# NBDsoftware/deep_cartograph

Measured on AMD Instinct MI355X. Metric: Deep-TICA training frames/sec on 10Mx512 feature matrix at 1/2/4/8 GPUs, higher is better.
Workload: dtype f32

## Files before the change

### deep_cartograph_amd/_lib.py

```python
from __future__ import annotations

import ctypes as C
import os

_HERE = os.path.dirname(os.path.abspath(__file__))
LIB_PATH = os.path.join(_HERE, "csrc", "libdcv.so")

DCV_MAX_LAYERS = 16
ACT = {None: 0, "linear": 0, "leaky_relu": 1, "relu": 2, "tanh": 3, "elu": 4, "softplus": 5, "shifted_softplus": 6, "custom_sigmoid": 7}
OPTIMIZER = {"Adam": 0, "AdamW": 1, "SGD": 2, "RMSprop": 3, "Adagrad": 4, "Adamax": 5, "NAdam": 6, "RAdam": 7, "Adadelta": 8, "ASGD": 9, "Rprop": 10}
MODEL_DEEPTICA = 1
MODEL_AE = 2
MODEL_VAE = 3
FEAT_DISTANCE, FEAT_TORSION_SINCOS, FEAT_TORSION = 0, 1, 2


class MlpDesc(C.Structure):
    _fields_ = [
        ("model", C.c_int32),
        ("n_layers", C.c_int32),
        ("dims", C.c_int32 * (DCV_MAX_LAYERS + 1)),
        ("act", C.c_int32 * DCV_MAX_LAYERS),
        ("latent_layer", C.c_int32),
        ("lag", C.c_int32),
        ("max_batch", C.c_int32),
        ("tica_reg", C.c_double),
        ("lr", C.c_double),
        ("beta1", C.c_double),
        ("beta2", C.c_double),
        ("eps", C.c_double),
        ("weight_decay", C.c_double),
        ("optimizer", C.c_int32),
        ("amsgrad", C.c_int32),
        ("nesterov", C.c_int32),
        ("centered", C.c_int32),
        ("momentum", C.c_double),
        ("dampening", C.c_double),
        ("alpha", C.c_double),
        ("lr_decay", C.c_double),
        ("initial_accumulator_value", C.c_double),
        ("opt_p", C.c_double * 4),
        ("dropout", C.c_float * DCV_MAX_LAYERS),
        ("seed", C.c_uint64),
        ("batchnorm", C.c_int32 * DCV_MAX_LAYERS),
        ("bn_eps", C.c_double),
        ("bn_momentum", C.c_double),
        ("maximize", C.c_int32),
    ]


class DcvError(RuntimeError):
    pass


_P = C.c_void_p
_I64 = C.c_int64
_I32 = C.c_int32
_SZ = C.c_size_t

SIGNATURES = {
    "dcv_abi_version": (C.c_int, []),
    "dcv_last_error": (C.c_char_p, []),
    "dcv_device_info": (C.c_int, [C.c_int, C.POINTER(C.c_int), C.POINTER(_I64), C.c_char_p, _SZ]),
    "dcv_col_stats_workspace": (_SZ, [_I64, _I32]),
    "dcv_col_stats": (C.c_int, [_P, _I64, _I32, _I64, _P, _P, _SZ, _P]),
    "dcv_col_histogram_workspace": (_SZ, [_I64, _I32, _I32]),
    "dcv_col_histogram": (C.c_int, [_P, _I64, _I32, _I64, _P, _I32, _P, _P, _SZ, _P]),
    "dcv_dip_sorted_workspace": (_SZ, [_I64, _I32]),
    "dcv_dip_sorted": (C.c_int, [_P, _I64, _I32, _I64, _P, _P, _P, _P, _SZ, _P]),
    "dcv_featurize_workspace": (_SZ, [_I64, _I32, _I32]),
    "dcv_featurize": (C.c_int, [_P, _I64, _I64, _I64, _I64, _I32, _P, _I32, C.c_double, _P, _I64, _P, _SZ, _P]),
    "dcv_normalize": (C.c_int, [_P, _P, _I64, _I32, _I64, _I64, _P, _P, _P]),
    "dcv_lagged_cov_workspace": (_SZ, [_I64, _I32, _I32]),
    "dcv_lagged_cov": (C.c_int, [_P, _I64, _I32, _I64, _I32, _P, _P, _P, _SZ, _P]),
    "dcv_project_linear_workspace": (_SZ, [_I64, _I32, _I32]),
    "dcv_project_linear": (C.c_int, [_P, _I64, _I32, _I64, _P, _P, _P, _I32, _P, _P, _P, _P, _P, _P, _SZ, _P]),
    "dcv_mlp_create": (C.c_int, [C.POINTER(MlpDesc), C.POINTER(_P)]),
    "dcv_mlp_destroy": (None, [_P]),
    "dcv_mlp_num_params": (_I64, [_P]),
    "dcv_mlp_param_offset": (_I64, [_P, _I32, _I32]),
    "dcv_mlp_params": (_P, [_P]),
    "dcv_mlp_grads": (_P, [_P]),
    "dcv_mlp_set_params": (C.c_int, [_P, _P, _P]),
    "dcv_mlp_get_params": (C.c_int, [_P, _P, _P]),
    "dcv_mlp_set_lr": (C.c_int, [_P, C.c_double]),
    "dcv_mlp_set_momentum": (C.c_int, [_P, C.c_double]),
    "dcv_mlp_dropout_mask": (C.c_int, [_P, _I32, _I64, _I64, _P, _P]),
    "dcv_mlp_dropout_step": (_I64, [_P]),
    "dcv_mlp_last_path": (_I32, [_P]),
    "dcv_mlp_last_eval_group": (_I32, [_P]),
    "dcv_gemm_tn_split": (C.c_int, [_P, _I64, _P, _I64, _P, _I64, _I64, _I64, _I64, _I64, _P]),
    "dcv_mlp_set_row_sharing": (C.c_int, [_P, _I32]),
    "dcv_mlp_set_feature_range": (C.c_int, [_P, _P, _P]),
    "dcv_mlp_set_kl_beta": (C.c_int, [_P, C.c_double]),
    "dcv_mlp_set_noise": (C.c_int, [_P, _P, _I64]),
    "dcv_mlp_noise_position": (_I64, [_P]),
    "dcv_mlp_latent_sample": (C.c_int, [_P, _I64, _P, _P]),
    "dcv_mlp_forward": (C.c_int, [_P, _P, _I64, _P, _I64, _I32, _I32, _P]),
    "dcv_mlp_stats": (_P, [_P]),
    "dcv_mlp_stats_len": (_I32, [_P]),
    "dcv_mlp_backward": (C.c_int, [_P, _P, _I64, _P, _I64, _I32, _I64, _I32, _P]),
    "dcv_mlp_apply": (C.c_int, [_P, _P]),
    "dcv_mlp_set_upper_grads_callback": (C.c_int, [_P, _P, _P]),
    "dcv_mlp_dp_step": (C.c_int, [_P, _P, _I64, _P, _I64, _I32, _I64, _I32, _I32, _P, _P, _P]),
    "dcv_comm_unique_id": (C.c_int, [_P]),
    "dcv_comm_create": (C.c_int, [_I32, _I32, _P, C.POINTER(_P)]),
    "dcv_comm_destroy": (None, [_P]),
    "dcv_comm_bind_stream": (C.c_int, [_P, _P]),
    "dcv_comm_allreduce": (C.c_int, [_P, _P, _I64, _I32, _I32, _P]),
    "dcv_comm_dp_allreduce_fn": (_P, []),
    "dcv_comm_world": (_I32, [_P]),
    "dcv_comm_rank": (_I32, [_P]),
    "dcv_mlp_set_rank": (C.c_int, [_P, _I32]),
    "dcv_mlp_bn_state": (C.c_int, [_P, _I32, _P, _P, C.POINTER(_I64), _I32, _P]),
    "dcv_mlp_layer_output": (C.c_int, [_P, _I32, _I64, _P, _P]),
    "dcv_mlp_train_step": (C.c_int, [_P, _P, _I64, _P, _I64, _I32, _P]),
    "dcv_mlp_eval_step": (C.c_int, [_P, _P, _I64, _P, _I64, _I32, _P]),
    "dcv_mlp_eval_steps": (C.c_int, [_P, _P, _I64, _P, _I64, _I32, _I32, _P]),
    "dcv_mlp_train_steps": (C.c_int, [_P, _P, _I64, _P, _I64, _I32, _I32, _P]),
    "dcv_mlp_log_width": (_I32, [_P]),
    "dcv_mlp_reset_log": (C.c_int, [_P, _I32, _P]),
    "dcv_mlp_read_log": (C.c_int, [_P, _P, _I32, C.POINTER(_I32), _P]),
    "dcv_mlp_profile_begin": (C.c_int, [_P, _I32, _I32]),
    "dcv_mlp_profile_end": (C.c_int, [_P, _P, _P]),
    "dcv_mlp_profile_pause": (C.c_int, [_P, _I32]),
    "dcv_mlp_graph_launches": (_I64, [_P]),
    "dcv_mlp_set_graph": (C.c_int, [_P, _I32]),
    "dcv_mlp_infer": (C.c_int, [_P, _P, _I64, _I64, _P, _P, _P, _P, _P, _P, _P]),
    "dcv_mlp_input_sensitivity_workspace": (_SZ, [_P, _I64]),
    "dcv_mlp_input_sensitivity": (C.c_int, [_P, _P, _I64, _I64, _P, _P, _P, _P, _SZ, _P]),
    "dcv_kmeans_workspace": (_SZ, [_I64, _I32, _I32]),
    "dcv_kmeans_step": (C.c_int, [_P, _I64, _I32, _P, _P, _I32, _P, _P, _P, _P, _SZ, _P]),
    "dcv_kmeanspp_workspace": (_SZ, [_I64, _I32]),
    "dcv_kmeanspp_potentials": (C.c_int, [_P, _I64, _I32, _P, _P, _I32, _P, _P, _P, _SZ, _P]),
    "dcv_kmeanspp_update": (C.c_int, [_P, _I64, _I32, _P, _P, _I32, _P, _P, _P, _SZ, _P]),
    "dcv_set_gemm_mode": (C.c_int, [C.c_int]),
    "dcv_get_gemm_mode": (C.c_int, []),
    "dcv_label_stats_workspace": (_SZ, [_I64, _I32, _I32]),
    "dcv_label_stats": (C.c_int, [_P, _I64, _I32, _P, _P, _I32, _P, _P, _SZ, _P]),
    "dcv_cluster_dist_sums": (C.c_int, [_P, _I64, _P, _P, _I32, _I32, _P, _P]),
    "dcv_silhouette_sum_workspace": (_SZ, [_I64]),
    "dcv_silhouette_sum": (C.c_int, [_P, _I64, _I32, _P, _P, _P, _P, _SZ, _P]),
    "dcv_linear_binning_workspace": (_SZ, [_I32, _I32]),
    "dcv_linear_binning": (C.c_int, [_P, _I64, _I64, _I32, _P, _P, _P, _I32, _P, _P, _P, _SZ, _P]),
    "dcv_nearest_rows_workspace": (_SZ, [_I64, _I32, _I32]),
    "dcv_nearest_rows": (C.c_int, [_P, _I64, _I32, _P, _I32, _I64, _P, _P, _P, _SZ, _P]),
    "dcv_nearest_point": (C.c_int, [_P, _I64, _P, _I64, _I32, _P, _P]),
    "dcv_linkage_workspace": (_SZ, [_I64, _I32]),
    "dcv_linkage_pdist": (C.c_int, [_P, _I64, _I32, _P, _SZ, _P]),
    "dcv_linkage": (C.c_int, [_P, _I64, _I32, _I32, _P, C.POINTER(_I64), _P, _SZ, _P]),
    "dcv_core_distances_workspace": (_SZ, [_I64, _I32, _I32]),
    "dcv_core_distances": (C.c_int, [_P, _I64, _I32, _I32, _P, _P, _SZ, _P]),
    "dcv_mr_mst_workspace": (_SZ, [_I64, _I32]),
    "dcv_mr_mst": (C.c_int, [_P, _I64, _I32, _P, _P, _P, _P, _P, _SZ, _P]),
    "dcv_gemm_f32": (C.c_int, [_I32, _P, _I64, _P, _I64, _P, _I64, _I64, _I64, _I64, _P]),
}

_lib = None


def load():
    global _lib
    if _lib is not None:
        return _lib
    if not os.path.exists(LIB_PATH):
        raise DcvError(
            f"libdcv.so not found at {LIB_PATH}: build it with `python -c 'import __graft_entry__ as g; g.build()'` "
            "or `make -C deep_cartograph_amd/csrc` -- there is no CPU fallback")
    lib = C.CDLL(LIB_PATH)
    for name, (res, args) in SIGNATURES.items():
        fn = getattr(lib, name)
        fn.restype = res
        fn.argtypes = args
    ver = lib.dcv_abi_version()
    if ver != 5:
        raise DcvError(f"libdcv.so ABI version {ver}, expected 5 (rebuild: make -C deep_cartograph_amd/csrc)")
    _lib = lib
    return lib


def check(rc: int, what: str = ""):
    if rc != 0:
        msg = load().dcv_last_error().decode(errors="replace")
        raise DcvError(f"{what} failed (code {rc}): {msg}")
```

### deep_cartograph_amd/csrc/mlp.hip

```cpp
#include "mlp_state.h"
#include <new>
#include <math.h>
#include <utility>

using namespace dcv;

namespace dcv {

__global__ __launch_bounds__(256) void colsum_kernel(const float* __restrict__ Z, int64_t rows, int n, int64_t ld,
                                                     float* __restrict__ part) {
    __shared__ float red[256];
    const int64_t r0 = (int64_t)blockIdx.x * kColsumRows;
    const int64_t r1 = r0 + kColsumRows < rows ? r0 + kColsumRows : rows;
    const int t = threadIdx.x;
    const int cols = n < 256 ? n : 256;
    const int groups = 256 / cols;
    const int c_in = t % cols, g = t / cols;
    for (int c0 = 0; c0 < n; c0 += cols) {
        const int c = c0 + c_in;
        float s = 0.f;
        if (g < groups && c < n) {
            for (int64_t rb = r0 + g; rb < r1; rb += 8 * (int64_t)groups) {
                float v[8];
#pragma unroll
                for (int u = 0; u < 8; ++u) {
                    const int64_t r = rb + (int64_t)u * groups;
                    v[u] = r < r1 ? Z[r * ld + c] : 0.f;
                }
#pragma unroll
                for (int u = 0; u < 8; ++u) s += v[u];
            }
        }
        red[t] = s;
        __syncthreads();
        if (g == 0 && c < n) {
            float tot = 0.f;
            for (int q = 0; q < groups; ++q) tot += red[q * cols + c_in];
            part[(int64_t)blockIdx.x * n + c] = tot;
        }
        __syncthreads();
    }
}

__global__ __launch_bounds__(kVaeRows) void vae_sample_kernel(const float* __restrict__ H, int64_t ldh, int64_t R, int d,
                                                             const float* __restrict__ eps, float* __restrict__ Z, int64_t ldz,
                                                             double* __restrict__ part) {
    __shared__ double red[kVaeRows];
    const int t = threadIdx.x;
    const int64_t r = (int64_t)blockIdx.x * kVaeRows + t;
    double kl = 0.0;
    if (r < R) {
        for (int j = 0; j < d; ++j) {
            const float mu = H[r * ldh + j], lv = H[r * ldh + d + j];
            Z[r * ldz + j] = __fadd_rn(__fmul_rn(eps[r * d + j], expf(0.5f * lv)), mu);
            kl += (double)lv - exp((double)lv) - (double)mu * (double)mu + 1.0;
        }
        kl *= -0.5;
    }
    red[t] = kl;
    __syncthreads();
    for (int off = kVaeRows / 2; off > 0; off >>= 1) {
        if (t < off) red[t] += red[t + off];
        __syncthreads();
    }
    if (t == 0) part[blockIdx.x] = red[0];
}

__global__ __launch_bounds__(kVaeRows) void vae_sample_backward_kernel(const float* __restrict__ H, int64_t ldh, int64_t R, int d,
                                                                      const float* __restrict__ eps, float* __restrict__ G, int64_t ldg,
                                                                      float beta_over_b) {
    const int64_t r = (int64_t)blockIdx.x * kVaeRows + threadIdx.x;
    if (r >= R) return;
    float dz[8];
    for (int j = 0; j < d; ++j) dz[j] = G[r * ldg + j];
    for (int j = 0; j < d; ++j) {
        const float mu = H[r * ldh + j], lv = H[r * ldh + d + j];
        G[r * ldg + j] = dz[j] + beta_over_b * mu;
        G[r * ldg + d + j] = dz[j] * eps[r * d + j] * 0.5f * expf(0.5f * lv) + beta_over_b * 0.5f * (expf(lv) - 1.f);
    }
}

__global__ __launch_bounds__(256) void dropout_mask_kernel(float* __restrict__ out, int64_t rows, int width, DropCfg drop) {
    const int q4 = (width + 3) / 4;
    for (int64_t i = (int64_t)blockIdx.x * 256 + threadIdx.x; i < rows * q4; i += (int64_t)gridDim.x * 256) {
        const int64_t r = i / q4;
        const int c = (int)(i - r * q4) * 4;
        const float4 k = drop.thr != 0u ? drop.mult(r, c) : make_float4(1.f, 1.f, 1.f, 1.f);
        float* o = out + r * width + c;
        o[0] = k.x;
        if (c + 1 < width) o[1] = k.y;
        if (c + 2 < width) o[2] = k.z;
        if (c + 3 < width) o[3] = k.w;
    }
}

static void wgrad_plan(int out, int in, int64_t rows, int64_t* k_chunk, int64_t* splits) {
    const int64_t tiles = (out <= 32 ? 1 : cdiv(out, 128)) * (in <= 32 ? 1 : cdiv(in, 128));
    int64_t want = cdiv(2 * (int64_t)num_cus(), tiles);
    int64_t max_by_rows = cdiv(rows, 256);
    static const bool q_wide = [] { const char* e = getenv("DCV_WGRAD_Q"); return e && e[0] == '1'; }();
    const int64_t tiles_q = cdiv(out, 64) * cdiv(in, 64);
    const int64_t want_q = cdiv(cdiv(2 * (int64_t)num_cus(), tiles_q), 8) * 8;
    if (out > 32 && in > 32 && want_q <= max_by_rows) {
        int64_t kc = cdiv(cdiv(rows, want_q), 32) * 32;
        if (cdiv(rows, kc) % 8 != 0) kc = cdiv(rows, want_q);
        if (tiles * cdiv(rows, kc) <= (int64_t)num_cus() / 2 &&
            (want > max_by_rows || (q_wide && kc <= 1024))) {
            *k_chunk = kc;
            *splits = cdiv(rows, kc);
            return;
        }
    }
    if (want > max_by_rows) {
        want = max_by_rows >= 8 ? max_by_rows / 8 * 8 : max_by_rows;
    }
    if (want < 1) want = 1;
    int64_t kc = cdiv(cdiv(rows, want), 32) * 32;
    *k_chunk = kc;
    *splits = cdiv(rows, kc);
}

static void mlp_free(dcv_mlp* m) {
    if (!m) return;
    snet_free(m);
    snet_dt_free(m);
    snet_image_free(m);
    auto f = [](void* p) { if (p) (void)hipFree(p); };
    f(m->params); f(m->grads); f(m->adam_m); f(m->adam_v); f(m->opt_aux); f(m->dZ[0]); f(m->dZ[1]); f(m->stats); f(m->gradp);
    f(m->spart); f(m->log); f(m->log_count); f(m->ticket); f(m->feat_range); f(m->ident); f(m->zeros_d); f(m->ones_d); f(m->proj_ws);
    f(m->vae_z); f(m->vae_kpart);
    for (auto& l : m->layers) { f(l.H); f(l.slab); f(l.bpart); f(l.mask); f(l.Y); f(l.rm); f(l.rv); f(l.bn_stat); f(l.bn_part); f(l.bn_gpart); f(l.bn_bpart); }
    g_launch_ev = LaunchEvents{};
    g_launch_taken = nullptr;
    for (hipEvent_t e : m->prof_ev) (void)hipEventDestroy(e);
    f(m->tail.ws); f(m->tail.cnt); f(m->eval_ws.base);
    for (int i = 0; i < 4; ++i) if (m->gexec[i]) (void)hipGraphExecDestroy(m->gexec[i]);
    delete m;
}

static int reset_bn_state(dcv_mlp* m, hipStream_t s) {
    for (auto& p : m->layers) {
        if (!p.bn) continue;
        DCV_CHECK_HIP(hipMemsetAsync(p.rm, 0, (size_t)p.out * sizeof(float), s));
        launch_fill(p.rv, (int64_t)p.out, 1.f, 1, 256, s);
        DCV_CHECK_LAUNCH();
        p.bn_batches = 0;
    }
    return DCV_OK;
}

static int create_validate(const dcv_mlp_desc* desc) {
    const int L = desc->n_layers;
    DCV_REQUIRE(desc->model == DCV_MODEL_DEEPTICA || desc->model == DCV_MODEL_AE || desc->model == DCV_MODEL_VAE, "dcv_mlp_create: unknown model %d",
                desc->model);
    DCV_REQUIRE(L >= 1 && L <= DCV_MAX_LAYERS, "dcv_mlp_create: n_layers=%d out of range", L);
    for (int l = 0; l <= L; ++l) DCV_REQUIRE(desc->dims[l] >= 1, "dcv_mlp_create: dims[%d]=%d", l, desc->dims[l]);
    for (int l = 0; l < L; ++l)
        DCV_REQUIRE(desc->act[l] >= DCV_ACT_NONE && desc->act[l] <= DCV_ACT_CUSTOM_SIGMOID, "dcv_mlp_create: act[%d]=%d unsupported", l, desc->act[l]);
    for (int l = 0; l < L; ++l)
        DCV_REQUIRE(desc->dropout[l] >= 0.f && desc->dropout[l] < 1.f, "dcv_mlp_create: dropout[%d]=%g outside [0, 1)", l, (double)desc->dropout[l]);
    DCV_REQUIRE(desc->optimizer >= DCV_OPT_ADAM && desc->optimizer <= DCV_OPT_RPROP, "dcv_mlp_create: optimizer %d unknown", desc->optimizer);
    DCV_REQUIRE(desc->max_batch >= 1, "dcv_mlp_create: max_batch=%d", desc->max_batch);
    if (desc->model == DCV_MODEL_DEEPTICA) {
        DCV_REQUIRE(desc->dims[L] <= kMaxTicaDim, "dcv_mlp_create: Deep-TICA output dimension %d > %d", desc->dims[L], kMaxTicaDim);
        DCV_REQUIRE(desc->lag >= 0, "dcv_mlp_create: lag=%d", desc->lag);
    } else {
        DCV_REQUIRE(desc->dims[L] == desc->dims[0], "dcv_mlp_create: autoencoder must map F=%d back to F (got %d)", desc->dims[0], desc->dims[L]);
        DCV_REQUIRE(desc->latent_layer >= 1 && desc->latent_layer < L, "dcv_mlp_create: latent_layer=%d", desc->latent_layer);
        DCV_REQUIRE(desc->dims[desc->latent_layer] <= 16, "dcv_mlp_create: latent dimension %d > 16", desc->dims[desc->latent_layer]);
        if (desc->model == DCV_MODEL_VAE) {
            const int h = desc->latent_layer - 1;
            DCV_REQUIRE(desc->dims[desc->latent_layer] % 2 == 0 && desc->dims[desc->latent_layer] <= 16,
                        "dcv_mlp_create: VAE head layer %d must output 2 * d <= 16 columns (got %d)", h, desc->dims[desc->latent_layer]);
            DCV_REQUIRE(desc->act[h] == DCV_ACT_NONE && !(desc->dropout[h] > 0.f) && !desc->batchnorm[h],
                        "dcv_mlp_create: the VAE heads (Linear %d) take no activation, dropout or batch normalisation", h);
        }
    }
    return DCV_OK;
}
static int proj_dim(const dcv_mlp* m) {
    return m->desc.model == DCV_MODEL_AE ? m->desc.dims[m->desc.latent_layer] : m->desc.model == DCV_MODEL_VAE ? m->vae_d : m->d_out;
}
static void plan_layers(dcv_mlp* m) {
    const dcv_mlp_desc* desc = &m->desc;
    const int L = m->L;
    m->layers.resize(L);
    int64_t off = 0;
    int maxdim = 0;
    for (int l = 0; l < L; ++l) {
        LayerPlan& p = m->layers[l];
        p.in = m->vae_d > 0 && l == desc->latent_layer ? m->vae_d : desc->dims[l];
        p.out = desc->dims[l + 1];
        p.act = desc->act[l];
        p.w_off = off;
        off += align_up((size_t)p.in * p.out, 4);
        p.b_off = off;
        off += align_up((size_t)p.out, 4);
        p.bn = desc->batchnorm[l] ? 1 : 0;
        if (p.bn) {
            p.g_off = off;
            off += align_up((size_t)p.out, 4);
            p.be_off = off;
            off += align_up((size_t)p.out, 4);
            m->any_bn = true;
        }
        p.ldh = align_up((size_t)p.out, 4);
        if (p.out > maxdim) maxdim = p.out;
        wgrad_plan(p.out, p.in, m->rows_cap, &p.k_chunk_cap, &p.max_splits);
        p.max_splits = cdiv(m->rows_cap, 256) > p.max_splits ? p.max_splits : cdiv(m->rows_cap, 256);
        if (p.max_splits < 1) p.max_splits = 1;
        if (l == L - 1 && p.out <= 8) {
            int64_t hb = 4 * (int64_t)num_cus();
            if (hb > cdiv(m->rows_cap, 32)) hb = cdiv(m->rows_cap, 32);
            if (hb > p.max_splits) p.max_splits = hb;
        }
    }
    m->n_params = off;
    m->ld_dz = align_up((size_t)maxdim, 4);
    const int d = m->d_out;
    m->stats_len = desc->model == DCV_MODEL_DEEPTICA ? 2 * d + 2 * d * d : desc->model == DCV_MODEL_VAE ? 2 : 1;
    m->log_width = desc->model == DCV_MODEL_DEEPTICA ? 2 + 2 * d * d + d : desc->model == DCV_MODEL_VAE ? 4 : 2;
    m->spart_blocks = desc->model == DCV_MODEL_DEEPTICA ? (int)cdiv(desc->max_batch, kStatBlockRows) : (int)cdiv(m->rows_cap, kSseRows);
}
static int alloc_buffers(dcv_mlp* m) {
    const dcv_mlp_desc* desc = &m->desc;
    int rc = DCV_OK;
    for (int l = 0; l < m->L && rc == DCV_OK; ++l) {
        LayerPlan& p = m->layers[l];
        rc = dmalloc(&p.H, (size_t)m->rows_cap * p.ldh);
        if (rc == DCV_OK) rc = dmalloc(&p.slab, (size_t)p.max_splits * p.in * p.out);
        if (rc == DCV_OK) rc = dmalloc(&p.bpart, (size_t)cdiv(m->rows_cap, 32) * p.out);
        if (rc == DCV_OK && p.bn) {
            const size_t nblk = (size_t)cdiv(m->rows_cap, 256) + 2;
            rc = dmalloc(&p.Y, (size_t)m->rows_cap * p.ldh);
            if (rc == DCV_OK) rc = dmalloc(&p.rm, (size_t)p.out);
            if (rc == DCV_OK) rc = dmalloc(&p.rv, (size_t)p.out);
            if (rc == DCV_OK) rc = dmalloc(&p.bn_stat, (size_t)4 * p.out);
            if (rc == DCV_OK) rc = dmalloc(&p.bn_part, nblk * 2 * p.out);
            if (rc == DCV_OK) rc = dmalloc(&p.bn_gpart, nblk * p.out);
            if (rc == DCV_OK) rc = dmalloc(&p.bn_bpart, nblk * p.out);
        }
        if (rc == DCV_OK && l + 1 < m->L && (p.act == DCV_ACT_RELU || p.act == DCV_ACT_LEAKY_RELU))
            rc = dmalloc(&p.mask, (size_t)((m->rows_cap + 128) * (int64_t)(p.out + 128)) / 64 + 64);
    }
    const int dl = proj_dim(m);
    if (rc == DCV_OK) rc = dmalloc(&m->params, (size_t)m->n_params);
    if (rc == DCV_OK) rc = dmalloc(&m->grads, (size_t)m->n_params);
    if (rc == DCV_OK) rc = dmalloc(&m->adam_m, (size_t)m->n_params);
    if (rc == DCV_OK) rc = dmalloc(&m->adam_v, (size_t)m->n_params);
    if (rc == DCV_OK && (((desc->optimizer == DCV_OPT_ADAM || desc->optimizer == DCV_OPT_ADAMW) && desc->amsgrad) ||
                         (desc->optimizer == DCV_OPT_RMSPROP && desc->centered)))
        rc = dmalloc(&m->opt_aux, (size_t)m->n_params);
    if (rc == DCV_OK) rc = dmalloc(&m->dZ[0], (size_t)m->rows_cap * m->ld_dz);
    if (rc == DCV_OK) rc = dmalloc(&m->dZ[1], (size_t)m->rows_cap * m->ld_dz);
    if (rc == DCV_OK) rc = dmalloc(&m->stats, (size_t)m->stats_len);
    if (rc == DCV_OK) rc = dmalloc(&m->gradp, (size_t)(2 * kMaxTicaDim + 2 * kMaxTicaDim * kMaxTicaDim));
    if (rc == DCV_OK) rc = dmalloc(&m->spart, (size_t)m->spart_blocks * m->stats_len);
    if (rc == DCV_OK) rc = dmalloc(&m->log_count, 1);
    if (rc == DCV_OK) rc = dmalloc(&m->ticket, 4);
    if (rc == DCV_OK) rc = dmalloc(&m->feat_range, (size_t)desc->dims[0]);
    if (rc == DCV_OK && m->vae_d > 0) rc = dmalloc(&m->vae_z, (size_t)m->rows_cap * m->ld_z);
    if (rc == DCV_OK && m->vae_d > 0) rc = dmalloc(&m->vae_kpart, (size_t)cdiv(m->rows_cap, kVaeRows));
    if (rc == DCV_OK) rc = dmalloc(&m->ident, (size_t)dl * dl);
    if (rc == DCV_OK) rc = dmalloc(&m->zeros_d, (size_t)dl);
    if (rc == DCV_OK) rc = dmalloc(&m->ones_d, (size_t)dl);
    m->proj_ws_bytes = dcv_project_linear_workspace(m->rows_cap, dl, dl);
    if (rc == DCV_OK) rc = dmalloc(reinterpret_cast<char**>(&m->proj_ws), m->proj_ws_bytes);
    return rc;
}
static int init_device_state(dcv_mlp* m) {
    const int dl = proj_dim(m);
    hipError_t e = hipMemset(m->params, 0, m->n_params * sizeof(float));
    if (e == hipSuccess) e = hipMemset(m->grads, 0, m->n_params * sizeof(float));
    if (e == hipSuccess && reset_opt_state(m, nullptr) != DCV_OK) e = hipErrorUnknown;
    if (e == hipSuccess) e = hipMemset(m->log_count, 0, sizeof(int));
    if (e == hipSuccess) e = hipMemset(m->ticket, 0, 4 * sizeof(unsigned));
    if (e == hipSuccess) e = hipMemset(m->zeros_d, 0, dl * sizeof(float));
    if (e == hipSuccess) e = hipMemset(m->ident, 0, (size_t)dl * dl * sizeof(float));
    if (e == hipSuccess) {
        launch_fill(m->ones_d, (int64_t)dl, 1.f, 1, 64, nullptr);
        launch_fill(m->feat_range, (int64_t)m->desc.dims[0], 1.f, 4, 256, nullptr);
        std::vector<float> eye((size_t)dl * dl, 0.f);
        for (int i = 0; i < dl; ++i) eye[(size_t)i * dl + i] = 1.f;
        e = hipMemcpy(m->ident, eye.data(), eye.size() * sizeof(float), hipMemcpyHostToDevice);
    }
    if (e == hipSuccess) {
        for (auto& p : m->layers)
            if (p.bn) launch_fill(m->params + p.g_off, (int64_t)p.out, 1.f, 1, 256, nullptr);
        if (reset_bn_state(m, nullptr) != DCV_OK) e = hipErrorUnknown;
    }
    if (e == hipSuccess) (void)alloc_tail_ws(&m->tail, 8);
    if (e == hipSuccess) e = hipDeviceSynchronize();
    if (e == hipSuccess) return DCV_OK;
    set_error("dcv_mlp_create: initialisation failed: %s", hipGetErrorString(e));
    return DCV_EHIP;
}

}

extern "C" int dcv_mlp_create(const dcv_mlp_desc* desc, dcv_mlp** out) {
    DCV_REQUIRE(desc && out, "dcv_mlp_create: null argument");
    *out = nullptr;
    int rc = create_validate(desc);
    if (rc) return rc;
    dcv_mlp* m = new (std::nothrow) dcv_mlp();
    DCV_REQUIRE(m, "dcv_mlp_create: out of host memory");
    m->desc = *desc;
    m->L = desc->n_layers;
    m->d_out = desc->dims[m->L];
    m->rows_cap = desc->model == DCV_MODEL_DEEPTICA ? 2 * (int64_t)desc->max_batch : desc->max_batch;
    m->lr = desc->lr;
    m->momentum_rt = (desc->optimizer == DCV_OPT_ADAM || desc->optimizer == DCV_OPT_ADAMW || desc->optimizer == DCV_OPT_ADAMAX ||
                      desc->optimizer == DCV_OPT_NADAM || desc->optimizer == DCV_OPT_RADAM) ? desc->beta1 : desc->momentum;
    for (int l = 0; l < m->L; ++l) m->any_drop = m->any_drop || desc->dropout[l] > 0.f;
    m->vae_d = desc->model == DCV_MODEL_VAE ? desc->dims[desc->latent_layer] / 2 : 0;
    m->ld_z = align_up((size_t)(m->vae_d > 0 ? m->vae_d : 1), 4);
    static const bool graph_env = [] { const char* e = getenv("DCV_GRAPH"); return e && e[0] == '1'; }();
    m->graph_on = graph_env;
    plan_layers(m);
    rc = alloc_buffers(m);
    if (rc == DCV_OK) rc = init_device_state(m);
    if (rc != DCV_OK) {
        mlp_free(m);
        return rc;
    }
    *out = m;
    return DCV_OK;
}

extern "C" void dcv_mlp_destroy(dcv_mlp* m) { mlp_free(m); }
extern "C" int64_t dcv_mlp_num_params(const dcv_mlp* m) { return m ? m->n_params : 0; }
extern "C" int64_t dcv_mlp_param_offset(const dcv_mlp* m, int32_t layer, int32_t which) {
    if (!m || layer < 0 || layer >= m->L) return -1;
    if (which == 2) return m->layers[layer].g_off;
    if (which == 3) return m->layers[layer].be_off;
    return which == 0 ? m->layers[layer].w_off : m->layers[layer].b_off;
}
extern "C" float* dcv_mlp_params(dcv_mlp* m) { return m ? m->params : nullptr; }
extern "C" float* dcv_mlp_grads(dcv_mlp* m) { return m ? m->grads : nullptr; }
extern "C" double* dcv_mlp_stats(dcv_mlp* m) { return m ? m->stats : nullptr; }
extern "C" int32_t dcv_mlp_stats_len(const dcv_mlp* m) { return m ? m->stats_len : 0; }
extern "C" int32_t dcv_mlp_log_width(const dcv_mlp* m) { return m ? m->log_width : 0; }

extern "C" int dcv_mlp_set_params(dcv_mlp* m, const float* params_h, void* stream) {
    DCV_REQUIRE(m && params_h, "dcv_mlp_set_params: null argument");
    hipStream_t s = as_stream(stream);
    DCV_CHECK_HIP(hipMemcpyAsync(m->params, params_h, m->n_params * sizeof(float), hipMemcpyHostToDevice, s));
    int rc = reset_opt_state(m, s);
    if (rc == DCV_OK) rc = reset_bn_state(m, s);
    if (rc == DCV_OK) rc = snet_image_repack(m, s);
    if (rc) return rc;
    DCV_CHECK_HIP(hipStreamSynchronize(s));
    return DCV_OK;
}

extern "C" int dcv_mlp_get_params(dcv_mlp* m, float* params_h, void* stream) {
    DCV_REQUIRE(m && params_h, "dcv_mlp_get_params: null argument");
    hipStream_t s = as_stream(stream);
    DCV_CHECK_HIP(hipMemcpyAsync(params_h, m->params, m->n_params * sizeof(float), hipMemcpyDeviceToHost, s));
    DCV_CHECK_HIP(hipStreamSynchronize(s));
    return DCV_OK;
}

extern "C" int dcv_mlp_bn_state(dcv_mlp* m, int32_t layer, float* running_mean_h, float* running_var_h, int64_t* num_batches_tracked,
                                int32_t set, void* stream) {
    DCV_REQUIRE(m && layer >= 0 && layer < m->L && running_mean_h && running_var_h && num_batches_tracked, "dcv_mlp_bn_state: bad arguments");
    LayerPlan& p = m->layers[layer];
    DCV_REQUIRE(p.bn, "dcv_mlp_bn_state: layer %d has no batch normalisation", layer);
    hipStream_t s = as_stream(stream);
    const size_t bytes = (size_t)p.out * sizeof(float);
    if (set) {
        DCV_CHECK_HIP(hipMemcpyAsync(p.rm, running_mean_h, bytes, hipMemcpyHostToDevice, s));
        DCV_CHECK_HIP(hipMemcpyAsync(p.rv, running_var_h, bytes, hipMemcpyHostToDevice, s));
        p.bn_batches = *num_batches_tracked;
    } else {
        DCV_CHECK_HIP(hipMemcpyAsync(running_mean_h, p.rm, bytes, hipMemcpyDeviceToHost, s));
        DCV_CHECK_HIP(hipMemcpyAsync(running_var_h, p.rv, bytes, hipMemcpyDeviceToHost, s));
        *num_batches_tracked = p.bn_batches;
    }
    DCV_CHECK_HIP(hipStreamSynchronize(s));
    return DCV_OK;
}

extern "C" int dcv_mlp_set_row_sharing(dcv_mlp* m, int32_t enable) {
    DCV_REQUIRE(m, "dcv_mlp_set_row_sharing: null");
    m->no_row_sharing = enable ? 0 : 1;
    return DCV_OK;
}

extern "C" int dcv_mlp_set_lr(dcv_mlp* m, double lr) {
    DCV_REQUIRE(m, "dcv_mlp_set_lr: null");
    m->lr = lr;
    return DCV_OK;
}

extern "C" int dcv_mlp_set_momentum(dcv_mlp* m, double value) {
    DCV_REQUIRE(m, "dcv_mlp_set_momentum: null");
    m->momentum_rt = value;
    return DCV_OK;
}

extern "C" int dcv_mlp_set_upper_grads_callback(dcv_mlp* m, void (*fn)(void*), void* user) {
    DCV_REQUIRE(m, "dcv_mlp_set_upper_grads_callback: null");
    m->upper_cb = fn;
    m->upper_cb_user = user;
    return DCV_OK;
}

extern "C" int dcv_mlp_set_rank(dcv_mlp* m, int32_t rank) {
    DCV_REQUIRE(m && rank >= 0, "dcv_mlp_set_rank: bad arguments");
    m->drop_rank = (uint32_t)rank;
    return DCV_OK;
}

extern "C" int dcv_mlp_layer_output(dcv_mlp* m, int32_t layer, int64_t rows, float* out_d, void* stream) {
    DCV_REQUIRE(m && out_d && layer >= 0 && layer < m->L && rows >= 1 && rows <= m->rows_cap, "dcv_mlp_layer_output: bad arguments");
    if (m->last_path != 0) {
        set_error("dcv_mlp_layer_output: the last forward ran as a fused small-network launch (activations never left LDS); set DCV_NO_SNET=1");
        return DCV_ESTATE;
    }
    const LayerPlan& p = m->layers[layer];
    DCV_CHECK_HIP(hipMemcpy2DAsync(out_d, (size_t)p.out * sizeof(float), p.H, (size_t)p.ldh * sizeof(float), (size_t)p.out * sizeof(float),
                                   (size_t)rows, hipMemcpyDeviceToDevice, as_stream(stream)));
    return DCV_OK;
}

extern "C" int64_t dcv_mlp_dropout_step(const dcv_mlp* m) { return m ? m->drop_step : 0; }
extern "C" int32_t dcv_mlp_last_path(const dcv_mlp* m) { return m ? m->last_path : -1; }
extern "C" int32_t dcv_mlp_last_eval_group(const dcv_mlp* m) { return m ? m->last_eval_group : -1; }

extern "C" int dcv_mlp_dropout_mask(dcv_mlp* m, int32_t layer, int64_t step, int64_t rows, float* out_d, void* stream) {
    DCV_REQUIRE(m && out_d && layer >= 0 && layer < m->L && rows >= 1 && step >= 0, "dcv_mlp_dropout_mask: bad arguments");
    const bool keep_mode = m->fwd_train;
    const int64_t keep_step = m->cur_step;
    m->fwd_train = true;
    m->cur_step = step;
    const DropCfg dc = drop_cfg(m, layer);
    m->fwd_train = keep_mode;
    m->cur_step = keep_step;
    const int width = m->layers[layer].out;
    int64_t blocks = cdiv(rows * ((width + 3) / 4), 256);
    if (blocks > 4096) blocks = 4096;
    hipLaunchKernelGGL(dropout_mask_kernel, dim3((unsigned)blocks), dim3(256), 0, as_stream(stream), out_d, rows, width, dc);
    DCV_CHECK_LAUNCH();
    return DCV_OK;
}

extern "C" int dcv_mlp_set_feature_range(dcv_mlp* m, const float* range_h, void* stream) {
    DCV_REQUIRE(m && range_h, "dcv_mlp_set_feature_range: null argument");
    hipStream_t s = as_stream(stream);
    DCV_CHECK_HIP(hipMemcpyAsync(m->feat_range, range_h, m->desc.dims[0] * sizeof(float), hipMemcpyHostToDevice, s));
    DCV_CHECK_HIP(hipStreamSynchronize(s));
    return DCV_OK;
}

extern "C" int dcv_mlp_set_kl_beta(dcv_mlp* m, double beta) {
    DCV_REQUIRE(m && m->vae_d > 0, "dcv_mlp_set_kl_beta: not a variational autoencoder");
    m->kl_beta = beta;
    return DCV_OK;
}

extern "C" int dcv_mlp_set_noise(dcv_mlp* m, const float* eps_d, int64_t rows) {
    DCV_REQUIRE(m && m->vae_d > 0, "dcv_mlp_set_noise: not a variational autoencoder");
    DCV_REQUIRE(rows >= 0 && (eps_d != nullptr || rows == 0), "dcv_mlp_set_noise: bad arguments");
    m->noise = eps_d;
    m->noise_rows = rows;
    m->noise_pos = 0;
    return DCV_OK;
}

extern "C" int64_t dcv_mlp_noise_position(const dcv_mlp* m) { return m ? m->noise_pos : -1; }

extern "C" int dcv_mlp_latent_sample(dcv_mlp* m, int64_t rows, float* out_d, void* stream) {
    DCV_REQUIRE(m && out_d && m->vae_d > 0, "dcv_mlp_latent_sample: bad arguments");
    DCV_REQUIRE(rows >= 1 && rows <= m->last_batch, "dcv_mlp_latent_sample: rows=%lld outside [1, %d]", (long long)rows, m->last_batch);
    if (m->last_path != 0) {
        set_error("dcv_mlp_latent_sample: the last forward ran fused: z never left LDS");
        return DCV_ESTATE;
    }
    DCV_CHECK_HIP(hipMemcpy2DAsync(out_d, (size_t)m->vae_d * sizeof(float), m->vae_z, (size_t)m->ld_z * sizeof(float), (size_t)m->vae_d * sizeof(float),
                                   (size_t)rows, hipMemcpyDeviceToDevice, as_stream(stream)));
    return DCV_OK;
}

extern "C" int dcv_mlp_reset_log(dcv_mlp* m, int32_t capacity, void* stream) {
    DCV_REQUIRE(m && capacity >= 1, "dcv_mlp_reset_log: bad arguments");
    hipStream_t s = as_stream(stream);
    if (capacity > m->log_cap) {
        DCV_CHECK_HIP(hipStreamSynchronize(s));
        if (m->log) (void)hipFree(m->log);
        m->log = nullptr;
        m->log_cap = 0;
        int rc = dmalloc(&m->log, (size_t)capacity * m->log_width);
        if (rc) return rc;
        m->log_cap = capacity;
    }
    DCV_CHECK_HIP(hipMemsetAsync(m->log_count, 0, sizeof(int), s));
    return DCV_OK;
}

extern "C" int dcv_mlp_read_log(dcv_mlp* m, double* out_h, int32_t max_records, int32_t* n_records, void* stream) {
    DCV_REQUIRE(m && out_h && n_records, "dcv_mlp_read_log: null argument");
    hipStream_t s = as_stream(stream);
    int cnt = 0;
    DCV_CHECK_HIP(hipMemcpyAsync(&cnt, m->log_count, sizeof(int), hipMemcpyDeviceToHost, s));
    DCV_CHECK_HIP(hipStreamSynchronize(s));
    if (cnt > m->log_cap) cnt = m->log_cap;
    if (cnt > max_records) cnt = max_records;
    if (cnt > 0) {
        DCV_CHECK_HIP(hipMemcpyAsync(out_h, m->log, (size_t)cnt * m->log_width * sizeof(double), hipMemcpyDeviceToHost, s));
        DCV_CHECK_HIP(hipStreamSynchronize(s));
    }
    *n_records = cnt;
    return DCV_OK;
}

namespace dcv {

static bool act_mask_enabled() {
    static const bool off = [] { const char* e = getenv("DCV_NO_ACT_MASK"); return e && e[0] == '1'; }();
    return !off;
}

int run_forward(dcv_mlp* m, const float* Xn, int64_t ld, const RowMap& rows_map, int64_t rows, int n_run, hipStream_t s,
                bool for_backward) {
    for (int l = 0; l < n_run; ++l) {
        LayerPlan& p = m->layers[l];
        p.mask_rows = -1;
        const bool from_z = m->vae_d > 0 && l == m->desc.latent_layer;
        if (from_z) {
            const LayerPlan& hd = m->layers[l - 1];
            m->vae_kblocks = (int)cdiv(rows, kVaeRows);
            hipLaunchKernelGGL(vae_sample_kernel, dim3((unsigned)m->vae_kblocks), dim3(kVaeRows), 0, s, (const float*)hd.H, hd.ldh, rows, m->vae_d,
                               m->eps_cur, m->vae_z, m->ld_z, m->vae_kpart);
            DCV_CHECK_LAUNCH();
        }
        Operand A = l == 0 ? make_operand(Xn, ld, p.in, rows_map)
                           : from_z ? make_operand(m->vae_z, m->ld_z, p.in) : make_operand(layer_out(m, l - 1), m->layers[l - 1].ldh, p.in);
        Operand B = make_operand(m->params + p.w_off, p.in, p.in);
        if (l + 1 < n_run && next_layer_fusable(m, l)) {
            LayerPlan& nx = m->layers[l + 1];
            const bool vec = quad_ok(p.H, p.ldh) && quad_ok(m->params + p.b_off, 4) && quad_ok(m->params + nx.w_off, nx.in);
            prof_mark(m, l, 0, 0, s);
            int rc;
            if (nx.out <= 4) {
                EpiBiasActHead<4> epi{p.H, p.ldh, m->params + p.b_off, p.act, vec, m->params + nx.w_off, nx.in, m->params + nx.b_off, nx.out, nx.act, nx.H, nx.ldh};
                epi.drop = drop_cfg(m, l);
                rc = gemm_nt_head4(A, B, rows, p.out, p.in, epi, s, &m->tail);
            } else {
                EpiBiasActHead<8> epi{p.H, p.ldh, m->params + p.b_off, p.act, vec, m->params + nx.w_off, nx.in, m->params + nx.b_off, nx.out, nx.act, nx.H, nx.ldh};
                epi.drop = drop_cfg(m, l);
                rc = gemm_nt_head8(A, B, rows, p.out, p.in, epi, s, &m->tail);
            }
            if (rc) return rc;
            prof_mark(m, l, 0, 1, s);
            prof_mark(m, l + 1, 0, 0, s);
            prof_mark(m, l + 1, 0, 1, s);
            ++l;
            continue;
        }
        EpiBiasAct epi{p.H, p.ldh, m->params + p.b_off, p.act, quad_ok(p.H, p.ldh) && quad_ok(m->params + p.b_off, 4)};
        epi.drop = drop_cfg(m, l);
        if (for_backward && p.mask && act_mask_enabled()) {
            epi.mask = p.mask;
            p.mask_rows = rows;
        }
        prof_mark(m, l, 0, 0, s);
        if (p.bn) {
            epi.mask = nullptr;
            p.mask_rows = -1;
        }
        int rc = gemm_nt_bias_act(A, B, rows, p.out, p.in, epi, s, &m->tail);
        if (rc) return rc;
        if (p.bn) {
            const bool train = m->fwd_train && for_backward;
            if (train && rows_map.half > 0) {
                rc = bn_forward(m, l, 0, rows_map.half, true, s);
                if (rc == DCV_OK) rc = bn_forward(m, l, rows_map.half, rows - rows_map.half, true, s);
            } else {
                rc = bn_forward(m, l, 0, rows, train, s);
            }
            if (rc) return rc;
        }
        prof_mark(m, l, 0, 1, s);
    }
    return DCV_OK;
}

template <class F>
static int run_graphed(dcv_mlp* m, int slot, hipStream_t s, F&& body) {
    if (!m->graph_on || m->graph_off || s == nullptr || (m->prof_level > 0 && !m->prof_paused) || !m->gwarm[slot]) {
        m->gwarm[slot] = true;
        return body();
    }
    if (hipStreamBeginCapture(s, hipStreamCaptureModeThreadLocal) != hipSuccess) {
        (void)hipGetLastError();
        return body();
    }
    struct HostStep {
        int64_t adam_t, drop_step, cur_step;
        double mu_product, eta;
        int64_t bn_batches[DCV_MAX_LAYERS];
        int64_t noise_pos;
        const float* eps_cur;
    };
    auto snap = [&]() {
        HostStep h{m->adam_t, m->drop_step, m->cur_step, m->nadam_mu_product, m->asgd_eta, {}, m->noise_pos, m->eps_cur};
        for (int l = 0; l < m->L; ++l) h.bn_batches[l] = m->layers[l].bn_batches;
        return h;
    };
    auto restore = [&](const HostStep& h) {
        m->adam_t = h.adam_t; m->drop_step = h.drop_step; m->cur_step = h.cur_step;
        m->nadam_mu_product = h.mu_product; m->asgd_eta = h.eta;
        for (int l = 0; l < m->L; ++l) m->layers[l].bn_batches = h.bn_batches[l];
        m->noise_pos = h.noise_pos; m->eps_cur = h.eps_cur;
    };
    const HostStep h0 = snap();
    const int rc = body();
    hipGraph_t g = nullptr;
    const hipError_t ec = hipStreamEndCapture(s, &g);
    if (rc != DCV_OK || ec != hipSuccess || g == nullptr) {
        if (g) (void)hipGraphDestroy(g);
        (void)hipGetLastError();
        if (rc != DCV_OK) return rc;
        m->gwarm[slot] = false;
        restore(h0);
        return body();
    }
    if (m->gexec[slot]) {
        hipGraphNode_t err_node = nullptr;
        hipGraphExecUpdateResult res = hipGraphExecUpdateSuccess;
        if (hipGraphExecUpdate(m->gexec[slot], g, &err_node, &res) != hipSuccess || res != hipGraphExecUpdateSuccess) {
            (void)hipGetLastError();
            (void)hipGraphExecDestroy(m->gexec[slot]);
            m->gexec[slot] = nullptr;
        }
    }
    if (!m->gexec[slot] && hipGraphInstantiate(&m->gexec[slot], g, nullptr, nullptr, 0) != hipSuccess) {
        (void)hipGetLastError();
        m->gexec[slot] = nullptr;
    }
    (void)hipGraphDestroy(g);
    if (!m->gexec[slot]) {
        m->graph_off = true;
        restore(h0);
        return body();
    }
    DCV_CHECK_HIP(hipGraphLaunch(m->gexec[slot], s));
    m->graph_launches += 1;
    return DCV_OK;
}

bool peek_noise(dcv_mlp* m, int64_t rows) {
    if (m->noise == nullptr || m->noise_pos + rows > m->noise_rows) return false;
    m->eps_cur = m->noise + m->noise_pos * m->vae_d;
    return true;
}
static int take_noise(dcv_mlp* m, int64_t batch) {
    if (!peek_noise(m, batch)) {
        set_error("dcv_mlp step: the VAE noise buffer holds %lld rows, %lld used, a step of %lld rows needs more (dcv_mlp_set_noise)",
                  (long long)m->noise_rows, (long long)m->noise_pos, (long long)batch);
        return DCV_ESTATE;
    }
    m->noise_pos += batch;
    return DCV_OK;
}

int forward_impl(dcv_mlp* m, const float* Xn_d, int64_t ld, const int64_t* idx_d, int64_t row0, int32_t batch, int32_t train, void* stream,
                 int fuse_head) {
    DCV_REQUIRE(m && Xn_d, "dcv_mlp_forward: null argument");
    DCV_REQUIRE(batch >= 1 && batch <= m->desc.max_batch, "dcv_mlp_forward: batch=%d exceeds max_batch=%d", batch, m->desc.max_batch);
    DCV_REQUIRE(ld >= m->desc.dims[0], "dcv_mlp_forward: ld=%lld < F=%d", (long long)ld, m->desc.dims[0]);
    if (fuse_head) DCV_REQUIRE(m->log && m->log_cap > 0, "dcv_mlp step: call dcv_mlp_reset_log first");
    if (m->vae_d > 0) {
        const int rcn = take_noise(m, batch);
        if (rcn) return rcn;
    }
    g_launch_ev = LaunchEvents{};
    step_begin(m, train != 0);
    step_done(m, 0, m->last_batch, false);
    hipStream_t s = as_stream(stream);
    if (m->desc.model == DCV_MODEL_DEEPTICA && !(m->snet_dt_tried && m->snet_dt == nullptr)) {
        prof_mark(m, 0, 0, 0, s);
        const int rcs = snet_dt_forward(m, Xn_d, ld, idx_d, row0, batch, fuse_head == 2 ? 2 : 0, fuse_head != 2, s);
        if (rcs < 0) return rcs;
        if (rcs == DCV_OK) {
            prof_mark(m, 0, 0, 1, s);
            step_done(m, 2, batch, fuse_head == 2);
            return DCV_OK;
        }
        if (prof_on(m, 0)) g_launch_ev = LaunchEvents{};
    }
    const RowMap rm = batch_rows(m, idx_d, row0, batch);
    const int64_t R = rows_of(m, idx_d, batch);
    int rc = run_forward(m, Xn_d, ld, rm, R, m->L, s, fuse_head != 2);
    if (rc) return rc;
    const LayerPlan& last = m->layers[m->L - 1];
    const float* net_out = layer_out(m, m->L - 1);
    bool head_ran = fuse_head != 0;
    if (m->desc.model == DCV_MODEL_DEEPTICA) rc = tica_stats(m, net_out, last.ldh, batch, lag_offset(m, idx_d, batch), fuse_head, &head_ran, s);
    else rc = ae_sse(m, net_out, last.ldh, Xn_d, ld, rm, R, batch, fuse_head != 0, s);
    if (rc) return rc;
    step_done(m, 0, batch, head_ran);
    return DCV_OK;
}

struct Backward {
    dcv_mlp* m;
    const float* Xn;
    int64_t ld;
    const int64_t* idx;
    RowMap rm;
    int64_t R;
    int32_t batch;
    int64_t global_batch;
    hipStream_t s;
    float *dz_cur, *dz_nxt;
    int bblocks;
    ReduceArgs ra;
};

static int backward_blob(dcv_mlp* m, int32_t batch, int64_t global_batch, bool head_in_bwd, bool fuse_opt, hipStream_t s) {
    if (!m->snet_fwd_valid) {
        set_error("dcv_mlp_backward: the fused forward of this batch kept no activations (evaluation step)");
        return DCV_ESTATE;
    }
    ReduceArgsView v;
    prof_mark(m, 0, 1, 0, s);
    const int rc = snet_dt_backward(m, batch, global_batch, head_in_bwd, &v, s);
    if (rc) return rc;
    prof_mark(m, 0, 1, 1, s);
    return finish_grads(m, reduce_args_of(m, v), fuse_opt, false, s);
}
static int seed_gradient(Backward& c, bool fused_head) {
    dcv_mlp* m = c.m;
    const LayerPlan& last = m->layers[m->L - 1];
    const float* net_out = layer_out(m, m->L - 1);
    const int act = last.bn ? DCV_ACT_NONE : last.act;
    const DropCfg drop = last.bn ? kNoDrop : drop_cfg(m, m->L - 1);
    const float hscale = last.bn ? 1.f : drop_hscale(m, m->L - 1);
    int rc = DCV_OK;
    if (!fused_head)
        rc = loss_gradient(m, net_out, last.ldh, c.Xn, c.ld, c.rm, c.R, c.batch, lag_offset(m, c.idx, c.batch), c.global_batch, act, c.dz_cur, drop, hscale, c.s);
    c.bblocks = (int)cdiv(c.R, kColsumRows);
    if (rc == DCV_OK && !fused_head && !last.bn) {
        hipLaunchKernelGGL(colsum_kernel, dim3(c.bblocks), dim3(256), 0, c.s, c.dz_cur, c.R, last.out, m->ld_dz, last.bpart);
        DCV_CHECK_LAUNCH();
    }
    return rc;
}
static int norm_backward(Backward& c, int l) {
    const LayerPlan& p = c.m->layers[l];
    const bool two = c.rm.half > 0;
    int nb = 0;
    const int rc = bn_backward(c.m, l, c.dz_cur, c.m->ld_dz, two ? 2 : 1, two ? (int64_t)c.rm.half : c.R, p.act, drop_hscale(c.m, l), drop_cfg(c.m, l), &nb, c.s);
    if (rc) return rc;
    c.bblocks = nb;
    c.ra.l[c.m->L + l] = ReduceDesc{p.bn_gpart, p.bn_bpart, p.g_off, p.be_off, p.out, p.out, nb, nb, 0, 0};
    return DCV_OK;
}
static int head_backward_layer(Backward& c) {
    dcv_mlp* m = c.m;
    const int l = m->L - 1;
    prof_mark(m, l, 1, 0, c.s);
    const int rc = head_backward(m, c.R, c.batch, lag_offset(m, c.idx, c.batch), c.dz_nxt, &c.bblocks, c.s);
    if (rc) return rc;
    prof_mark(m, l, 1, 1, c.s);
    prof_mark(m, l, 2, 0, c.s);
    prof_mark(m, l, 2, 1, c.s);
    c.ra.l[l] = linear_reduce_desc(m->layers[l], c.bblocks, c.bblocks);
    std::swap(c.dz_cur, c.dz_nxt);
    return DCV_OK;
}
static int64_t plan_wgrad(Backward& c, int l) {
    const LayerPlan& p = c.m->layers[l];
    int64_t kc, splits;
    wgrad_plan(p.out, p.in, c.R, &kc, &splits);
    if (splits > p.max_splits) {
        splits = p.max_splits;
        kc = cdiv(cdiv(c.R, splits), 32) * 32;
        splits = cdiv(c.R, kc);
    }
    c.ra.l[l] = linear_reduce_desc(p, (int)splits, c.bblocks);
    return kc;
}
static EpiSlab slab_epi(const LayerPlan& p) { return EpiSlab{p.slab, p.out, p.in, 1, 0, quad_ok(p.slab, p.in), p.max_splits}; }
static int wgrad_alone(Backward& c, int l, const Operand& B, int64_t kc) {
    const LayerPlan& p = c.m->layers[l];
    prof_mark(c.m, l, 1, 0, c.s);
    const int rc = gemm_tn_slab(make_operand(c.dz_cur, c.m->ld_dz, p.out), B, p.out, p.in, c.R, kc, slab_epi(p), c.s);
    if (rc) return rc;
    prof_mark(c.m, l, 1, 1, c.s);
    return DCV_OK;
}
static int latent_backward_layer(Backward& c, int l) {
    dcv_mlp* m = c.m;
    const LayerPlan& p = m->layers[l];
    const LayerPlan& hd = m->layers[l - 1];
    const int64_t kc = plan_wgrad(c, l);
    int rc = wgrad_alone(c, l, make_operand(m->vae_z, m->ld_z, p.in), kc);
    if (rc) return rc;
    Operand A = make_operand(c.dz_cur, m->ld_dz, p.out);
    Operand Bd = make_operand(m->params + p.w_off, p.in, p.in);
    EpiActGrad eg{c.dz_nxt, m->ld_dz, m->vae_z, m->ld_z, DCV_ACT_NONE, hd.bpart, p.in, quad_ok(c.dz_nxt, m->ld_dz) && quad_ok(m->vae_z, m->ld_z)};
    int dblocks = 0;
    prof_mark(m, l, 2, 0, c.s);
    rc = gemm_nn_act_grad(A, Bd, c.R, p.in, p.out, eg, c.s, &dblocks, &m->tail);
    if (rc) return rc;
    hipLaunchKernelGGL(vae_sample_backward_kernel, dim3((unsigned)cdiv(c.R, kVaeRows)), dim3(kVaeRows), 0, c.s, (const float*)hd.H, hd.ldh, c.R, m->vae_d,
                       m->eps_cur, c.dz_nxt, m->ld_dz, (float)(m->kl_beta / (double)c.global_batch));
    DCV_CHECK_LAUNCH();
    c.bblocks = (int)cdiv(c.R, kColsumRows);
    hipLaunchKernelGGL(colsum_kernel, dim3(c.bblocks), dim3(256), 0, c.s, (const float*)c.dz_nxt, c.R, hd.out, m->ld_dz, hd.bpart);
    DCV_CHECK_LAUNCH();
    prof_mark(m, l, 2, 1, c.s);
    std::swap(c.dz_cur, c.dz_nxt);
    return DCV_OK;
}
static int backward_layer(Backward& c, int l) {
    dcv_mlp* m = c.m;
    hipStream_t s = c.s;
    const LayerPlan& p = m->layers[l];
    const int64_t R = c.R;
    const int64_t kc = plan_wgrad(c, l);
    if (l == 0) return wgrad_alone(c, l, make_operand(c.Xn, c.ld, p.in, c.rm), kc);
    const LayerPlan& q = m->layers[l - 1];
    Operand A = make_operand(c.dz_cur, m->ld_dz, p.out);
    Operand B = make_operand(layer_out(m, l - 1), q.ldh, p.in);
    const EpiSlab epi = slab_epi(p);
    Operand Bd = make_operand(m->params + p.w_off, p.in, p.in);
    EpiActGrad eg{c.dz_nxt, m->ld_dz, q.H, q.ldh, q.act, q.bpart, q.out, quad_ok(c.dz_nxt, m->ld_dz) && quad_ok(q.H, q.ldh)};
    if (q.mask && q.mask_rows == R) {
        eg.mask = q.mask;
        eg.slope = q.act == DCV_ACT_LEAKY_RELU ? 0.01f : 0.f;
    }
    eg.drop = drop_cfg(m, l - 1);
    eg.hscale = drop_hscale(m, l - 1);
    if (q.bn) {
        eg.act = DCV_ACT_NONE;
        eg.mask = nullptr;
        eg.drop = kNoDrop;
        eg.hscale = 1.f;
    }
    prof_mark(m, l, 1, 0, s);
    prof_mark(m, l, 2, 0, s);
    int rc = launch_wgrad_dgrad(A, B, p.out, p.in, R, kc, epi, A, Bd, R, p.in, p.out, eg, &c.bblocks, &m->tail, s);
    if (rc < 0) return rc;
    if (rc == 1) {
        rc = gemm_tn_slab(A, B, p.out, p.in, R, kc, epi, s);
        if (rc) return rc;
        prof_mark(m, l, 1, 1, s);
        prof_mark(m, l, 2, 0, s);
        rc = gemm_nn_act_grad(A, Bd, R, p.in, p.out, eg, s, &c.bblocks, &m->tail);
        if (rc) return rc;
        prof_mark(m, l, 2, 1, s);
    } else {
        prof_mark(m, l, 1, 1, s);
        prof_mark(m, l, 2, 1, s);
    }
    std::swap(c.dz_cur, c.dz_nxt);
    return DCV_OK;
}

int backward_impl(dcv_mlp* m, const float* Xn_d, int64_t ld, const int64_t* idx_d, int64_t row0, int32_t batch, int64_t global_batch, int32_t train,
                  void* stream, bool fuse_opt) {
    DCV_REQUIRE(m && Xn_d, "dcv_mlp_backward: null argument");
    g_launch_ev = LaunchEvents{};
    if (m->last_batch != batch) {
        set_error("dcv_mlp_backward: batch=%d does not match the preceding forward (%d)", batch, m->last_batch);
        return DCV_ESTATE;
    }
    DCV_REQUIRE(global_batch >= batch, "dcv_mlp_backward: global_batch=%lld < batch=%d", (long long)global_batch, batch);
    if (m->any_drop && train && !m->fwd_train) {
        set_error("dcv_mlp_backward: train=1 after an evaluation-mode forward (dropout masks would not match)");
        return DCV_ESTATE;
    }
    DCV_REQUIRE(m->log && m->log_cap > 0, "dcv_mlp_backward: call dcv_mlp_reset_log first");
    hipStream_t s = as_stream(stream);
    const bool tica = m->desc.model == DCV_MODEL_DEEPTICA;
    const bool head_in_bwd = tica && m->last_path == 2 && train && !m->head_done && m->snet_fwd_valid;
    int rc = loss_record(m, global_batch, train != 0, head_in_bwd, s);
    if (rc || !train) return rc;
    if (tica && m->last_path == 2) return backward_blob(m, batch, global_batch, head_in_bwd, fuse_opt, s);
    const int L = m->L;
    Backward c{m, Xn_d, ld, idx_d, batch_rows(m, idx_d, row0, batch), rows_of(m, idx_d, batch), batch, global_batch, s, m->dZ[0], m->dZ[1], 0, ReduceArgs{}};
    c.ra.L = L;
    const bool fused_head = tica && head_fusable(m);
    rc = seed_gradient(c, fused_head);
    bool upper_done = false;
    for (int l = L - 1; l >= 0 && rc == DCV_OK; --l) {
        if (l == 0) rc = reduce_upper(m, c.ra, fuse_opt, &upper_done, s);
        if (rc == DCV_OK && m->layers[l].bn) rc = norm_backward(c, l);
        if (rc) break;
        if (fused_head && l == L - 1) rc = head_backward_layer(c);
        else if (m->vae_d > 0 && l == m->desc.latent_layer) rc = latent_backward_layer(c, l);
        else rc = backward_layer(c, l);
    }
    if (rc) return rc;
    return finish_grads(m, c.ra, fuse_opt, upper_done, s);
}

static int snet_step(dcv_mlp* m, const float* Xn_d, int64_t ld, const int64_t* idx_d, int64_t row0, int32_t batch, int32_t train, void* stream) {
    if ((m->desc.model != DCV_MODEL_AE && m->desc.model != DCV_MODEL_VAE) || m->any_drop || m->any_bn || (m->snet_tried && m->snet == nullptr)) return 1;
    if (!(Xn_d && batch >= 1 && batch <= m->desc.max_batch && ld >= m->desc.dims[0] && m->log && m->log_cap > 0)) return 1;
    if (m->vae_d > 0 && !peek_noise(m, batch)) return 1;
    hipStream_t s = as_stream(stream);
    ReduceArgsView v;
    prof_mark(m, 0, 0, 0, s);
    prof_mark(m, 0, 1, 0, s);
    int rc = snet_ae_step(m, Xn_d, ld, RowMap{idx_d, row0, 0, 0}, batch, batch, train, &v, s);
    if (rc) return rc;
    if (m->vae_d > 0) m->noise_pos += batch;
    prof_mark(m, 0, 0, 1, s);
    prof_mark(m, 0, 1, 1, s);
    step_begin(m, train != 0);
    step_done(m, 1, batch, false);
    if (!train) return DCV_OK;
    return finish_grads(m, reduce_args_of(m, v), true, false, s);
}

}

extern "C" int dcv_mlp_profile_begin(dcv_mlp* m, int32_t max_steps, int32_t level) {
    DCV_REQUIRE(m && max_steps >= 1 && (level == 1 || level == 2), "dcv_mlp_profile_begin: bad arguments");
    const size_t need = (size_t)3 * m->L * max_steps * 2;
    while (m->prof_ev.size() < need) {
        hipEvent_t e;
        DCV_CHECK_HIP(hipEventCreate(&e));
        m->prof_ev.push_back(e);
    }
    m->prof_cap = max_steps;
    m->prof_cnt.assign((size_t)3 * m->L, 0);
    m->prof_kind_off = 0;
    m->prof_paused = false;
    m->prof_level = level;
    return DCV_OK;
}

extern "C" int dcv_mlp_profile_pause(dcv_mlp* m, int32_t paused) {
    DCV_REQUIRE(m, "dcv_mlp_profile_pause: null");
    m->prof_paused = (paused & 1) != 0;
    m->prof_kind_off = (paused >> 1) & 7;
    return DCV_OK;
}

extern "C" int dcv_mlp_profile_end(dcv_mlp* m, double* ms_h, int32_t* counts_h) {
    DCV_REQUIRE(m && ms_h && counts_h, "dcv_mlp_profile_end: null argument");
    const int level = m->prof_level;
    m->prof_level = 0;
    for (int c = 0; c < 3 * m->L; ++c) {
        ms_h[c] = 0.0;
        counts_h[c] = 0;
        const int layer = c / 3, kind = c % 3;
        if (level < 2 && layer != 0) continue;
        if (kind == 2 && layer == 0) continue;
        const int steps = (size_t)c < m->prof_cnt.size() ? m->prof_cnt[c] : 0;
        for (int i = 0; i < steps; ++i) {
            hipEvent_t a = m->prof_ev[((size_t)c * m->prof_cap + i) * 2 + 0];
            hipEvent_t b = m->prof_ev[((size_t)c * m->prof_cap + i) * 2 + 1];
            DCV_CHECK_HIP(hipEventSynchronize(b));
            float ms = 0.f;
            DCV_CHECK_HIP(hipEventElapsedTime(&ms, a, b));
            ms_h[c] += (double)ms;
            counts_h[c] += 1;
        }
    }
    return DCV_OK;
}

extern "C" int dcv_mlp_forward(dcv_mlp* m, const float* Xn_d, int64_t ld, const int64_t* idx_d, int64_t row0, int32_t batch,
                               int32_t train, void* stream) {
    DCV_REQUIRE(m, "dcv_mlp_forward: null");
    return run_graphed(m, 1, as_stream(stream), [&] { return forward_impl(m, Xn_d, ld, idx_d, row0, batch, train, stream); });
}

extern "C" int dcv_mlp_backward(dcv_mlp* m, const float* Xn_d, int64_t ld, const int64_t* idx_d, int64_t row0, int32_t batch,
                                int64_t global_batch, int32_t train, void* stream) {
    DCV_REQUIRE(m, "dcv_mlp_backward: null");
    if (!train) return backward_impl(m, Xn_d, ld, idx_d, row0, batch, global_batch, train, stream);
    return run_graphed(m, 2, as_stream(stream), [&] { return backward_impl(m, Xn_d, ld, idx_d, row0, batch, global_batch, train, stream); });
}

extern "C" int dcv_mlp_apply(dcv_mlp* m, void* stream) { return apply_impl(m, stream); }
extern "C" int64_t dcv_mlp_graph_launches(const dcv_mlp* m) { return m ? m->graph_launches : 0; }
extern "C" int dcv_mlp_set_graph(dcv_mlp* m, int32_t enable) {
    DCV_REQUIRE(m, "dcv_mlp_set_graph: null");
    m->graph_on = enable != 0;
    return DCV_OK;
}

static int one_step(dcv_mlp* m, const float* Xn_d, int64_t ld, const int64_t* idx_d, int64_t row0, int32_t batch, int32_t train, void* stream) {
    int rc = snet_step(m, Xn_d, ld, idx_d, row0, batch, train, stream);
    if (rc != 1) return rc;
    rc = forward_impl(m, Xn_d, ld, idx_d, row0, batch, train, stream, train ? 1 : 2);
    if (rc) return rc;
    return backward_impl(m, Xn_d, ld, idx_d, row0, batch, batch, train, stream, train != 0);
}
extern "C" int dcv_mlp_train_step(dcv_mlp* m, const float* Xn_d, int64_t ld, const int64_t* idx_d, int64_t row0, int32_t batch,
                                  void* stream) {
    DCV_REQUIRE(m, "dcv_mlp_train_step: null");
    return run_graphed(m, 0, as_stream(stream), [&] { return one_step(m, Xn_d, ld, idx_d, row0, batch, 1, stream); });
}

extern "C" int dcv_mlp_eval_step(dcv_mlp* m, const float* Xn_d, int64_t ld, const int64_t* idx_d, int64_t row0, int32_t batch,
                                 void* stream) {
    DCV_REQUIRE(m, "dcv_mlp_eval_step: null");
    return run_graphed(m, 3, as_stream(stream), [&] { return one_step(m, Xn_d, ld, idx_d, row0, batch, 0, stream); });
}
```

### deep_cartograph_amd/csrc/mlp_opt.hip

```cpp
#include "mlp_state.h"
#include <math.h>

namespace dcv {

static inline int64_t rd_wstride(const ReduceDesc& d) { return d.w_stride > 0 ? d.w_stride : d.w_count; }
static inline int64_t rd_bstride(const ReduceDesc& d) { return d.b_stride > 0 ? d.b_stride : (int64_t)d.out; }

struct OptArgs {
    int kind, flag;
    int first;
    float lr, b1, b2, eps, wd;
    float c1, c2;
    float w1, w2;
    float decay;
    float p0, p1, p2, p3;
    int maximize;
    float* img;
    const int* img_idx;
};
template <bool WT>
__device__ __forceinline__ void opt_st(float* p, float v) {
    if constexpr (WT) handoff_store(p, v);
    else *p = v;
}
template <bool WT>
__device__ __forceinline__ void opt_stp(const OptArgs& a, float* p, int64_t i, float v) {
    opt_st<WT>(p + i, v);
    if (a.img != nullptr) {
        const int j = a.img_idx[i];
        if (j >= 0) opt_st<WT>(a.img + j, v);
    }
}
template <bool WT = false>
__device__ __forceinline__ void opt_update_p(int64_t i, float gi, float pi, float* __restrict__ p, float* __restrict__ s1, float* __restrict__ s2,
                                             float* __restrict__ s3, const OptArgs& a) {
    if (a.maximize) gi = -gi;
    switch (a.kind) {
        case DCV_OPT_ADAM:
        case DCV_OPT_ADAMW: {
            if (a.kind == DCV_OPT_ADAMW) pi = pi * a.decay;
            else if (a.wd != 0.f) gi = fmaf(a.wd, pi, gi);
            float mi = s1[i], vi = s2[i];
            mi = mi + (gi - mi) * a.w1;
            vi = vi * a.b2 + a.w2 * gi * gi;
            float vden = vi;
            if (a.flag) {
                vden = fmaxf(s3[i], vi);
                opt_st<WT>(s3 + i, vden);
            }
            const float denom = sqrtf(vden) / a.c2 + a.eps;
            opt_st<WT>(s1 + i, mi);
            opt_st<WT>(s2 + i, vi);
            opt_stp<WT>(a, p, i, pi - a.c1 * (mi / denom));
            break;
        }
        case DCV_OPT_SGD: {
            if (a.wd != 0.f) gi = fmaf(a.wd, pi, gi);
            if (a.b1 != 0.f) {
                float bi = a.first ? gi : s1[i] * a.b1 + a.w1 * gi;
                opt_st<WT>(s1 + i, bi);
                gi = a.flag ? fmaf(a.b1, bi, gi) : bi;
            }
            opt_stp<WT>(a, p, i, pi - a.lr * gi);
            break;
        }
        case DCV_OPT_RMSPROP: {
            if (a.wd != 0.f) gi = fmaf(a.wd, pi, gi);
            float sq = s2[i] * a.b2 + a.w2 * gi * gi;
            opt_st<WT>(s2 + i, sq);
            float avg;
            if (a.flag) {
                float ga = s3[i];
                ga = ga + (gi - ga) * a.w2;
                opt_st<WT>(s3 + i, ga);
                avg = sqrtf(sq - ga * ga) + a.eps;
            } else {
                avg = sqrtf(sq) + a.eps;
            }
            if (a.b1 > 0.f) {
                const float bi = s1[i] * a.b1 + gi / avg;
                opt_st<WT>(s1 + i, bi);
                opt_stp<WT>(a, p, i, pi - a.lr * bi);
            } else {
                opt_stp<WT>(a, p, i, pi - a.lr * (gi / avg));
            }
            break;
        }
        case DCV_OPT_ADAMAX: {
            if (a.wd != 0.f) gi = fmaf(a.wd, pi, gi);
            float mi = s1[i];
            mi = mi + (gi - mi) * a.w1;
            const float ui = fmaxf(s2[i] * a.b2, fabsf(gi) + a.eps);
            opt_st<WT>(s1 + i, mi);
            opt_st<WT>(s2 + i, ui);
            opt_stp<WT>(a, p, i, pi - a.c1 * (mi / ui));
            break;
        }
        case DCV_OPT_NADAM: {
            if (a.wd != 0.f) {
                if (a.flag) pi = pi * a.decay;
                else gi = fmaf(a.wd, pi, gi);
            }
            float mi = s1[i], vi = s2[i];
            mi = mi + (gi - mi) * a.w1;
            vi = vi * a.b2 + a.w2 * gi * gi;
            const float denom = sqrtf(vi / a.c2) + a.eps;
            opt_st<WT>(s1 + i, mi);
            opt_st<WT>(s2 + i, vi);
            pi = pi + a.p0 * (gi / denom);
            opt_stp<WT>(a, p, i, pi + a.p1 * (mi / denom));
            break;
        }
        case DCV_OPT_RADAM: {
            if (a.wd != 0.f) {
                if (a.flag) pi = pi * a.decay;
                else gi = fmaf(a.wd, pi, gi);
            }
            float mi = s1[i], vi = s2[i];
            mi = mi + (gi - mi) * a.w1;
            vi = vi * a.b2 + a.w2 * gi * gi;
            opt_st<WT>(s1 + i, mi);
            opt_st<WT>(s2 + i, vi);
            const float mhat = mi / a.c1;
            if (a.p0 > 0.f) opt_stp<WT>(a, p, i, pi - ((mhat * a.lr) * (a.c2 / (sqrtf(vi) + a.eps))) * a.p0);
            else opt_stp<WT>(a, p, i, pi - mhat * a.lr);
            break;
        }
        case DCV_OPT_ADADELTA: {
            if (a.wd != 0.f) gi = fmaf(a.wd, pi, gi);
            const float sq = s1[i] * a.b2 + a.w2 * gi * gi;
            const float acc = s2[i];
            const float delta = sqrtf(acc + a.eps) / sqrtf(sq + a.eps) * gi;
            opt_st<WT>(s1 + i, sq);
            opt_st<WT>(s2 + i, acc * a.b2 + a.w2 * delta * delta);
            opt_stp<WT>(a, p, i, pi - a.lr * delta);
            break;
        }
        case DCV_OPT_ASGD: {
            if (a.wd != 0.f) gi = fmaf(a.wd, pi, gi);
            pi = pi * a.p0;
            opt_stp<WT>(a, p, i, pi - a.p1 * gi);
            break;
        }
        case DCV_OPT_RPROP: {
            const float sg = gi * s1[i];
            const float f = sg > 0.f ? a.p1 : (sg < 0.f ? a.p0 : 1.f);
            const float st = fminf(fmaxf(s2[i] * f, a.p2), a.p3);
            opt_st<WT>(s2 + i, st);
            if (sg < 0.f) gi = 0.f;
            const float sgn = gi > 0.f ? 1.f : (gi < 0.f ? -1.f : 0.f);
            opt_stp<WT>(a, p, i, pi - sgn * st);
            opt_st<WT>(s1 + i, gi);
            break;
        }
        default: {
            if (a.wd != 0.f) gi = fmaf(a.wd, pi, gi);
            const float su = s2[i] + gi * gi;
            opt_st<WT>(s2 + i, su);
            opt_stp<WT>(a, p, i, pi - a.c1 * (gi / (sqrtf(su) + a.eps)));
            break;
        }
    }
}
__device__ __forceinline__ void opt_update(int64_t i, float gi, float* __restrict__ p, float* __restrict__ s1, float* __restrict__ s2,
                                           float* __restrict__ s3, const OptArgs& a) {
    opt_update_p(i, gi, p[i], p, s1, s2, s3, a);
}
__global__ __launch_bounds__(256) void optimizer_kernel(float* __restrict__ p, const float* __restrict__ g, float* __restrict__ s1,
                                                        float* __restrict__ s2, float* __restrict__ s3, int64_t n, OptArgs a) {
    for (int64_t i = (int64_t)blockIdx.x * 256 + threadIdx.x; i < n; i += (int64_t)gridDim.x * 256) opt_update(i, g[i], p, s1, s2, s3, a);
}

constexpr int kRedWaves = 16;
__global__ __launch_bounds__(64 * kRedWaves) void reduce_grads_kernel(ReduceArgs a, float* __restrict__ grads, float scale, int fuse,
                                                                      float* __restrict__ params, float* __restrict__ s1,
                                                                      float* __restrict__ s2, float* __restrict__ s3, OptArgs oa) {
    __shared__ double s_red[kRedWaves][64];
    const int l = blockIdx.y;
    const ReduceDesc& d = a.l[l];
    const int64_t total = d.w_count + d.out;
    const int lane = threadIdx.x & 63, wave = threadIdx.x >> 6;
    for (int64_t base = (int64_t)blockIdx.x * 64; base < total; base += (int64_t)gridDim.x * 64) {
        const int64_t i = base + lane;
        double s = 0.0;
        if (i < d.w_count) {
            const float* p = d.slab + i;
#pragma unroll 8
            for (int q = wave; q < d.splits; q += kRedWaves) s += (double)p[(int64_t)q * (d.w_stride > 0 ? d.w_stride : d.w_count)];
        } else if (i < total) {
            const float* p = d.bpart + (i - d.w_count);
#pragma unroll 8
            for (int q = wave; q < d.bblocks; q += kRedWaves) s += (double)p[(int64_t)q * (d.b_stride > 0 ? d.b_stride : (int64_t)d.out)];
        }
        s_red[wave][lane] = s;
        __syncthreads();
        if (wave == 0 && i < total) {
            double tot = 0.0;
#pragma unroll
            for (int w = 0; w < kRedWaves; ++w) tot += s_red[w][lane];
            const float g = (float)(tot * (double)scale);
            const int64_t pidx = i < d.w_count ? d.w_off + i : d.b_off + (i - d.w_count);
            grads[pidx] = g;
            if (fuse) opt_update(pidx, g, params, s1, s2, s3, oa);
        }
        __syncthreads();
    }
}

__global__ __launch_bounds__(256) void reduce_grads_small_kernel(ReduceArgs a, float* __restrict__ grads, float scale, int fuse,
                                                                 float* __restrict__ params, float* __restrict__ s1,
                                                                 float* __restrict__ s2, float* __restrict__ s3, OptArgs oa) {
    __shared__ double s_red[4][64];
    const ReduceDesc& d = a.l[blockIdx.y];
    const int64_t total = d.w_count + d.out;
    const int lane = threadIdx.x & 63, wave = threadIdx.x >> 6;
    for (int64_t base = (int64_t)blockIdx.x * 64; base < total; base += (int64_t)gridDim.x * 64) {
        const int64_t i = base + lane;
        double s = 0.0;
        if (i < d.w_count) {
            const float* p = d.slab + i;
#pragma unroll 8
            for (int q = wave; q < d.splits; q += 4) s += (double)p[(int64_t)q * (d.w_stride > 0 ? d.w_stride : d.w_count)];
        } else if (i < total) {
            const float* p = d.bpart + (i - d.w_count);
#pragma unroll 8
            for (int q = wave; q < d.bblocks; q += 4) s += (double)p[(int64_t)q * (d.b_stride > 0 ? d.b_stride : (int64_t)d.out)];
        }
        s_red[wave][lane] = s;
        __syncthreads();
        if (wave == 0 && i < total) {
            const double tot = ((s_red[0][lane] + s_red[1][lane]) + s_red[2][lane]) + s_red[3][lane];
            const float g = (float)(tot * (double)scale);
            const int64_t pidx = i < d.w_count ? d.w_off + i : d.b_off + (i - d.w_count);
            grads[pidx] = g;
            if (fuse) opt_update(pidx, g, params, s1, s2, s3, oa);
        }
        __syncthreads();
    }
}

struct QuadItem {
    const float* src;
    int64_t dst;
    int64_t stride;
    int count, parts;
    int blk0;
    int groups;
};
struct QuadArgs {
    QuadItem it[4 * DCV_MAX_LAYERS];
    int n;
};
inline int quad_groups(int parts) { return parts > 32 ? 16 : 4; }
template <int G>
__device__ __forceinline__ void reduce_quad_block(const QuadItem& d, int blk, float* __restrict__ grads, float scale, int fuse,
                                                  float* __restrict__ params, float* __restrict__ s1, float* __restrict__ s2,
                                                  float* __restrict__ s3, const OptArgs& oa, double* s_red) {
    constexpr int EPB = 1024 / G, TPG = EPB / 4;
    const int t = threadIdx.x, g = t / TPG, sub = t % TPG;
    const int base = blk * EPB;
    const int mine = base + t;
    const bool fin = t < EPB && mine < d.count;
    float pi = 0.f;
    if (fuse && fin) pi = params[d.dst + mine];
    const int e0 = base + 4 * sub;
    double acc[4] = {0.0, 0.0, 0.0, 0.0};
    if (e0 < d.count && (d.stride & 3) == 0 && e0 + 4 <= d.stride && (reinterpret_cast<uintptr_t>(d.src) & 15) == 0) {
        const float* p = d.src + e0;
#pragma unroll 8
        for (int q = g; q < d.parts; q += G) {
            const float4 v = *reinterpret_cast<const float4*>(p + (int64_t)q * d.stride);
            acc[0] += (double)v.x;
            acc[1] += (double)v.y;
            acc[2] += (double)v.z;
            acc[3] += (double)v.w;
        }
    } else if (e0 < d.count) {
        const float* p = d.src + e0;
        const int nv = d.count - e0 < 4 ? d.count - e0 : 4;
#pragma unroll 4
        for (int q = g; q < d.parts; q += G) {
#pragma unroll
            for (int j = 0; j < 4; ++j)
                if (j < nv) acc[j] += (double)p[(int64_t)q * d.stride + j];
        }
    }
#pragma unroll
    for (int j = 0; j < 4; ++j) s_red[g * EPB + 4 * sub + j] = acc[j];
    __syncthreads();
    if (fin) {
        double tot = s_red[t];
#pragma unroll
        for (int k = 1; k < G; ++k) tot += s_red[k * EPB + t];
        const float gr = (float)(tot * (double)scale);
        handoff_store(grads + d.dst + mine, gr);
        if (fuse) opt_update_p<true>(d.dst + mine, gr, pi, params, s1, s2, s3, oa);
    }
}
__global__ __launch_bounds__(256) void reduce_grads_quad_kernel(QuadArgs a, float* __restrict__ grads, float scale, int fuse,
                                                                float* __restrict__ params, float* __restrict__ s1,
                                                                float* __restrict__ s2, float* __restrict__ s3, OptArgs oa) {
    __shared__ double s_red[1024];
    int l = 0;
    while (l + 1 < a.n && (int)blockIdx.x >= a.it[l + 1].blk0) ++l;
    const QuadItem& d = a.it[l];
    const int blk = (int)blockIdx.x - d.blk0;
    if (d.groups == 16) reduce_quad_block<16>(d, blk, grads, scale, fuse, params, s1, s2, s3, oa, s_red);
    else reduce_quad_block<4>(d, blk, grads, scale, fuse, params, s1, s2, s3, oa, s_red);
}

__global__ void fill_kernel(float* p, int64_t n, float v) {
    for (int64_t i = (int64_t)blockIdx.x * blockDim.x + threadIdx.x; i < n; i += (int64_t)gridDim.x * blockDim.x) p[i] = v;
}

void launch_fill(float* p, int64_t n, float v, int blocks, int threads, hipStream_t s) {
    hipLaunchKernelGGL(fill_kernel, dim3(blocks), dim3(threads), 0, s, p, n, v);
}

int reset_opt_state(dcv_mlp* m, hipStream_t s) {
    const size_t bytes = m->n_params * sizeof(float);
    DCV_CHECK_HIP(hipMemsetAsync(m->adam_m, 0, bytes, s));
    DCV_CHECK_HIP(hipMemsetAsync(m->adam_v, 0, bytes, s));
    if (m->opt_aux) DCV_CHECK_HIP(hipMemsetAsync(m->opt_aux, 0, bytes, s));
    if (m->desc.optimizer == DCV_OPT_ADAGRAD && m->desc.initial_accumulator_value != 0.0) {
        hipLaunchKernelGGL(fill_kernel, dim3(256), dim3(256), 0, s, m->adam_v, m->n_params, (float)m->desc.initial_accumulator_value);
        DCV_CHECK_LAUNCH();
    }
    m->nadam_mu_product = 1.0;
    m->asgd_eta = (double)(float)m->lr;
    m->adam_t = 0;
    m->drop_step = 0;
    return DCV_OK;
}

static int launch_reduce(dcv_mlp* m, const ReduceArgs& ra_all, int l0, int l1, bool fuse_opt, const OptArgs& oa, hipStream_t s) {
    ReduceArgs ra;
    ra.L = 0;
    int max_splits = 0, max_bblocks = 0;
    int64_t max_total = 0;
    auto take = [&](const ReduceDesc& d) {
        ra.l[ra.L++] = d;
        if (d.splits > max_splits) max_splits = d.splits;
        if (d.bblocks > max_bblocks) max_bblocks = d.bblocks;
        if (d.w_count + d.out > max_total) max_total = d.w_count + d.out;
    };
    for (int l = l0; l < l1; ++l) take(ra_all.l[l]);
    for (int l = l0; l < l1; ++l)
        if (m->layers[l].bn) take(ra_all.l[m->L + l]);
    if (ra.L <= 0) return DCV_OK;
    static const bool quad_off = [] { const char* e = getenv("DCV_REDUCE_QUAD"); return e && e[0] == '0'; }();
    if (max_splits <= 512 && max_bblocks <= 1024 && !quad_off) {
        QuadArgs qa;
        qa.n = 0;
        int64_t blocks = 0;
        auto item = [&](const float* src, int64_t dst, int64_t count, int parts, int64_t stride) {
            if (count <= 0) return;
            if (!src || parts < 0) parts = 0;
            QuadItem& q = qa.it[qa.n++];
            q = QuadItem{src, dst, stride, (int)count, parts, (int)blocks, quad_groups(parts)};
            blocks += cdiv(count, 1024 / q.groups);
        };
        for (int l = 0; l < ra.L; ++l) {
            DCV_REQUIRE(ra.l[l].w_count < (1ll << 31), "reduce: layer too large");
            item(ra.l[l].slab, ra.l[l].w_off, ra.l[l].w_count, ra.l[l].splits, rd_wstride(ra.l[l]));
            item(ra.l[l].bpart, ra.l[l].b_off, ra.l[l].out, ra.l[l].bblocks, rd_bstride(ra.l[l]));
        }
        if (blocks <= 0) return DCV_OK;
        DCV_REQUIRE(blocks < (1ll << 31), "reduce: grid out of range");
        hipLaunchKernelGGL(reduce_grads_quad_kernel, dim3((unsigned)blocks), dim3(256), 0, s, qa, m->grads, 1.f, fuse_opt ? 1 : 0, m->params,
                           m->adam_m, m->adam_v, m->opt_aux, oa);
    } else if (max_splits <= 512 && max_bblocks <= 1024) {
        int64_t bx = cdiv(max_total, 64);
        if (bx > 2048) bx = 2048;
        hipLaunchKernelGGL(reduce_grads_small_kernel, dim3((unsigned)bx, ra.L), dim3(256), 0, s, ra, m->grads, 1.f, fuse_opt ? 1 : 0, m->params,
                           m->adam_m, m->adam_v, m->opt_aux, oa);
    } else {
        hipLaunchKernelGGL(reduce_grads_kernel, dim3(512, ra.L), dim3(64 * kRedWaves), 0, s, ra, m->grads, 1.f, fuse_opt ? 1 : 0, m->params, m->adam_m,
                           m->adam_v, m->opt_aux, oa);
    }
    DCV_CHECK_LAUNCH();
    return DCV_OK;
}
int launch_reduce(dcv_mlp* m, const ReduceArgs& ra, int l0, int l1, hipStream_t s) { return launch_reduce(m, ra, l0, l1, false, OptArgs{}, s); }

static OptArgs next_opt_args(dcv_mlp* m) {
    m->adam_t += 1;
    const dcv_mlp_desc& d = m->desc;
    const double t = (double)m->adam_t;
    OptArgs a{};
    a.kind = d.optimizer;
    a.first = m->adam_t == 1;
    a.lr = (float)m->lr;
    a.decay = 1.f;
    a.eps = (float)d.eps;
    a.wd = (float)d.weight_decay;
    a.maximize = d.maximize ? 1 : 0;
    a.img = m->snet_img;
    a.img_idx = m->snet_img_idx;
    switch (d.optimizer) {
        case DCV_OPT_ADAM:
        case DCV_OPT_ADAMW: {
            const double b1 = m->momentum_rt, b2 = d.beta2;
            a.flag = d.amsgrad ? 1 : 0;
            a.b1 = (float)b1;
            a.b2 = (float)b2;
            a.w1 = (float)(1.0 - b1);
            a.w2 = (float)(1.0 - b2);
            a.c1 = (float)(m->lr / (1.0 - pow(b1, t)));
            a.c2 = (float)sqrt(1.0 - pow(b2, t));
            a.decay = (float)(1.0 - m->lr * d.weight_decay);
            break;
        }
        case DCV_OPT_SGD:
            a.flag = d.nesterov ? 1 : 0;
            a.b1 = (float)m->momentum_rt;
            a.w1 = (float)(1.0 - d.dampening);
            break;
        case DCV_OPT_RMSPROP:
            a.flag = d.centered ? 1 : 0;
            a.b1 = (float)m->momentum_rt;
            a.b2 = (float)d.alpha;
            a.w2 = (float)(1.0 - d.alpha);
            break;
        case DCV_OPT_ADAMAX: {
            const double b1 = m->momentum_rt;
            a.b1 = (float)b1;
            a.b2 = (float)d.beta2;
            a.w1 = (float)(1.0 - b1);
            a.c1 = (float)(m->lr / (1.0 - pow(b1, t)));
            break;
        }
        case DCV_OPT_NADAM: {
            const double b1 = m->momentum_rt, b2 = d.beta2, md = d.opt_p[0];
            a.flag = d.opt_p[1] != 0.0 ? 1 : 0;
            a.b1 = (float)b1;
            a.b2 = (float)b2;
            a.w1 = (float)(1.0 - b1);
            a.w2 = (float)(1.0 - b2);
            a.c2 = (float)(1.0 - pow(b2, t));
            a.decay = (float)(1.0 - m->lr * d.weight_decay);
            const double mu = b1 * (1.0 - 0.5 * pow(0.96, t * md));
            const double mu_next = b1 * (1.0 - 0.5 * pow(0.96, (t + 1.0) * md));
            m->nadam_mu_product = (double)(float)((double)(float)m->nadam_mu_product * mu);
            const double mp = m->nadam_mu_product, mp_next = mp * mu_next;
            a.p0 = (float)(-m->lr * (1.0 - mu) / (1.0 - mp));
            a.p1 = (float)((-m->lr * mu_next) / (1.0 - mp_next));
            break;
        }
        case DCV_OPT_RADAM: {
            const double b1 = m->momentum_rt, b2 = d.beta2;
            a.flag = d.opt_p[1] != 0.0 ? 1 : 0;
            a.b1 = (float)b1;
            a.b2 = (float)b2;
            a.w1 = (float)(1.0 - b1);
            a.w2 = (float)(1.0 - b2);
            a.decay = (float)(1.0 - m->lr * d.weight_decay);
            const double bc1 = 1.0 - pow(b1, t), bc2 = 1.0 - pow(b2, t);
            a.c1 = (float)bc1;
            a.c2 = (float)sqrt(bc2);
            const double rho_inf = 2.0 / (1.0 - b2) - 1.0;
            const double rho_t = rho_inf - 2.0 * t * pow(b2, t) / bc2;
            a.p0 = rho_t > 5.0 ? (float)sqrt((rho_t - 4.0) * (rho_t - 2.0) * rho_inf / ((rho_inf - 4.0) * (rho_inf - 2.0) * rho_t)) : 0.f;
            break;
        }
        case DCV_OPT_ADADELTA:
            a.b2 = (float)d.opt_p[0];
            a.w2 = (float)(1.0 - d.opt_p[0]);
            break;
        case DCV_OPT_ASGD: {
            const double eta = m->asgd_eta;
            a.p0 = (float)(1.0 - d.opt_p[0] * eta);
            a.p1 = (float)eta;
            m->asgd_eta = (double)(float)(m->lr / pow(1.0 + d.opt_p[0] * m->lr * t, d.opt_p[1]));
            break;
        }
        case DCV_OPT_RPROP:
            a.p0 = (float)d.opt_p[0];
            a.p1 = (float)d.opt_p[1];
            a.p2 = (float)d.opt_p[2];
            a.p3 = (float)d.opt_p[3];
            break;
        default:
            a.c1 = (float)(m->lr / (1.0 + (t - 1.0) * d.lr_decay));
            break;
    }
    return a;
}

static int first_step_state(dcv_mlp* m, hipStream_t s) {
    if (m->adam_t != 0) return DCV_OK;
    if (m->desc.optimizer == DCV_OPT_RPROP) {
        hipLaunchKernelGGL(fill_kernel, dim3(256), dim3(256), 0, s, m->adam_v, m->n_params, (float)m->lr);
        DCV_CHECK_LAUNCH();
    }
    if (m->desc.optimizer == DCV_OPT_ASGD) m->asgd_eta = (double)(float)m->lr;
    return DCV_OK;
}

ReduceArgs reduce_args_of(const dcv_mlp* m, const ReduceArgsView& v) {
    ReduceArgs ra{};
    ra.L = m->L;
    for (int l = 0; l < m->L; ++l) {
        ReduceDesc& rd = ra.l[l];
        rd = linear_reduce_desc(m->layers[l], v.splits[l], v.bblocks[l]);
        rd.slab = v.slab[l];
        rd.bpart = v.bpart[l];
        rd.w_stride = v.wstride[l];
        rd.b_stride = v.bstride[l];
    }
    return ra;
}
int reduce_upper(dcv_mlp* m, const ReduceArgs& ra, bool fuse_opt, bool* done, hipStream_t s) {
    if (*done || m->L <= 1 || !m->upper_cb || fuse_opt) return DCV_OK;
    const int rc = launch_reduce(m, ra, 1, m->L, s);
    if (rc) return rc;
    *done = true;
    m->upper_cb(m->upper_cb_user);
    return DCV_OK;
}
int finish_grads(dcv_mlp* m, const ReduceArgs& ra, bool fuse_opt, bool upper_done, hipStream_t s) {
    int rc = reduce_upper(m, ra, fuse_opt, &upper_done, s);
    if (rc) return rc;
    OptArgs oa{};
    if (fuse_opt) {
        rc = first_step_state(m, s);
        if (rc) return rc;
        oa = next_opt_args(m);
    }
    return launch_reduce(m, ra, 0, upper_done ? 1 : m->L, fuse_opt, oa, s);
}
int apply_impl(dcv_mlp* m, void* stream) {
    DCV_REQUIRE(m, "dcv_mlp_apply: null");
    hipStream_t s = as_stream(stream);
    const int rcf = first_step_state(m, s);
    if (rcf) return rcf;
    const OptArgs a = next_opt_args(m);
    int64_t blocks = cdiv(m->n_params, 256);
    if (blocks > 1024) blocks = 1024;
    hipLaunchKernelGGL(optimizer_kernel, dim3((unsigned)blocks), dim3(256), 0, s, m->params, (const float*)m->grads, m->adam_m, m->adam_v,
                       m->opt_aux, m->n_params, a);
    DCV_CHECK_LAUNCH();
    return DCV_OK;
}

}
```

### deep_cartograph_amd/csrc/mlp_state.h

```cpp
#pragma once
#include "gemm_kernels.h"
#include <stdlib.h>
#include <vector>

namespace dcv {

constexpr int kMaxTicaDim = 16;

struct EvalGroupWs {
    char* base = nullptr;
    size_t bytes = 0;
    int members = 0, batch = 0;
    int64_t rows = 0;
    bool failed = false;
};

struct LayerPlan {
    int in, out, act;
    int64_t w_off, b_off;
    int64_t ldh;
    float* H;
    int64_t k_chunk_cap;
    int64_t max_splits;
    float* slab;
    float* bpart;
    unsigned long long* mask;
    int64_t mask_rows = -1;
    int bn;
    int64_t g_off = -1, be_off = -1;
    float* Y;
    float *rm, *rv;
    double* bn_stat;
    double* bn_part;
    float *bn_gpart, *bn_bpart;
    int64_t bn_batches;
};

}

struct dcv_mlp {
    dcv_mlp_desc desc;
    int L;
    int d_out;
    int64_t rows_cap;
    int64_t n_params;
    std::vector<dcv::LayerPlan> layers;
    float *params, *grads, *adam_m, *adam_v;
    float* opt_aux;
    double momentum_rt;
    double nadam_mu_product;
    double asgd_eta;
    bool any_drop;
    bool any_bn;
    bool fwd_train;
    dcv::TailWs tail;
    dcv::EvalGroupWs eval_ws;
    int last_eval_group;
    void (*upper_cb)(void*);
    void* upper_cb_user;
    bool head_done;
    int64_t drop_step;
    int64_t cur_step;
    uint32_t drop_rank;
    void* snet;
    bool snet_tried;
    float* snet_img;
    int* snet_img_idx;
    int snet_img_floats;
    void* snet_dt;
    bool snet_dt_tried;
    bool snet_fwd_valid;
    int last_path;
    float* dZ[2];
    int64_t ld_dz;
    double* stats;
    int stats_len;
    double* gradp;
    double* spart;
    int spart_blocks;
    double* log;
    int* log_count;
    unsigned* ticket;
    hipGraphExec_t gexec[4];
    bool gwarm[4];
    bool graph_on;
    bool graph_off;
    int64_t graph_launches;
    bool prof_paused;
    int log_cap, log_width;
    float* feat_range;
    int vae_d;
    float* vae_z;
    int64_t ld_z;
    double* vae_kpart;
    int vae_kblocks;
    double kl_beta;
    const float* noise;
    int64_t noise_rows, noise_pos;
    const float* eps_cur;
    float *ident, *zeros_d, *ones_d;
    float* proj_ws;
    size_t proj_ws_bytes;
    int64_t adam_t;
    double lr;
    int32_t last_batch;
    int no_row_sharing;
    int prof_level, prof_cap;
    int prof_kind_off;
    std::vector<int> prof_cnt;
    std::vector<hipEvent_t> prof_ev;
};


namespace dcv {
struct ReduceArgsView {
    const float* slab[DCV_MAX_LAYERS];
    const float* bpart[DCV_MAX_LAYERS];
    int splits[DCV_MAX_LAYERS];
    int bblocks[DCV_MAX_LAYERS];
    int64_t wstride[DCV_MAX_LAYERS], bstride[DCV_MAX_LAYERS];
};
constexpr int kEvalBatchesPerLaunch = 64;
constexpr size_t kEvalGroupBudgetBytes = 256ull << 20;
constexpr int64_t kEvalWorkgroupsPerLaunch = 4096;
int snet_ae_step(dcv_mlp* m, const float* Xn_d, int64_t ld, const RowMap& rm, int64_t R, int64_t batch, int train, ReduceArgsView* ra,
                 hipStream_t s, bool write_log = true, int nb = 1);
int snet_ae_tile_rows(dcv_mlp* m, int64_t R = 0);
void snet_free(dcv_mlp* m);
int snet_ae_last_tile_rows(const dcv_mlp* m);
bool snet_image_build(dcv_mlp* m);
int snet_image_repack(dcv_mlp* m, hipStream_t s);
void snet_image_free(dcv_mlp* m);
int snet_dt_forward(dcv_mlp* m, const float* Xn_d, int64_t ld, const int64_t* idx_d, int64_t row0, int32_t batch, int head, bool keep_blob,
                    hipStream_t s, int nb = 1);
int snet_dt_backward(dcv_mlp* m, int32_t batch, int64_t global_batch, bool head, ReduceArgsView* ra, hipStream_t s);
void snet_dt_free(dcv_mlp* m);
int snet_dt_last_tile_rows(const dcv_mlp* m);
int bn_forward(dcv_mlp* m, int l, int64_t row0, int64_t rows, bool train, hipStream_t s);
int bn_backward(dcv_mlp* m, int l, float* dz, int64_t ld_dz, int halves, int64_t rows_half, int act, float hscale, const DropCfg& drop,
                int* blocks_out, hipStream_t s);
int bn_eval_backward(dcv_mlp* m, int l, float* dz, int64_t ld_dz, int64_t rows, int act, hipStream_t s);

constexpr int kColsumRows = 32;
constexpr int kSseRows = 16;
constexpr int kStatBlockRows = 128;
constexpr int kVaeRows = 256;

struct ReduceDesc {
    const float* slab;
    const float* bpart;
    int64_t w_off, b_off;
    int64_t w_count;
    int out;
    int splits, bblocks;
    int64_t w_stride, b_stride;
};
struct ReduceArgs {
    ReduceDesc l[2 * DCV_MAX_LAYERS];
    int L;
};
inline ReduceDesc linear_reduce_desc(const LayerPlan& p, int splits, int bblocks) {
    return ReduceDesc{p.slab, p.bpart, p.w_off, p.b_off, (int64_t)p.out * p.in, p.out, splits, bblocks, 0, 0};
}

inline bool prof_on(const dcv_mlp* m, int layer, int kind = -1) {
    if (!(m->prof_level > 0 && !m->prof_paused && (m->prof_level > 1 || layer == 0))) return false;
    if (kind < 0) return true;
    return ((m->prof_kind_off >> kind) & 1) == 0 && m->prof_cnt[(size_t)3 * layer + kind] < m->prof_cap;
}
inline void prof_mark(dcv_mlp* m, int layer, int kind, int which, hipStream_t s) {
    if (!prof_on(m, layer, kind)) return;
    const size_t cls = (size_t)3 * layer + kind;
    hipEvent_t* ev = &m->prof_ev[(cls * m->prof_cap + m->prof_cnt[cls]) * 2];
    if (which == 0) {
        (void)hipEventRecord(ev[0], s);
        if (g_launch_ev.start == nullptr) g_launch_ev = LaunchEvents{ev[0], ev[1]};
    } else {
        m->prof_cnt[cls] += 1;
        if (g_launch_taken == ev[0]) {
            g_launch_taken = nullptr;
            return;
        }
        if (g_launch_ev.start == ev[0]) g_launch_ev = LaunchEvents{};
        (void)hipEventRecord(ev[1], s);
    }
}

inline bool shared_rows(const dcv_mlp* m, const int64_t* idx, int batch) {
    return m->desc.model == DCV_MODEL_DEEPTICA && idx == nullptr && m->desc.lag >= 1 && m->desc.lag <= batch && !m->no_row_sharing &&
           !(m->fwd_train && (m->any_drop || m->any_bn));
}
inline DropCfg drop_cfg(const dcv_mlp* m, int layer) {
    const float p = m->desc.dropout[layer];
    if (!m->fwd_train || !(p > 0.f)) return kNoDrop;
    double t = (double)p * 4294967296.0;
    if (t > 4294967295.0) t = 4294967295.0;
    if (t < 1.0) t = 1.0;
    return DropCfg{(uint32_t)t, 1.f / (1.f - p), (uint32_t)(m->desc.seed & 0xFFFFFFFFull), (uint32_t)(m->desc.seed >> 32) + 0x9E3779B9u * m->drop_rank, (uint32_t)layer,
                   (uint32_t)m->cur_step};
}
inline float drop_hscale(const dcv_mlp* m, int layer) {
    const float p = m->desc.dropout[layer];
    return (m->fwd_train && p > 0.f) ? 1.f - p : 1.f;
}
inline RowMap batch_rows(const dcv_mlp* m, const int64_t* idx, int64_t row0, int batch) {
    if (m->desc.model == DCV_MODEL_DEEPTICA && !shared_rows(m, idx, batch)) return RowMap{idx, row0, batch, m->desc.lag};
    return RowMap{idx, row0, 0, 0};
}
inline int64_t rows_of(const dcv_mlp* m, const int64_t* idx, int batch) {
    if (m->desc.model != DCV_MODEL_DEEPTICA) return batch;
    return shared_rows(m, idx, batch) ? (int64_t)batch + m->desc.lag : 2 * (int64_t)batch;
}
inline int lag_offset(const dcv_mlp* m, const int64_t* idx, int batch) { return shared_rows(m, idx, batch) ? m->desc.lag : batch; }

template <class T>
int dmalloc(T** p, size_t count) {
    *p = nullptr;
    hipError_t e = hipMalloc(reinterpret_cast<void**>(p), (count ? count : 1) * sizeof(T));
    if (e != hipSuccess) {
        set_error("hipMalloc of %zu bytes failed: %s", count * sizeof(T), hipGetErrorString(e));
        return DCV_ENOMEM;
    }
    return DCV_OK;
}

inline bool next_layer_fusable(const dcv_mlp* m, int l) {
    static const bool off = [] { const char* e = getenv("DCV_NO_HEAD_FUSION"); return e && e[0] == '1'; }();
    if (off || l + 1 >= m->L || m->any_bn) return false;
    if (m->desc.dropout[l + 1] > 0.f) return false;
    if (m->vae_d > 0 && l + 1 == m->desc.latent_layer) return false;
    return m->layers[l + 1].out <= 8 && m->layers[l].out <= 128;
}

inline float* layer_out(const dcv_mlp* m, int l) { return m->layers[l].bn ? m->layers[l].Y : m->layers[l].H; }

inline void step_begin(dcv_mlp* m, bool train) {
    m->fwd_train = train;
    if (train) m->cur_step = m->drop_step++;
}
inline void step_done(dcv_mlp* m, int path, int32_t batch, bool head_done) {
    m->head_done = head_done;
    m->last_batch = batch;
    m->last_path = path;
    m->snet_fwd_valid = path == 2 && !head_done;
}

void launch_fill(float* p, int64_t n, float v, int blocks, int threads, hipStream_t s);
int reset_opt_state(dcv_mlp* m, hipStream_t s);
ReduceArgs reduce_args_of(const dcv_mlp* m, const ReduceArgsView& v);
int launch_reduce(dcv_mlp* m, const ReduceArgs& ra, int l0, int l1, hipStream_t s);
int reduce_upper(dcv_mlp* m, const ReduceArgs& ra, bool fuse_opt, bool* done, hipStream_t s);
int finish_grads(dcv_mlp* m, const ReduceArgs& ra, bool fuse_opt, bool upper_done, hipStream_t s);
int apply_impl(dcv_mlp* m, void* stream);
int launch_sum_partials(const double* part, int nblocks, int width, double* out, hipStream_t s);
int stats_rows_per_block(int64_t batch);
int tica_stats(dcv_mlp* m, const float* F, int64_t ldf, int batch, int lag_off, int fuse_head, bool* head_ran, hipStream_t s);
bool tica_stats_groupable(int d);
int tica_stats_group(dcv_mlp* m, const float* F, int64_t ldf, int64_t f_stride, int batch, int lag_off, int blocks, int members, double* part,
                     unsigned* tickets, hipStream_t s);
int loss_record(dcv_mlp* m, int64_t global_batch, bool train, bool head_in_bwd, hipStream_t s);
bool head_fusable(const dcv_mlp* m);
int head_backward(dcv_mlp* m, int64_t R, int batch, int lag_off, float* dZ, int* blocks, hipStream_t s);
int ae_sse(dcv_mlp* m, const float* Y, int64_t ldy, const float* Xn, int64_t ldx, const RowMap& rm, int64_t R, int batch, bool fuse_head, hipStream_t s);
int loss_gradient(dcv_mlp* m, const float* Y, int64_t ldy, const float* Xn, int64_t ldx, const RowMap& rm, int64_t R, int batch, int lag_off,
                  int64_t global_batch, int act, float* dZ, const DropCfg& drop, float hscale, hipStream_t s);
int run_forward(dcv_mlp* m, const float* Xn, int64_t ld, const RowMap& rows_map, int64_t rows, int n_run, hipStream_t s, bool for_backward = false);
bool peek_noise(dcv_mlp* m, int64_t rows);
int forward_impl(dcv_mlp* m, const float* Xn_d, int64_t ld, const int64_t* idx_d, int64_t row0, int32_t batch, int32_t train, void* stream,
                 int fuse_head = 0);
int backward_impl(dcv_mlp* m, const float* Xn_d, int64_t ld, const int64_t* idx_d, int64_t row0, int32_t batch, int64_t global_batch, int32_t train,
                  void* stream, bool fuse_opt = false);
}
```

### deep_cartograph_amd/hip.py

```python
from __future__ import annotations

import os
from typing import Optional, Tuple

import numpy as np
import torch

from . import _lib
from ._lib import FEAT_DISTANCE, FEAT_TORSION, FEAT_TORSION_SINCOS, DcvError, check


def _require_gpu(*tensors):
    for t in tensors:
        if t is not None and not t.is_cuda:
            raise DcvError("deep_cartograph_amd kernels need tensors on an MI355X (cuda) device; got a CPU tensor")


def _ptr(t: Optional[torch.Tensor]):
    return None if t is None else t.data_ptr()


def _stream():
    return torch.cuda.current_stream().cuda_stream


def _ws(nbytes: int, device) -> torch.Tensor:
    return torch.empty(max(int(nbytes), 16), dtype=torch.uint8, device=device)


def _check_matrix(X: torch.Tensor, dtype=torch.float32):
    if X.dim() != 2 or X.dtype != dtype or X.stride(1) != 1:
        raise DcvError(f"expected a row-major 2-D {dtype} tensor, got shape {tuple(X.shape)} dtype {X.dtype} strides {X.stride()}")


def col_stats_raw(X: torch.Tensor) -> torch.Tensor:
    _require_gpu(X)
    _check_matrix(X)
    lib = _lib.load()
    n, F = X.shape
    out = torch.empty(4, F, dtype=torch.float64, device=X.device)
    ws = _ws(lib.dcv_col_stats_workspace(n, F), X.device)
    check(lib.dcv_col_stats(_ptr(X), n, F, X.stride(0), _ptr(out), _ptr(ws), ws.numel(), _stream()), "dcv_col_stats")
    return out


def finalize_stats(raw: torch.Tensor, n: int) -> dict:
    r = raw.detach().cpu().numpy()
    mean = r[0] / n
    var = (r[1] - n * mean * mean) / max(n - 1, 1)
    std = np.sqrt(np.maximum(var, 0.0))
    return {"mean": mean.astype(np.float32), "std": std.astype(np.float32),
            "min": r[2].astype(np.float32), "max": r[3].astype(np.float32)}


def col_histogram(X: torch.Tensor, edges: torch.Tensor) -> torch.Tensor:
    _require_gpu(X, edges)
    _check_matrix(X)
    n, F = X.shape
    if edges.dim() != 2 or edges.shape[0] != F or edges.shape[1] < 2 or edges.dtype != torch.float32 or not edges.is_contiguous():
        raise DcvError(f"col_histogram: edges must be a contiguous float32 [F, bins + 1] tensor, got {tuple(edges.shape)} {edges.dtype}")
    lib = _lib.load()
    bins = edges.shape[1] - 1
    counts = torch.empty(F, bins, dtype=torch.int64, device=X.device)
    ws = _ws(lib.dcv_col_histogram_workspace(n, F, bins), X.device)
    check(lib.dcv_col_histogram(_ptr(X), n, F, X.stride(0), _ptr(edges), bins, _ptr(counts), _ptr(ws), ws.numel(), _stream()),
          "dcv_col_histogram")
    return counts


def dip_sorted_workspace_bytes(n: int, C: int) -> int:
    return int(_lib.load().dcv_dip_sorted_workspace(n, C))


def dip_sorted(Xs: torch.Tensor) -> Tuple[torch.Tensor, torch.Tensor, torch.Tensor]:
    _require_gpu(Xs)
    _check_matrix(Xs)
    n, C = Xs.shape
    if n == 0 or C == 0:
        raise DcvError("dip_sorted: empty matrix")
    if not bool(torch.isfinite(Xs[0]).all() & torch.isfinite(Xs[-1]).all()):
        raise DcvError("dip_sorted: the matrix holds NaN or infinite values")
    lib = _lib.load()
    dip = torch.empty(C, dtype=torch.float64, device=Xs.device)
    lo = torch.empty(C, dtype=torch.int32, device=Xs.device)
    hi = torch.empty(C, dtype=torch.int32, device=Xs.device)
    ws = _ws(lib.dcv_dip_sorted_workspace(n, C), Xs.device)
    check(lib.dcv_dip_sorted(_ptr(Xs), n, C, Xs.stride(0), _ptr(dip), _ptr(lo), _ptr(hi), _ptr(ws), ws.numel(), _stream()),
          "dcv_dip_sorted")
    return dip, lo, hi


_FEAT_COLUMNS = {FEAT_DISTANCE: 1, FEAT_TORSION_SINCOS: 2, FEAT_TORSION: 1}


def featurize(xyz: torch.Tensor, defs, n_atoms: int, strides=None, unit: float = 0.1, out: Optional[torch.Tensor] = None) -> torch.Tensor:
    _require_gpu(xyz, out)
    if xyz.dtype != torch.float32:
        raise DcvError(f"featurize: coordinates must be float32, got {xyz.dtype}")
    defs = np.ascontiguousarray(np.asarray(defs), dtype=np.int32)
    if defs.ndim != 2 or defs.shape[1] != 6 or defs.shape[0] == 0:
        raise DcvError(f"featurize: defs must be a non-empty (n_defs, 6) int32 array, got shape {defs.shape}")
    n_atoms = int(n_atoms)
    if strides is None:
        if xyz.dim() != 3 or xyz.shape[1] != n_atoms or xyz.shape[2] != 3:
            raise DcvError(f"featurize: expected a (n, {n_atoms}, 3) tensor, got {tuple(xyz.shape)}")
        n, offset = xyz.shape[0], 0
        fs, as_, cs = (int(s) for s in xyz.stride())
        base = xyz.data_ptr()
    else:
        n, offset, fs, as_, cs = (int(v) for v in strides)
        if xyz.dim() != 1 or not xyz.is_contiguous():
            raise DcvError("featurize: with explicit strides the coordinates must be a contiguous 1-D buffer")
        last = offset + max(n - 1, 0) * fs + (n_atoms - 1) * as_ + 2 * cs
        if n < 0 or offset < 0 or min(fs, as_, cs) < 0 or (n > 0 and last >= xyz.numel()):
            raise DcvError(f"featurize: layout {tuple(strides)} with {n_atoms} atoms reaches element {last} of a buffer of {xyz.numel()}")
        base = xyz.data_ptr() + 4 * offset
    F = max(int(r[5]) + _FEAT_COLUMNS.get(int(r[0]), 1) for r in defs)
    if out is None:
        out = torch.empty(n, max(F, 1), dtype=torch.float32, device=xyz.device)
    else:
        _check_matrix(out)
        if out.shape[0] != n:
            raise DcvError(f"featurize: out has {out.shape[0]} rows for {n} frames")
        if F > out.shape[1] or int(defs[:, 5].min()) < 0:
            raise DcvError(f"featurize: the records write columns [{int(defs[:, 5].min())}, {F}), out has {out.shape[1]}")
    if n == 0:
        return out
    lib = _lib.load()
    ws = _ws(lib.dcv_featurize_workspace(n, n_atoms, defs.shape[0]), xyz.device)
    ldo = max(out.stride(0), out.shape[1])
    check(lib.dcv_featurize(base, n, fs, as_, cs, n_atoms, defs.ctypes.data, defs.shape[0], float(unit), _ptr(out), ldo,
                            _ptr(ws), ws.numel(), _stream()), "dcv_featurize")
    return out


def normalize(X: torch.Tensor, mean: torch.Tensor, rng: torch.Tensor, out: Optional[torch.Tensor] = None) -> torch.Tensor:
    _require_gpu(X, mean, rng, out)
    _check_matrix(X)
    if out is None:
        out = torch.empty_like(X)
    _check_matrix(out)
    n, F = X.shape
    check(_lib.load().dcv_normalize(_ptr(X), _ptr(out), n, F, X.stride(0), out.stride(0), _ptr(mean), _ptr(rng), _stream()),
          "dcv_normalize")
    return out


def lagged_cov_raw(X: torch.Tensor, n_pairs: int, lag: int, shift: Optional[torch.Tensor] = None) -> torch.Tensor:
    _require_gpu(X, shift)
    _check_matrix(X)
    lib = _lib.load()
    n, F = X.shape
    if n_pairs + lag > n:
        raise DcvError(f"lagged_cov: n_pairs + lag = {n_pairs + lag} exceeds the {n} rows available")
    out = torch.empty(2 * F + 2 * F * F, dtype=torch.float64, device=X.device)
    ws = _ws(lib.dcv_lagged_cov_workspace(n_pairs, F, lag), X.device)
    check(lib.dcv_lagged_cov(_ptr(X), n_pairs, F, X.stride(0), lag, _ptr(shift), _ptr(out), _ptr(ws), ws.numel(), _stream()),
          "dcv_lagged_cov")
    return out


def covariances_from_raw(raw: np.ndarray, n_pairs: int, F: int) -> Tuple[np.ndarray, np.ndarray, np.ndarray]:
    a = raw[:F]
    b = raw[F:2 * F]
    A = raw[2 * F:2 * F + F * F].reshape(F, F)
    B = raw[2 * F + F * F:].reshape(F, F)
    P = float(n_pairs)
    delta = a / P
    C0 = A / P - np.outer(delta, delta)
    Ct = B / P - np.outer(delta, b / P)
    C0 = 0.5 * (C0 + C0.T)
    Ct = 0.5 * (Ct + Ct.T)
    return delta, C0, Ct


def project_linear(X: torch.Tensor, W: torch.Tensor, *, fmean=None, frange=None, bias=None, cvmean=None, cvrange=None,
                   want_out=True, want_minmax=False):
    _require_gpu(X, W, fmean, frange, bias, cvmean, cvrange)
    _check_matrix(X)
    lib = _lib.load()
    n, F = X.shape
    if W.dim() != 2 or W.shape[0] != F or not W.is_contiguous() or W.dtype != torch.float32:
        raise DcvError("project_linear: W must be a contiguous float32 F x d tensor")
    d = W.shape[1]
    out = torch.empty(n, d, dtype=torch.float32, device=X.device) if want_out else None
    mm = torch.empty(2, d, dtype=torch.float32, device=X.device) if want_minmax else None
    ws = _ws(lib.dcv_project_linear_workspace(n, F, d), X.device)
    check(lib.dcv_project_linear(_ptr(X), n, F, X.stride(0), _ptr(fmean), _ptr(frange), _ptr(W), d, _ptr(bias),
                                 _ptr(cvmean), _ptr(cvrange), _ptr(out), _ptr(mm), _ptr(ws), ws.numel(), _stream()),
          "dcv_project_linear")
    return out, mm


def gemm(mode: str, A: torch.Tensor, B: torch.Tensor) -> torch.Tensor:
    _require_gpu(A, B)
    _check_matrix(A)
    _check_matrix(B)
    m = {"nt": 0, "nn": 1, "tn": 2}[mode]
    if m == 0:
        M, K = A.shape
        N = B.shape[0]
    elif m == 1:
        M, K = A.shape
        N = B.shape[1]
    else:
        K, M = A.shape
        N = B.shape[1]
    Cm = torch.empty(M, N, dtype=torch.float32, device=A.device)
    check(_lib.load().dcv_gemm_f32(m, _ptr(A), A.stride(0), _ptr(B), B.stride(0), _ptr(Cm), Cm.stride(0), M, N, K, _stream()),
          "dcv_gemm_f32")
    return Cm


def gemm_tn_split(A: torch.Tensor, B: torch.Tensor, k_chunk: int, slab_cap: int) -> torch.Tensor:
    _require_gpu(A, B)
    _check_matrix(A)
    _check_matrix(B)
    K, M = A.shape
    N = B.shape[1]
    slab = torch.full((slab_cap + 1, M, N), float("nan"), dtype=torch.float32, device=A.device)
    check(_lib.load().dcv_gemm_tn_split(_ptr(A), A.stride(0), _ptr(B), B.stride(0), _ptr(slab), slab_cap, M, N, K, int(k_chunk), _stream()),
          "dcv_gemm_tn_split")
    return slab


def set_gemm_mode(mode: str) -> None:
    lib = _lib.load()
    check(lib.dcv_set_gemm_mode({"native": 0, "split": 1}[mode]), "dcv_set_gemm_mode")


def get_gemm_mode() -> str:
    return "split" if _lib.load().dcv_get_gemm_mode() == 1 else "native"


def kmeans_step(P: torch.Tensor, centers: torch.Tensor, labels: torch.Tensor, offset: Optional[torch.Tensor] = None,
                want_mindist=False):
    _require_gpu(P, centers, labels, offset)
    _check_matrix(P, torch.float64)
    lib = _lib.load()
    n, d = P.shape
    k = centers.shape[0]
    acc = torch.empty(k * d + k + 2, dtype=torch.float64, device=P.device)
    md = torch.empty(n, dtype=torch.float64, device=P.device) if want_mindist else None
    ws = _ws(lib.dcv_kmeans_workspace(n, d, k), P.device)
    check(lib.dcv_kmeans_step(_ptr(P), n, d, _ptr(offset), _ptr(centers), k, _ptr(labels), _ptr(acc), _ptr(md), _ptr(ws), ws.numel(), _stream()),
          "dcv_kmeans_step")
    return acc, md


def kmeanspp_update(P: torch.Tensor, centre: torch.Tensor, closest: torch.Tensor, first: bool, offset: Optional[torch.Tensor] = None) -> torch.Tensor:
    _require_gpu(P, centre, closest, offset)
    _check_matrix(P, torch.float64)
    lib = _lib.load()
    n, d = P.shape
    if n == 0:
        return torch.zeros(1, dtype=torch.float64, device=P.device)
    pot = torch.empty(1, dtype=torch.float64, device=P.device)
    ws = _ws(lib.dcv_kmeanspp_workspace(n, 1), P.device)
    check(lib.dcv_kmeanspp_update(_ptr(P), n, d, _ptr(offset), _ptr(centre), 1 if first else 0, _ptr(closest), _ptr(pot), _ptr(ws), ws.numel(),
                                  _stream()), "dcv_kmeanspp_update")
    return pot


def kmeanspp_potentials(P: torch.Tensor, cand: torch.Tensor, closest: torch.Tensor, offset: Optional[torch.Tensor] = None) -> torch.Tensor:
    _require_gpu(P, cand, closest, offset)
    _check_matrix(P, torch.float64)
    lib = _lib.load()
    n, d = P.shape
    t = cand.shape[0]
    if n == 0:
        return torch.zeros(t, dtype=torch.float64, device=P.device)
    pot = torch.empty(t, dtype=torch.float64, device=P.device)
    ws = _ws(lib.dcv_kmeanspp_workspace(n, t), P.device)
    check(lib.dcv_kmeanspp_potentials(_ptr(P), n, d, _ptr(offset), _ptr(cand.contiguous()), t, _ptr(closest), _ptr(pot), _ptr(ws), ws.numel(),
                                      _stream()), "dcv_kmeanspp_potentials")
    return pot


def label_stats(P: torch.Tensor, labels: torch.Tensor, k: int, centers: Optional[torch.Tensor] = None) -> torch.Tensor:
    _require_gpu(P, labels, centers)
    _check_matrix(P, torch.float64)
    lib = _lib.load()
    n, d = P.shape
    acc = torch.empty(k * d + 3 * k, dtype=torch.float64, device=P.device)
    ws = _ws(lib.dcv_label_stats_workspace(n, d, k), P.device)
    check(lib.dcv_label_stats(_ptr(P), n, d, _ptr(labels), _ptr(centers), k, _ptr(acc), _ptr(ws), ws.numel(), _stream()), "dcv_label_stats")
    return acc


def cluster_dist_sums(Q: torch.Tensor, P_sorted: torch.Tensor, start: torch.Tensor) -> torch.Tensor:
    _require_gpu(Q, P_sorted, start)
    _check_matrix(Q, torch.float64)
    _check_matrix(P_sorted, torch.float64)
    lib = _lib.load()
    nq, d = Q.shape
    k = start.numel() - 1
    S = torch.empty(nq, k, dtype=torch.float64, device=Q.device)
    check(lib.dcv_cluster_dist_sums(_ptr(Q), nq, _ptr(P_sorted), _ptr(start), k, d, _ptr(S), _stream()), "dcv_cluster_dist_sums")
    return S


def silhouette_sum(S: torch.Tensor, qlabels: torch.Tensor, start: torch.Tensor) -> torch.Tensor:
    _require_gpu(S, qlabels, start)
    lib = _lib.load()
    nq, k = S.shape
    out = torch.empty(1, dtype=torch.float64, device=S.device)
    ws = _ws(lib.dcv_silhouette_sum_workspace(nq), S.device)
    check(lib.dcv_silhouette_sum(_ptr(S), nq, k, _ptr(qlabels), _ptr(start), _ptr(out), _ptr(ws), ws.numel(), _stream()), "dcv_silhouette_sum")
    return out


def linear_binning(P: torch.Tensor, cols, lo, hi, bins: int):
    import ctypes as C

    _require_gpu(P)
    _check_matrix(P, torch.float64)
    lib = _lib.load()
    d = len(cols)
    cols_a = (C.c_int32 * d)(*[int(c) for c in cols])
    lo_a = (C.c_double * d)(*[float(v) for v in lo])
    hi_a = (C.c_double * d)(*[float(v) for v in hi])
    grid = torch.empty((bins,) * d, dtype=torch.float64, device=P.device)
    ws = _ws(lib.dcv_linear_binning_workspace(d, bins), P.device)
    out = C.c_int64(0)
    check(lib.dcv_linear_binning(_ptr(P), P.shape[0], P.stride(0), d, cols_a, lo_a, hi_a, int(bins), _ptr(grid), C.byref(out), _ptr(ws),
                                 ws.numel(), _stream()), "dcv_linear_binning")
    return grid, int(out.value)


def nearest_rows(P: torch.Tensor, centers: torch.Tensor, row_offset: int = 0):
    _require_gpu(P, centers)
    _check_matrix(P, torch.float64)
    lib = _lib.load()
    n, d = P.shape
    k = centers.shape[0]
    dist = torch.empty(k, dtype=torch.float64, device=P.device)
    rows = torch.empty(k, dtype=torch.int64, device=P.device)
    ws = _ws(lib.dcv_nearest_rows_workspace(n, d, k), P.device)
    check(lib.dcv_nearest_rows(_ptr(P), n, d, _ptr(centers), k, row_offset, _ptr(dist), _ptr(rows), _ptr(ws), ws.numel(), _stream()),
          "dcv_nearest_rows")
    return dist, rows


def nearest_point(train: torch.Tensor, sup: torch.Tensor) -> torch.Tensor:
    _require_gpu(train, sup)
    _check_matrix(train, torch.float64)
    _check_matrix(sup, torch.float64)
    nn = torch.empty(sup.shape[0], dtype=torch.int64, device=sup.device)
    check(_lib.load().dcv_nearest_point(_ptr(train.contiguous()), train.shape[0], _ptr(sup.contiguous()), sup.shape[0],
                                        train.shape[1], _ptr(nn), _stream()), "dcv_nearest_point")
    return nn


LINKAGE_METHOD = {"complete": 0, "average": 1, "ward": 2}


def linkage_workspace_bytes(n: int, d: int) -> int:
    return int(_lib.load().dcv_linkage_workspace(n, d))


def linkage(P: torch.Tensor, method: str = "complete", return_searches: bool = False):
    _require_gpu(P)
    _check_matrix(P, torch.float64)
    if method not in LINKAGE_METHOD:
        raise DcvError(f"linkage: method {method!r} is not one of {sorted(LINKAGE_METHOD)}")
    P = P.contiguous()
    n, d = P.shape
    if n > 0 and not bool(torch.isfinite(P).all()):
        raise DcvError("linkage failed (code -1): the points hold NaN or infinite values")
    import ctypes as C

    lib = _lib.load()
    Z = np.empty((max(n - 1, 0), 4), dtype=np.float64)
    searches = C.c_int64(0)
    nbytes = lib.dcv_linkage_workspace(n, d)
    ws = _ws(nbytes, P.device) if nbytes else None
    check(lib.dcv_linkage(_ptr(P), n, d, LINKAGE_METHOD[method], Z.ctypes.data, C.byref(searches), _ptr(ws), nbytes, _stream()),
          "dcv_linkage")
    return (Z, int(searches.value)) if return_searches else Z


CORE_MAX_K = 64


def _check_points(P: torch.Tensor, what: str):
    _require_gpu(P)
    _check_matrix(P, torch.float64)
    n, d = P.shape
    if not (2 <= n < 2 ** 31) or not (1 <= d <= 16):
        raise DcvError(f"{what} failed (code -1): {n} points in {d} dimensions, supported n >= 2, 1 <= d <= 16")
    if not bool(torch.isfinite(P).all()):
        raise DcvError(f"{what} failed (code -1): the points hold NaN or infinite values")


def core_distances_workspace_bytes(n: int, d: int, k: int) -> int:
    return int(_lib.load().dcv_core_distances_workspace(n, d, k))


def core_distances(P: torch.Tensor, k: int) -> torch.Tensor:
    _check_points(P, "core_distances")
    P = P.contiguous()
    n, d = P.shape
    k = int(k)
    if not (1 <= k <= min(n, CORE_MAX_K)):
        raise DcvError(f"core_distances failed (code -1): k = {k}, supported 1..min(n, {CORE_MAX_K})")
    lib = _lib.load()
    core = torch.empty(n, dtype=torch.float64, device=P.device)
    nbytes = lib.dcv_core_distances_workspace(n, d, k)
    ws = _ws(nbytes, P.device)
    check(lib.dcv_core_distances(_ptr(P), n, d, k, _ptr(core), _ptr(ws), nbytes, _stream()), "dcv_core_distances")
    return core


def mr_mst_workspace_bytes(n: int, d: int) -> int:
    return int(_lib.load().dcv_mr_mst_workspace(n, d))


def mr_mst(P: torch.Tensor, core: torch.Tensor) -> Tuple[np.ndarray, np.ndarray, np.ndarray]:
    _check_points(P, "mr_mst")
    _require_gpu(core)
    P = P.contiguous()
    n, d = P.shape
    if core.dtype != torch.float64 or core.dim() != 1 or core.shape[0] != n:
        raise DcvError(f"mr_mst failed (code -1): expected {n} float64 core distances, got shape {tuple(core.shape)} dtype {core.dtype}")
    core = core.contiguous()
    if not bool(torch.isfinite(core).all()):
        raise DcvError("mr_mst failed (code -1): the core distances hold NaN or infinite values")
    lib = _lib.load()
    src = np.empty(n - 1, dtype=np.int64)
    dst = np.empty(n - 1, dtype=np.int64)
    w = np.empty(n - 1, dtype=np.float64)
    nbytes = lib.dcv_mr_mst_workspace(n, d)
    ws = _ws(nbytes, P.device)
    check(lib.dcv_mr_mst(_ptr(P), n, d, _ptr(core), src.ctypes.data, dst.ctypes.data, w.ctypes.data, _ptr(ws), nbytes, _stream()),
          "dcv_mr_mst")
    return src, dst, w


class RcclComm:

    def __init__(self, dist=None, device="cuda"):
        import ctypes as C

        self.lib = _lib.load()
        world = dist.get_world_size() if dist is not None else 1
        rank = dist.get_rank() if dist is not None else 0
        uid = (C.c_uint8 * 128)()
        if rank == 0:
            check(self.lib.dcv_comm_unique_id(uid), "dcv_comm_unique_id")
        if world > 1:
            backend = dist.get_backend()
            t = torch.tensor(list(uid), dtype=torch.uint8, device=device if backend == "nccl" else "cpu")
            dist.broadcast(t, src=0)
            uid = (C.c_uint8 * 128)(*t.cpu().tolist())
        h = C.c_void_p()
        check(self.lib.dcv_comm_create(world, rank, uid, C.byref(h)), "dcv_comm_create")
        self.h, self.world, self.rank = h, world, rank

    def all_reduce(self, t: torch.Tensor, op: str = "sum"):
        _require_gpu(t)
        dt = {torch.float32: 0, torch.float64: 1}[t.dtype]
        check(self.lib.dcv_comm_allreduce(self.h, _ptr(t), t.numel(), dt, {"sum": 0, "min": 1, "max": 2}[op], _stream()), "dcv_comm_allreduce")

    def close(self):
        if getattr(self, "h", None):
            self.lib.dcv_comm_destroy(self.h)
            self.h = None

    def __del__(self):
        try:
            self.close()
        except Exception:
            pass


class Mlp:

    def __init__(self, model: str, dims, acts, *, max_batch: int, lag: int = 0, tica_reg: float = 1e-6,
                 latent_layer: Optional[int] = None, lr: float = 1e-3, betas=(0.9, 0.999), eps: Optional[float] = None,
                 weight_decay: float = 0.0, optimizer: str = "Adam", amsgrad: bool = False, momentum: float = 0.0,
                 dampening: float = 0.0, nesterov: bool = False, alpha: float = 0.99, centered: bool = False,
                 lr_decay: float = 0.0, initial_accumulator_value: float = 0.0, opt_params=None, dropout=None, seed: int = 0,
                 batchnorm=None, bn_eps: float = 1e-5, bn_momentum: float = 0.1, maximize: bool = False, device="cuda"):
        import ctypes as C

        if not torch.cuda.is_available():
            raise DcvError("the MLP engine needs an MI355X: torch.cuda.is_available() is False and there is no CPU path")
        self.lib = _lib.load()
        self.device = torch.device(device)
        self.model = model
        self.dims = [int(x) for x in dims]
        self.acts = list(acts)
        L = len(self.dims) - 1
        if len(self.acts) != L:
            raise DcvError("one activation per Linear layer expected")
        desc = _lib.MlpDesc()
        desc.model = {"deep_tica": _lib.MODEL_DEEPTICA, "ae": _lib.MODEL_AE, "vae": _lib.MODEL_VAE}[model]
        desc.n_layers = L
        for i, v in enumerate(self.dims):
            desc.dims[i] = v
        for i, a in enumerate(self.acts):
            if a not in _lib.ACT:
                raise DcvError(f"activation {a!r} is not implemented by the HIP engine")
            desc.act[i] = _lib.ACT[a]
        desc.latent_layer = L if latent_layer is None else int(latent_layer)
        desc.lag = int(lag)
        desc.max_batch = int(max_batch)
        desc.tica_reg = float(tica_reg)
        if eps is None:
            eps = {"Adagrad": 1e-10, "Adadelta": 1e-6}.get(optimizer, 1e-8)
        desc.lr, desc.beta1, desc.beta2, desc.eps, desc.weight_decay = float(lr), float(betas[0]), float(betas[1]), float(eps), float(weight_decay)
        if optimizer not in _lib.OPTIMIZER:
            raise DcvError(f"optimizer {optimizer!r} is not implemented by the HIP engine (have: {sorted(_lib.OPTIMIZER)})")
        desc.optimizer = _lib.OPTIMIZER[optimizer]
        desc.amsgrad, desc.nesterov, desc.centered = int(bool(amsgrad)), int(bool(nesterov)), int(bool(centered))
        desc.momentum, desc.dampening, desc.alpha = float(momentum), float(dampening), float(alpha)
        desc.lr_decay, desc.initial_accumulator_value = float(lr_decay), float(initial_accumulator_value)
        for i, v in enumerate(list(opt_params or [])[:4]):
            desc.opt_p[i] = float(v)
        self.batchnorm = [bool(b) for b in (batchnorm if batchnorm is not None else [False] * L)]
        if len(self.batchnorm) != L:
            raise DcvError("one batchnorm flag per Linear layer expected")
        for i, b in enumerate(self.batchnorm):
            desc.batchnorm[i] = 1 if b else 0
        desc.bn_eps, desc.bn_momentum = float(bn_eps), float(bn_momentum)
        desc.maximize = 1 if maximize else 0
        self.dropout = [float(p or 0.0) for p in (dropout if dropout is not None else [0.0] * L)]
        if len(self.dropout) != L:
            raise DcvError("one dropout probability per Linear layer expected")
        for i, p in enumerate(self.dropout):
            desc.dropout[i] = p
        desc.seed = int(seed) & 0xFFFFFFFFFFFFFFFF
        h = C.c_void_p()
        check(self.lib.dcv_mlp_create(C.byref(desc), C.byref(h)), "dcv_mlp_create")
        self.h = h
        self.L = L
        self.latent_layer = desc.latent_layer
        self.in_dims = [self.dims[l] // 2 if model == "vae" and l == self.latent_layer else self.dims[l] for l in range(L)]
        self.max_batch = int(max_batch)
        self.rows_cap = 2 * self.max_batch if model == "deep_tica" else self.max_batch
        self.n_params = self.lib.dcv_mlp_num_params(self.h)
        self.offsets = [(self.lib.dcv_mlp_param_offset(self.h, l, 0), self.lib.dcv_mlp_param_offset(self.h, l, 1)) for l in range(L)]
        self.bn_offsets = [(self.lib.dcv_mlp_param_offset(self.h, l, 2), self.lib.dcv_mlp_param_offset(self.h, l, 3)) for l in range(L)]
        self.log_width = self.lib.dcv_mlp_log_width(self.h)
        self.stats_len = self.lib.dcv_mlp_stats_len(self.h)
        self._log_cap = 0
        self._dp = None
        self._upper_thunk = None
        self._upper_fn = None
        self._upper_err = None
        self._noise = None

    def close(self):
        if getattr(self, "h", None):
            self.lib.dcv_mlp_destroy(self.h)
            self.h = None

    def __del__(self):
        try:
            self.close()
        except Exception:
            pass

    def set_linears(self, linears, bn=None):
        flat = np.zeros(self.n_params, dtype=np.float32)
        for l in range(self.L):
            if self.batchnorm[l]:
                go, bo_ = self.bn_offsets[l]
                d = (bn[l] if bn is not None else None) or {}
                flat[go: go + self.dims[l + 1]] = np.asarray(d.get("weight", np.ones(self.dims[l + 1])), dtype=np.float32)
                flat[bo_: bo_ + self.dims[l + 1]] = np.asarray(d.get("bias", np.zeros(self.dims[l + 1])), dtype=np.float32)
        for l, (w, b) in enumerate(linears):
            w = np.asarray(w, dtype=np.float32)
            b = np.asarray(b, dtype=np.float32)
            if w.shape != (self.dims[l + 1], self.in_dims[l]) or b.shape != (self.dims[l + 1],):
                raise DcvError(f"layer {l}: expected weight {(self.dims[l + 1], self.in_dims[l])}, got {w.shape}")
            wo, bo = self.offsets[l]
            flat[wo: wo + w.size] = w.ravel()
            flat[bo: bo + b.size] = b
        check(self.lib.dcv_mlp_set_params(self.h, flat.ctypes.data, _stream()), "dcv_mlp_set_params")
        if bn is not None:
            import ctypes as C

            for l in range(self.L):
                if self.batchnorm[l] and bn[l] is not None and "running_mean" in bn[l]:
                    rm = np.ascontiguousarray(np.asarray(bn[l]["running_mean"], dtype=np.float32))
                    rv = np.ascontiguousarray(np.asarray(bn[l]["running_var"], dtype=np.float32))
                    nbt = C.c_int64(int(bn[l].get("num_batches_tracked", 0)))
                    check(self.lib.dcv_mlp_bn_state(self.h, l, rm.ctypes.data, rv.ctypes.data, C.byref(nbt), 1, _stream()), "dcv_mlp_bn_state")

    def get_bn(self):
        import ctypes as C

        flat = np.empty(self.n_params, dtype=np.float32)
        check(self.lib.dcv_mlp_get_params(self.h, flat.ctypes.data, _stream()), "dcv_mlp_get_params")
        out = []
        for l in range(self.L):
            if not self.batchnorm[l]:
                out.append(None)
                continue
            o = self.dims[l + 1]
            go, bo_ = self.bn_offsets[l]
            rm, rv, nbt = np.empty(o, np.float32), np.empty(o, np.float32), C.c_int64(0)
            check(self.lib.dcv_mlp_bn_state(self.h, l, rm.ctypes.data, rv.ctypes.data, C.byref(nbt), 0, _stream()), "dcv_mlp_bn_state")
            out.append({"weight": flat[go: go + o].copy(), "bias": flat[bo_: bo_ + o].copy(), "running_mean": rm, "running_var": rv,
                        "num_batches_tracked": int(nbt.value)})
        return out

    def get_linears(self):
        flat = np.empty(self.n_params, dtype=np.float32)
        check(self.lib.dcv_mlp_get_params(self.h, flat.ctypes.data, _stream()), "dcv_mlp_get_params")
        out = []
        for l in range(self.L):
            wo, bo = self.offsets[l]
            o, i = self.dims[l + 1], self.in_dims[l]
            out.append((flat[wo: wo + o * i].reshape(o, i).copy(), flat[bo: bo + o].copy()))
        return out

    def _flat_view(self, ptr, n, dtype):
        import ctypes as C

        class _Holder:
            pass

        itemsize = torch.tensor([], dtype=dtype).element_size()
        holder = _Holder()
        holder.__cuda_array_interface__ = {
            "shape": (n,), "typestr": {torch.float32: "<f4", torch.float64: "<f8"}[dtype],
            "data": (int(ptr), False), "version": 2, "strides": (itemsize,)}
        return torch.as_tensor(holder, device=self.device)

    def grads_view(self) -> torch.Tensor:
        return self._flat_view(self.lib.dcv_mlp_grads(self.h), self.n_params, torch.float32)

    def params_view(self) -> torch.Tensor:
        return self._flat_view(self.lib.dcv_mlp_params(self.h), self.n_params, torch.float32)

    def stats_view(self) -> torch.Tensor:
        return self._flat_view(self.lib.dcv_mlp_stats(self.h), self.stats_len, torch.float64)

    def set_lr(self, lr: float):
        check(self.lib.dcv_mlp_set_lr(self.h, float(lr)), "dcv_mlp_set_lr")

    def set_momentum(self, value: float):
        check(self.lib.dcv_mlp_set_momentum(self.h, float(value)), "dcv_mlp_set_momentum")

    def last_path(self) -> int:
        return int(self.lib.dcv_mlp_last_path(self.h))

    def dropout_step(self) -> int:
        return int(self.lib.dcv_mlp_dropout_step(self.h))

    def dropout_mask(self, layer: int, step: int, rows: int) -> torch.Tensor:
        out = torch.empty(rows, self.dims[layer + 1], dtype=torch.float32, device=self.device)
        check(self.lib.dcv_mlp_dropout_mask(self.h, int(layer), int(step), int(rows), _ptr(out), _stream()), "dcv_mlp_dropout_mask")
        return out

    def set_row_sharing(self, enable: bool):
        check(self.lib.dcv_mlp_set_row_sharing(self.h, 1 if enable else 0), "dcv_mlp_set_row_sharing")

    def set_feature_range(self, rng):
        r = np.ascontiguousarray(np.asarray(rng, dtype=np.float32))
        check(self.lib.dcv_mlp_set_feature_range(self.h, r.ctypes.data, _stream()), "dcv_mlp_set_feature_range")

    def set_kl_beta(self, beta: float):
        check(self.lib.dcv_mlp_set_kl_beta(self.h, float(beta)), "dcv_mlp_set_kl_beta")

    def set_noise(self, eps: torch.Tensor):
        _require_gpu(eps)
        eps = eps.to(torch.float32).contiguous()
        d = self.dims[self.latent_layer] // 2
        if eps.dim() != 2 or eps.shape[1] != d:
            raise DcvError(f"set_noise: expected a [rows, {d}] tensor, got {tuple(eps.shape)}")
        self._noise = eps
        check(self.lib.dcv_mlp_set_noise(self.h, _ptr(eps), int(eps.shape[0])), "dcv_mlp_set_noise")

    def noise_position(self) -> int:
        return int(self.lib.dcv_mlp_noise_position(self.h))

    def latent_sample(self, rows: int) -> torch.Tensor:
        out = torch.empty(int(rows), self.dims[self.latent_layer] // 2, dtype=torch.float32, device=self.device)
        check(self.lib.dcv_mlp_latent_sample(self.h, int(rows), _ptr(out), _stream()), "dcv_mlp_latent_sample")
        return out

    def _args(self, Xn, idx, row0, batch):
        _require_gpu(Xn, idx)
        _check_matrix(Xn)
        if idx is not None and (idx.dtype != torch.int64 or not idx.is_contiguous()):
            raise DcvError("batch indices must be a contiguous int64 device tensor")
        return _ptr(Xn), Xn.stride(0), _ptr(idx), int(row0), int(batch)

    def forward(self, Xn, idx=None, row0=0, batch=None, train=True):
        batch = int(batch if batch is not None else idx.numel())
        check(self.lib.dcv_mlp_forward(self.h, *self._args(Xn, idx, row0, batch), 1 if train else 0, _stream()), "dcv_mlp_forward")

    def backward(self, Xn, idx=None, row0=0, batch=None, global_batch=None, train=True, on_upper_grads=None):
        import ctypes as C

        batch = int(batch if batch is not None else idx.numel())
        gb = int(global_batch if global_batch is not None else batch)
        use_cb = on_upper_grads is not None and train and self.L > 1
        if use_cb:
            if self._upper_thunk is None:

                def _tramp(_u):
                    try:
                        self._upper_fn()
                    except BaseException as e:
                        self._upper_err = e

                self._upper_thunk = C.CFUNCTYPE(None, C.c_void_p)(_tramp)
            self._upper_fn, self._upper_err = on_upper_grads, None
            check(self.lib.dcv_mlp_set_upper_grads_callback(self.h, C.cast(self._upper_thunk, C.c_void_p), None), "dcv_mlp_set_upper_grads_callback")
        try:
            check(self.lib.dcv_mlp_backward(self.h, *self._args(Xn, idx, row0, batch), gb, 1 if train else 0, _stream()), "dcv_mlp_backward")
        finally:
            if use_cb:
                check(self.lib.dcv_mlp_set_upper_grads_callback(self.h, None, None), "dcv_mlp_set_upper_grads_callback")
                self._upper_fn = None
        if use_cb and self._upper_err is not None:
            e, self._upper_err = self._upper_err, None
            raise e

    def upper_grads_view(self) -> torch.Tensor:
        return self.grads_view()[self.offsets[1][0]:] if self.L > 1 else self.grads_view()[:0]

    def layer0_grads_view(self) -> torch.Tensor:
        return self.grads_view()[: self.offsets[1][0]] if self.L > 1 else self.grads_view()

    def data_parallel_step(self, Xn, dist, global_batch, idx=None, row0=0, batch=None, train=True, group=None):
        import ctypes as C

        rows = int(batch if batch is not None else idx.numel())
        if isinstance(dist, RcclComm):
            env = os.environ.get("DCV_DP_OVERLAP")
            overlap = (rows >= 32768) if env is None else env == "1"
            check(self.lib.dcv_comm_bind_stream(dist.h, _stream()), "dcv_comm_bind_stream")
            check(self.lib.dcv_mlp_dp_step(self.h, *self._args(Xn, idx, row0, rows), int(global_batch), 1 if train else 0, 1 if overlap else 0,
                                           self.lib.dcv_comm_dp_allreduce_fn(), dist.h, _stream()), "dcv_mlp_dp_step")
            return
        env = os.environ.get("DCV_DP_OVERLAP")
        overlap = (rows >= 32768) if env is None else env == "1"
        st = self._dp
        if st is None:
            st = self._dp = {"views": {}, "pending": [], "error": None, "dist": None, "group": None}

            def _cb(_user, buf, count, dtype, phase):
                try:
                    if phase == 3:
                        for w in st["pending"]:
                            w.wait()
                        st["pending"].clear()
                        return 0
                    key = (int(buf), int(count), int(dtype))
                    t = st["views"].get(key)
                    if t is None:
                        t = st["views"][key] = self._flat_view(buf, int(count), torch.float64 if dtype == 1 else torch.float32)
                    d = st["dist"]
                    if phase == 2:
                        st["pending"].append(d.all_reduce(t, op=d.ReduceOp.SUM, group=st["group"], async_op=True))
                    else:
                        d.all_reduce(t, op=d.ReduceOp.SUM, group=st["group"])
                    return 0
                except BaseException as e:
                    st["error"] = e
                    return 1

            st["thunk"] = C.CFUNCTYPE(C.c_int, C.c_void_p, C.c_void_p, C.c_int64, C.c_int32, C.c_int32)(_cb)
        st["dist"], st["group"], st["error"] = dist, group, None
        st["pending"].clear()
        rc = self.lib.dcv_mlp_dp_step(self.h, *self._args(Xn, idx, row0, rows), int(global_batch), 1 if train else 0, 1 if overlap else 0,
                                      C.cast(st["thunk"], C.c_void_p), None, _stream())
        if st["error"] is not None:
            err, st["error"] = st["error"], None
            raise err
        check(rc, "dcv_mlp_dp_step")

    def set_rank(self, rank: int):
        check(self.lib.dcv_mlp_set_rank(self.h, int(rank)), "dcv_mlp_set_rank")

    def layer_output(self, layer: int, rows: int) -> torch.Tensor:
        out = torch.empty(int(rows), self.dims[layer + 1], dtype=torch.float32, device=self.device)
        check(self.lib.dcv_mlp_layer_output(self.h, int(layer), int(rows), _ptr(out), _stream()), "dcv_mlp_layer_output")
        return out

    def apply(self):
        check(self.lib.dcv_mlp_apply(self.h, _stream()), "dcv_mlp_apply")

    def set_graph(self, enable: bool):
        check(self.lib.dcv_mlp_set_graph(self.h, 1 if enable else 0), "dcv_mlp_set_graph")

    def graph_launches(self) -> int:
        return int(self.lib.dcv_mlp_graph_launches(self.h))

    def train_step(self, Xn, idx=None, row0=0, batch=None):
        batch = int(batch if batch is not None else idx.numel())
        check(self.lib.dcv_mlp_train_step(self.h, *self._args(Xn, idx, row0, batch), _stream()), "dcv_mlp_train_step")

    def eval_step(self, Xn, idx=None, row0=0, batch=None):
        batch = int(batch if batch is not None else idx.numel())
        check(self.lib.dcv_mlp_eval_step(self.h, *self._args(Xn, idx, row0, batch), _stream()), "dcv_mlp_eval_step")

    def train_steps(self, Xn, batch: int, nsteps: int, idx=None, row0=0):
        batch, nsteps = int(batch), int(nsteps)
        if idx is not None and idx.numel() < batch * nsteps:
            raise DcvError(f"train_steps: {idx.numel()} indices for {nsteps} batches of {batch}")
        if idx is None and int(row0) + batch * nsteps > Xn.shape[0]:
            raise DcvError(f"train_steps: rows {row0} + {nsteps} x {batch} exceed the matrix ({Xn.shape[0]} rows)")
        check(self.lib.dcv_mlp_train_steps(self.h, *self._args(Xn, idx, row0, batch), nsteps, _stream()), "dcv_mlp_train_steps")

    def eval_steps(self, Xn, batch: int, nbatches: int, idx=None, row0=0):
        batch, nbatches = int(batch), int(nbatches)
        if idx is not None and idx.numel() < batch * nbatches:
            raise DcvError(f"eval_steps: {idx.numel()} indices for {nbatches} batches of {batch}")
        if idx is None and int(row0) + batch * nbatches > Xn.shape[0]:
            raise DcvError(f"eval_steps: rows {row0} + {nbatches} x {batch} exceed the matrix ({Xn.shape[0]} rows)")
        check(self.lib.dcv_mlp_eval_steps(self.h, *self._args(Xn, idx, row0, batch), nbatches, _stream()), "dcv_mlp_eval_steps")

    def reset_log(self, capacity: int):
        check(self.lib.dcv_mlp_reset_log(self.h, int(capacity), _stream()), "dcv_mlp_reset_log")
        self._log_cap = max(self._log_cap, int(capacity))

    def read_log(self) -> np.ndarray:
        import ctypes as C

        out = np.empty((max(self._log_cap, 1), self.log_width), dtype=np.float64)
        n = C.c_int32(0)
        check(self.lib.dcv_mlp_read_log(self.h, out.ctypes.data, out.shape[0], C.byref(n), _stream()), "dcv_mlp_read_log")
        return out[: n.value].copy()

    def profile_begin(self, max_steps: int, level: int = 1):
        check(self.lib.dcv_mlp_profile_begin(self.h, int(max_steps), int(level)), "dcv_mlp_profile_begin")

    def profile_pause(self, paused: bool, skip_kinds=()):
        code = 1 if paused else 0
        for k in skip_kinds:
            code |= 2 << ("fwd", "wgrad", "dgrad").index(k)
        check(self.lib.dcv_mlp_profile_pause(self.h, code), "dcv_mlp_profile_pause")

    def profile_end(self):
        ms = np.zeros(3 * self.L, dtype=np.float64)
        cnt = np.zeros(3 * self.L, dtype=np.int32)
        check(self.lib.dcv_mlp_profile_end(self.h, ms.ctypes.data, cnt.ctypes.data), "dcv_mlp_profile_end")
        kinds = ("fwd", "wgrad", "dgrad")
        return {(c // 3, kinds[c % 3]): (float(ms[c]), int(cnt[c])) for c in range(3 * self.L) if cnt[c] > 0}

    def input_sensitivity(self, Xn, gout, scale):
        _require_gpu(Xn, gout, scale)
        _check_matrix(Xn)
        n, F = Xn.shape
        total = torch.zeros(F, dtype=torch.float64, device=Xn.device)
        part = torch.empty(F, dtype=torch.float64, device=Xn.device)
        cap = min(self.rows_cap, max(1, n))
        nbytes = self.lib.dcv_mlp_input_sensitivity_workspace(self.h, cap)
        ws = torch.empty(nbytes, dtype=torch.uint8, device=Xn.device)
        gout = gout.to(torch.float32).contiguous()
        scale = scale.to(torch.float32).contiguous()
        for s in range(0, n, cap):
            e = min(n, s + cap)
            check(self.lib.dcv_mlp_input_sensitivity(self.h, _ptr(Xn[s:e]), e - s, Xn.stride(0), _ptr(gout), _ptr(scale), _ptr(part),
                                                     _ptr(ws), ws.numel(), _stream()), "dcv_mlp_input_sensitivity")
            total += part
        return total

    def infer(self, Xn, *, tmean=None, tevecs=None, pmean=None, prange=None, want_out=True, want_minmax=False):
        _require_gpu(Xn, tmean, tevecs, pmean, prange)
        _check_matrix(Xn)
        n = Xn.shape[0]
        d = self.dims[self.latent_layer] // (2 if self.model == "vae" else 1)
        out = torch.empty(n, d, dtype=torch.float32, device=Xn.device) if want_out else None
        mm = None
        for s in range(0, n, self.rows_cap):
            e = min(n, s + self.rows_cap)
            chunk = Xn[s:e]
            mmc = torch.empty(2, d, dtype=torch.float32, device=Xn.device) if want_minmax else None
            check(self.lib.dcv_mlp_infer(self.h, _ptr(chunk), e - s, Xn.stride(0), _ptr(tmean), _ptr(tevecs), _ptr(pmean), _ptr(prange),
                                         _ptr(out[s:e]) if want_out else None, _ptr(mmc), _stream()), "dcv_mlp_infer")
            if want_minmax:
                if mm is None:
                    mm = mmc
                else:
                    mm = torch.stack([torch.minimum(mm[0], mmc[0]), torch.maximum(mm[1], mmc[1])])
        return out, mm
```

### include/dcv.h

```cpp
#ifndef DCV_H
#define DCV_H

#include <stddef.h>
#include <stdint.h>

#ifdef __cplusplus
extern "C" {
#endif

#define DCV_OK 0
#define DCV_EINVAL (-1)
#define DCV_EHIP (-2)
#define DCV_ENOMEM (-3)
#define DCV_ESTATE (-4)
#define DCV_ECALLBACK (-5)

#define DCV_ABI_VERSION 5

int dcv_abi_version(void);
const char* dcv_last_error(void);
int dcv_device_info(int device, int* n_cu, int64_t* hbm_bytes, char* name, size_t name_len);

#define DCV_GEMM_NATIVE_F32 0
#define DCV_GEMM_SPLIT_BF16X6 1
int dcv_set_gemm_mode(int mode);
int dcv_get_gemm_mode(void);

size_t dcv_col_stats_workspace(int64_t n, int32_t F);
int dcv_col_stats(const float* X_d, int64_t n, int32_t F, int64_t ld, double* out_d,
                  void* ws_d, size_t ws_bytes, void* stream);

size_t dcv_col_histogram_workspace(int64_t n, int32_t F, int32_t bins);
int dcv_col_histogram(const float* X_d, int64_t n, int32_t F, int64_t ld, const float* edges_d, int32_t bins,
                      int64_t* counts_d, void* ws_d, size_t ws_bytes, void* stream);

size_t dcv_dip_sorted_workspace(int64_t n, int32_t C);
int dcv_dip_sorted(const float* Xs_d, int64_t n, int32_t C, int64_t ld, double* dip_d, int32_t* lo_d,
                   int32_t* hi_d, void* ws_d, size_t ws_bytes, void* stream);

#define DCV_FEAT_DISTANCE 0
#define DCV_FEAT_TORSION_SINCOS 1
#define DCV_FEAT_TORSION 2
size_t dcv_featurize_workspace(int64_t n_frames, int32_t n_atoms, int32_t n_defs);
int dcv_featurize(const float* xyz_d, int64_t n_frames, int64_t frame_stride, int64_t atom_stride, int64_t comp_stride,
                  int32_t n_atoms, const int32_t* defs_h, int32_t n_defs, double unit,
                  float* out_d, int64_t ldo, void* ws_d, size_t ws_bytes, void* stream);

int dcv_normalize(const float* X_d, float* Y_d, int64_t n, int32_t F, int64_t ldx, int64_t ldy,
                  const float* mean_d, const float* range_d, void* stream);

size_t dcv_lagged_cov_workspace(int64_t n_pairs, int32_t F, int32_t lag);
int dcv_lagged_cov(const float* X_d, int64_t n_pairs, int32_t F, int64_t ld, int32_t lag,
                   const float* shift_d, double* out_d, void* ws_d, size_t ws_bytes, void* stream);

size_t dcv_project_linear_workspace(int64_t n, int32_t F, int32_t d);
int dcv_project_linear(const float* X_d, int64_t n, int32_t F, int64_t ld,
                       const float* fmean_d, const float* frange_d, const float* W_d, int32_t d,
                       const float* bias_d, const float* cvmean_d, const float* cvrange_d,
                       float* out_d, float* minmax_d, void* ws_d, size_t ws_bytes, void* stream);

#define DCV_ACT_NONE 0
#define DCV_ACT_LEAKY_RELU 1
#define DCV_ACT_RELU 2
#define DCV_ACT_TANH 3
#define DCV_ACT_ELU 4
#define DCV_ACT_SOFTPLUS 5
#define DCV_ACT_SHIFTED_SOFTPLUS 6
#define DCV_ACT_CUSTOM_SIGMOID 7
#define DCV_MAX_LAYERS 16

#define DCV_OPT_ADAM 0
#define DCV_OPT_ADAMW 1
#define DCV_OPT_SGD 2
#define DCV_OPT_RMSPROP 3
#define DCV_OPT_ADAGRAD 4
#define DCV_OPT_ADAMAX 5
#define DCV_OPT_NADAM 6
#define DCV_OPT_RADAM 7
#define DCV_OPT_ADADELTA 8
#define DCV_OPT_ASGD 9
#define DCV_OPT_RPROP 10

#define DCV_MODEL_DEEPTICA 1
#define DCV_MODEL_AE 2
#define DCV_MODEL_VAE 3

typedef struct dcv_mlp_desc {
    int32_t model;
    int32_t n_layers;
    int32_t dims[DCV_MAX_LAYERS + 1];
    int32_t act[DCV_MAX_LAYERS];
    int32_t latent_layer;
    int32_t lag;
    int32_t max_batch;
    double tica_reg;
    double lr, beta1, beta2, eps, weight_decay;
    int32_t optimizer;
    int32_t amsgrad;
    int32_t nesterov;
    int32_t centered;
    double momentum, dampening;
    double alpha;
    double lr_decay, initial_accumulator_value;
    double opt_p[4];
    float dropout[DCV_MAX_LAYERS];
    uint64_t seed;
    int32_t batchnorm[DCV_MAX_LAYERS];
    double bn_eps, bn_momentum;
    int32_t maximize;
} dcv_mlp_desc;

typedef struct dcv_mlp dcv_mlp;

int dcv_mlp_create(const dcv_mlp_desc* desc, dcv_mlp** out);
void dcv_mlp_destroy(dcv_mlp* m);
int64_t dcv_mlp_num_params(const dcv_mlp* m);
int64_t dcv_mlp_param_offset(const dcv_mlp* m, int32_t layer, int32_t which);
float* dcv_mlp_params(dcv_mlp* m);
float* dcv_mlp_grads(dcv_mlp* m);
int dcv_mlp_set_params(dcv_mlp* m, const float* params_h, void* stream);
int dcv_mlp_get_params(dcv_mlp* m, float* params_h, void* stream);
int dcv_mlp_set_lr(dcv_mlp* m, double lr);
int dcv_mlp_set_momentum(dcv_mlp* m, double value);
int dcv_mlp_set_row_sharing(dcv_mlp* m, int32_t enable);
int dcv_mlp_set_feature_range(dcv_mlp* m, const float* range_h, void* stream);
int dcv_mlp_set_kl_beta(dcv_mlp* m, double beta);
int dcv_mlp_set_noise(dcv_mlp* m, const float* eps_d, int64_t rows);
int64_t dcv_mlp_noise_position(const dcv_mlp* m);
int dcv_mlp_latent_sample(dcv_mlp* m, int64_t rows, float* out_d, void* stream);

int dcv_mlp_forward(dcv_mlp* m, const float* Xn_d, int64_t ld, const int64_t* idx_d, int64_t row0,
                    int32_t batch, int32_t train, void* stream);
double* dcv_mlp_stats(dcv_mlp* m);
int32_t dcv_mlp_stats_len(const dcv_mlp* m);
int dcv_mlp_backward(dcv_mlp* m, const float* Xn_d, int64_t ld, const int64_t* idx_d, int64_t row0,
                     int32_t batch, int64_t global_batch, int32_t train, void* stream);
int dcv_mlp_apply(dcv_mlp* m, void* stream);
int dcv_mlp_set_upper_grads_callback(dcv_mlp* m, void (*fn)(void* user), void* user);
#define DCV_DTYPE_F32 0
#define DCV_DTYPE_F64 1
#define DCV_DP_STATS 0
#define DCV_DP_GRADS 1
#define DCV_DP_UPPER_START 2
#define DCV_DP_WAIT 3
typedef int (*dcv_allreduce_fn)(void* user, void* buf_d, int64_t count, int32_t dtype, int32_t phase);
int dcv_mlp_dp_step(dcv_mlp* m, const float* Xn_d, int64_t ld, const int64_t* idx_d, int64_t row0, int32_t batch,
                    int64_t global_batch, int32_t train, int32_t overlap, dcv_allreduce_fn fn, void* user, void* stream);
typedef struct dcv_comm dcv_comm;
int dcv_comm_unique_id(void* id_out_128);
int dcv_comm_create(int32_t world, int32_t rank, const void* id_128, dcv_comm** out);
void dcv_comm_destroy(dcv_comm* c);
int dcv_comm_bind_stream(dcv_comm* c, void* stream);
int dcv_comm_allreduce(dcv_comm* c, void* buf_d, int64_t count, int32_t dtype, int32_t op, void* stream);
dcv_allreduce_fn dcv_comm_dp_allreduce_fn(void);
int32_t dcv_comm_world(const dcv_comm* c);
int32_t dcv_comm_rank(const dcv_comm* c);
int dcv_mlp_set_rank(dcv_mlp* m, int32_t rank);
int dcv_mlp_bn_state(dcv_mlp* m, int32_t layer, float* running_mean_h, float* running_var_h, int64_t* num_batches_tracked,
                     int32_t set, void* stream);
int32_t dcv_mlp_last_path(const dcv_mlp* m);
int32_t dcv_mlp_last_eval_group(const dcv_mlp* m);
int dcv_mlp_layer_output(dcv_mlp* m, int32_t layer, int64_t rows, float* out_d, void* stream);
int dcv_mlp_train_step(dcv_mlp* m, const float* Xn_d, int64_t ld, const int64_t* idx_d, int64_t row0,
                       int32_t batch, void* stream);
int dcv_mlp_eval_step(dcv_mlp* m, const float* Xn_d, int64_t ld, const int64_t* idx_d, int64_t row0,
                      int32_t batch, void* stream);
int dcv_mlp_train_steps(dcv_mlp* m, const float* Xn_d, int64_t ld, const int64_t* idx_d, int64_t row0,
                        int32_t batch, int32_t nsteps, void* stream);
int dcv_mlp_eval_steps(dcv_mlp* m, const float* Xn_d, int64_t ld, const int64_t* idx_d, int64_t row0,
                       int32_t batch, int32_t nbatches, void* stream);

int dcv_mlp_dropout_mask(dcv_mlp* m, int32_t layer, int64_t step, int64_t rows, float* out_d, void* stream);
int64_t dcv_mlp_dropout_step(const dcv_mlp* m);

int32_t dcv_mlp_log_width(const dcv_mlp* m);
int dcv_mlp_reset_log(dcv_mlp* m, int32_t capacity, void* stream);
int dcv_mlp_read_log(dcv_mlp* m, double* out_h, int32_t max_records, int32_t* n_records, void* stream);

int dcv_mlp_profile_begin(dcv_mlp* m, int32_t max_steps, int32_t level);
int dcv_mlp_profile_end(dcv_mlp* m, double* ms_h, int32_t* counts_h);
int dcv_mlp_profile_pause(dcv_mlp* m, int32_t paused);

int64_t dcv_mlp_graph_launches(const dcv_mlp* m);
int dcv_mlp_set_graph(dcv_mlp* m, int32_t enable);

int dcv_mlp_infer(dcv_mlp* m, const float* Xn_d, int64_t n, int64_t ld,
                  const float* tmean_d, const float* tevecs_d, const float* pmean_d,
                  const float* prange_d, float* out_d, float* minmax_d, void* stream);

size_t dcv_mlp_input_sensitivity_workspace(const dcv_mlp* m, int64_t n);
int dcv_mlp_input_sensitivity(dcv_mlp* m, const float* Xn_d, int64_t n, int64_t ld, const float* gout_d,
                              const float* scale_d, double* sens_d, void* ws_d, size_t ws_bytes, void* stream);

size_t dcv_kmeans_workspace(int64_t n, int32_t d, int32_t k);
int dcv_kmeans_step(const double* P_d, int64_t n, int32_t d, const double* offset_d ,
                    const double* centers_d, int32_t k, int32_t* labels_d, double* acc_d, double* mindist_d ,
                    void* ws_d, size_t ws_bytes, void* stream);

size_t dcv_kmeanspp_workspace(int64_t n, int32_t trials);
int dcv_kmeanspp_potentials(const double* P_d, int64_t n, int32_t d, const double* offset_d, const double* cand_d, int32_t trials,
                            const double* closest_d, double* pot_d, void* ws_d, size_t ws_bytes, void* stream);
int dcv_kmeanspp_update(const double* P_d, int64_t n, int32_t d, const double* offset_d, const double* centre_d, int32_t first,
                        double* closest_d, double* pot_d, void* ws_d, size_t ws_bytes, void* stream);

size_t dcv_label_stats_workspace(int64_t n, int32_t d, int32_t k);
int dcv_label_stats(const double* P_d, int64_t n, int32_t d, const int32_t* labels_d, const double* centers_d ,
                    int32_t k, double* acc_d, void* ws_d, size_t ws_bytes, void* stream);
int dcv_cluster_dist_sums(const double* Q_d, int64_t nq, const double* Psorted_d, const int64_t* start_d, int32_t k, int32_t d,
                          double* S_d , void* stream);
size_t dcv_silhouette_sum_workspace(int64_t nq);
int dcv_silhouette_sum(const double* S_d, int64_t nq, int32_t k, const int32_t* qlabels_d, const int64_t* start_d,
                       double* sum_d, void* ws_d, size_t ws_bytes, void* stream);

size_t dcv_linear_binning_workspace(int32_t d, int32_t bins);
int dcv_linear_binning(const double* P_d, int64_t n, int64_t ldp, int32_t d, const int32_t* cols_h, const double* lo_h,
                       const double* hi_h, int32_t bins, double* grid_d, int64_t* outside_h, void* ws_d, size_t ws_bytes, void* stream);

size_t dcv_nearest_rows_workspace(int64_t n, int32_t d, int32_t k);
int dcv_nearest_rows(const double* P_d, int64_t n, int32_t d, const double* centers_d, int32_t k,
                     int64_t row_offset, double* dist_d, int64_t* rows_d,
                     void* ws_d, size_t ws_bytes, void* stream);

int dcv_nearest_point(const double* train_d, int64_t n_train, const double* sup_d, int64_t n_sup,
                      int32_t d, int64_t* nn_d, void* stream);

size_t dcv_linkage_workspace(int64_t n, int32_t d);
int dcv_linkage_pdist(const double* P_d, int64_t n, int32_t d, void* ws_d, size_t ws_bytes, void* stream);
int dcv_linkage(const double* P_d, int64_t n, int32_t d, int32_t method, double* Z_h, int64_t* searches_h,
                void* ws_d, size_t ws_bytes, void* stream);

size_t dcv_core_distances_workspace(int64_t n, int32_t d, int32_t k);
int dcv_core_distances(const double* P_d, int64_t n, int32_t d, int32_t k, double* core_d, void* ws_d,
                       size_t ws_bytes, void* stream);
size_t dcv_mr_mst_workspace(int64_t n, int32_t d);
int dcv_mr_mst(const double* P_d, int64_t n, int32_t d, const double* core_d, int64_t* src_h, int64_t* dst_h,
               double* w_h, void* ws_d, size_t ws_bytes, void* stream);

int dcv_gemm_f32(int32_t mode, const float* A_d, int64_t lda, const float* B_d, int64_t ldb, float* C_d,
                 int64_t ldc, int64_t M, int64_t N, int64_t K, void* stream);
int dcv_gemm_tn_split(const float* A_d, int64_t lda, const float* B_d, int64_t ldb, float* slab_d, int64_t slab_cap,
                      int64_t M, int64_t N, int64_t K, int64_t k_chunk, void* stream);

#ifdef __cplusplus
}
#endif
#endif
```

Before: 82.53 million.

## Fuse upper-layer gradient reduction and optimizer into layer-0 wgrad GEMM launch

Adds a combined kernel in which extra blocks, appended to the grid of the first-layer weight-gradient GEMM, perform the quad split-reduction and fused optimizer update for the upper layers. The upper layers' reduce and update then run concurrently with the largest wgrad GEMM instead of in a separate serial launch afterward, which removes a kernel boundary and fills idle CUs. Optimizer helpers and quad-reduce structs move into a shared header, and accessors for the ride flag and optimizer state are added. In exchange, LDS and occupancy are shared between GEMM and reduction blocks, and the combined path only applies to ungathered, vector-aligned operands with specific tile configs.

```diff
diff --git a/deep_cartograph_amd/_lib.py b/deep_cartograph_amd/_lib.py
--- a/deep_cartograph_amd/_lib.py
+++ b/deep_cartograph_amd/_lib.py
@@ -89,6 +89,8 @@
     "dcv_mlp_dropout_step": (_I64, [_P]),
     "dcv_mlp_last_path": (_I32, [_P]),
     "dcv_mlp_last_eval_group": (_I32, [_P]),
+    "dcv_mlp_last_ride": (_I32, [_P]),
+    "dcv_mlp_opt_state": (_P, [_P, _I32]),
     "dcv_gemm_tn_split": (C.c_int, [_P, _I64, _P, _I64, _P, _I64, _I64, _I64, _I64, _I64, _P]),
     "dcv_mlp_set_row_sharing": (C.c_int, [_P, _I32]),
     "dcv_mlp_set_feature_range": (C.c_int, [_P, _P, _P]),
diff --git a/deep_cartograph_amd/csrc/mlp.hip b/deep_cartograph_amd/csrc/mlp.hip
--- a/deep_cartograph_amd/csrc/mlp.hip
+++ b/deep_cartograph_amd/csrc/mlp.hip
@@ -1,4 +1,5 @@
 #include "mlp_state.h"
+#include "reduce_quad.h"
 #include <new>
 #include <math.h>
 #include <utility>
@@ -428,6 +429,11 @@
 extern "C" int64_t dcv_mlp_dropout_step(const dcv_mlp* m) { return m ? m->drop_step : 0; }
 extern "C" int32_t dcv_mlp_last_path(const dcv_mlp* m) { return m ? m->last_path : -1; }
 extern "C" int32_t dcv_mlp_last_eval_group(const dcv_mlp* m) { return m ? m->last_eval_group : -1; }
+extern "C" int32_t dcv_mlp_last_ride(const dcv_mlp* m) { return m ? m->last_ride : -1; }
+extern "C" float* dcv_mlp_opt_state(dcv_mlp* m, int32_t which) {
+    if (!m) return nullptr;
+    return which == 0 ? m->adam_m : which == 1 ? m->adam_v : which == 2 ? m->opt_aux : nullptr;
+}
 
 extern "C" int dcv_mlp_dropout_mask(dcv_mlp* m, int32_t layer, int64_t step, int64_t rows, float* out_d, void* stream) {
     DCV_REQUIRE(m && out_d && layer >= 0 && layer < m->L && rows >= 1 && step >= 0, "dcv_mlp_dropout_mask: bad arguments");
@@ -718,6 +724,9 @@
     float *dz_cur, *dz_nxt;
     int bblocks;
     ReduceArgs ra;
+    bool fuse_opt = false;
+    bool ridden = false;
+    OptArgs oa{};
 };
 
 static int backward_blob(dcv_mlp* m, int32_t batch, int64_t global_batch, bool head_in_bwd, bool fuse_opt, hipStream_t s) {
@@ -823,7 +832,20 @@
     const LayerPlan& p = m->layers[l];
     const int64_t R = c.R;
     const int64_t kc = plan_wgrad(c, l);
-    if (l == 0) return wgrad_alone(c, l, make_operand(c.Xn, c.ld, p.in, c.rm), kc);
+    if (l == 0) {
+        const Operand X = make_operand(c.Xn, c.ld, p.in, c.rm);
+        if (c.fuse_opt) {
+            prof_mark(m, l, 1, 0, s);
+            const int rc = ride_upper(m, c.ra, make_operand(c.dz_cur, m->ld_dz, p.out), X, p.out, p.in, R, kc, slab_epi(p), &c.oa, s);
+            if (rc < 0) return rc;
+            if (rc == DCV_OK) {
+                prof_mark(m, l, 1, 1, s);
+                c.ridden = true;
+                return DCV_OK;
+            }
+        }
+        return wgrad_alone(c, l, X, kc);
+    }
     const LayerPlan& q = m->layers[l - 1];
     Operand A = make_operand(c.dz_cur, m->ld_dz, p.out);
     Operand B = make_operand(layer_out(m, l - 1), q.ldh, p.in);
@@ -881,10 +903,12 @@
     const bool head_in_bwd = tica && m->last_path == 2 && train && !m->head_done && m->snet_fwd_valid;
     int rc = loss_record(m, global_batch, train != 0, head_in_bwd, s);
     if (rc || !train) return rc;
+    m->last_ride = 0;
     if (tica && m->last_path == 2) return backward_blob(m, batch, global_batch, head_in_bwd, fuse_opt, s);
     const int L = m->L;
     Backward c{m, Xn_d, ld, idx_d, batch_rows(m, idx_d, row0, batch), rows_of(m, idx_d, batch), batch, global_batch, s, m->dZ[0], m->dZ[1], 0, ReduceArgs{}};
     c.ra.L = L;
+    c.fuse_opt = fuse_opt;
     const bool fused_head = tica && head_fusable(m);
     rc = seed_gradient(c, fused_head);
     bool upper_done = false;
@@ -897,7 +921,7 @@
         else rc = backward_layer(c, l);
     }
     if (rc) return rc;
-    return finish_grads(m, c.ra, fuse_opt, upper_done, s);
+    return finish_grads(m, c.ra, fuse_opt, upper_done, s, c.ridden ? &c.oa : nullptr);
 }
 
 static int snet_step(dcv_mlp* m, const float* Xn_d, int64_t ld, const int64_t* idx_d, int64_t row0, int32_t batch, int32_t train, void* stream) {
diff --git a/deep_cartograph_amd/csrc/mlp_opt.hip b/deep_cartograph_amd/csrc/mlp_opt.hip
--- a/deep_cartograph_amd/csrc/mlp_opt.hip
+++ b/deep_cartograph_amd/csrc/mlp_opt.hip
@@ -1,4 +1,5 @@
 #include "mlp_state.h"
+#include "reduce_quad.h"
 #include <math.h>
 
 namespace dcv {
@@ -6,166 +7,6 @@
 static inline int64_t rd_wstride(const ReduceDesc& d) { return d.w_stride > 0 ? d.w_stride : d.w_count; }
 static inline int64_t rd_bstride(const ReduceDesc& d) { return d.b_stride > 0 ? d.b_stride : (int64_t)d.out; }
 
-struct OptArgs {
-    int kind, flag;
-    int first;
-    float lr, b1, b2, eps, wd;
-    float c1, c2;
-    float w1, w2;
-    float decay;
-    float p0, p1, p2, p3;
-    int maximize;
-    float* img;
-    const int* img_idx;
-};
-template <bool WT>
-__device__ __forceinline__ void opt_st(float* p, float v) {
-    if constexpr (WT) handoff_store(p, v);
-    else *p = v;
-}
-template <bool WT>
-__device__ __forceinline__ void opt_stp(const OptArgs& a, float* p, int64_t i, float v) {
-    opt_st<WT>(p + i, v);
-    if (a.img != nullptr) {
-        const int j = a.img_idx[i];
-        if (j >= 0) opt_st<WT>(a.img + j, v);
-    }
-}
-template <bool WT = false>
-__device__ __forceinline__ void opt_update_p(int64_t i, float gi, float pi, float* __restrict__ p, float* __restrict__ s1, float* __restrict__ s2,
-                                             float* __restrict__ s3, const OptArgs& a) {
-    if (a.maximize) gi = -gi;
-    switch (a.kind) {
-        case DCV_OPT_ADAM:
-        case DCV_OPT_ADAMW: {
-            if (a.kind == DCV_OPT_ADAMW) pi = pi * a.decay;
-            else if (a.wd != 0.f) gi = fmaf(a.wd, pi, gi);
-            float mi = s1[i], vi = s2[i];
-            mi = mi + (gi - mi) * a.w1;
-            vi = vi * a.b2 + a.w2 * gi * gi;
-            float vden = vi;
-            if (a.flag) {
-                vden = fmaxf(s3[i], vi);
-                opt_st<WT>(s3 + i, vden);
-            }
-            const float denom = sqrtf(vden) / a.c2 + a.eps;
-            opt_st<WT>(s1 + i, mi);
-            opt_st<WT>(s2 + i, vi);
-            opt_stp<WT>(a, p, i, pi - a.c1 * (mi / denom));
-            break;
-        }
-        case DCV_OPT_SGD: {
-            if (a.wd != 0.f) gi = fmaf(a.wd, pi, gi);
-            if (a.b1 != 0.f) {
-                float bi = a.first ? gi : s1[i] * a.b1 + a.w1 * gi;
-                opt_st<WT>(s1 + i, bi);
-                gi = a.flag ? fmaf(a.b1, bi, gi) : bi;
-            }
-            opt_stp<WT>(a, p, i, pi - a.lr * gi);
-            break;
-        }
-        case DCV_OPT_RMSPROP: {
-            if (a.wd != 0.f) gi = fmaf(a.wd, pi, gi);
-            float sq = s2[i] * a.b2 + a.w2 * gi * gi;
-            opt_st<WT>(s2 + i, sq);
-            float avg;
-            if (a.flag) {
-                float ga = s3[i];
-                ga = ga + (gi - ga) * a.w2;
-                opt_st<WT>(s3 + i, ga);
-                avg = sqrtf(sq - ga * ga) + a.eps;
-            } else {
-                avg = sqrtf(sq) + a.eps;
-            }
-            if (a.b1 > 0.f) {
-                const float bi = s1[i] * a.b1 + gi / avg;
-                opt_st<WT>(s1 + i, bi);
-                opt_stp<WT>(a, p, i, pi - a.lr * bi);
-            } else {
-                opt_stp<WT>(a, p, i, pi - a.lr * (gi / avg));
-            }
-            break;
-        }
-        case DCV_OPT_ADAMAX: {
-            if (a.wd != 0.f) gi = fmaf(a.wd, pi, gi);
-            float mi = s1[i];
-            mi = mi + (gi - mi) * a.w1;
-            const float ui = fmaxf(s2[i] * a.b2, fabsf(gi) + a.eps);
-            opt_st<WT>(s1 + i, mi);
-            opt_st<WT>(s2 + i, ui);
-            opt_stp<WT>(a, p, i, pi - a.c1 * (mi / ui));
-            break;
-        }
-        case DCV_OPT_NADAM: {
-            if (a.wd != 0.f) {
-                if (a.flag) pi = pi * a.decay;
-                else gi = fmaf(a.wd, pi, gi);
-            }
-            float mi = s1[i], vi = s2[i];
-            mi = mi + (gi - mi) * a.w1;
-            vi = vi * a.b2 + a.w2 * gi * gi;
-            const float denom = sqrtf(vi / a.c2) + a.eps;
-            opt_st<WT>(s1 + i, mi);
-            opt_st<WT>(s2 + i, vi);
-            pi = pi + a.p0 * (gi / denom);
-            opt_stp<WT>(a, p, i, pi + a.p1 * (mi / denom));
-            break;
-        }
-        case DCV_OPT_RADAM: {
-            if (a.wd != 0.f) {
-                if (a.flag) pi = pi * a.decay;
-                else gi = fmaf(a.wd, pi, gi);
-            }
-            float mi = s1[i], vi = s2[i];
-            mi = mi + (gi - mi) * a.w1;
-            vi = vi * a.b2 + a.w2 * gi * gi;
-            opt_st<WT>(s1 + i, mi);
-            opt_st<WT>(s2 + i, vi);
-            const float mhat = mi / a.c1;
-            if (a.p0 > 0.f) opt_stp<WT>(a, p, i, pi - ((mhat * a.lr) * (a.c2 / (sqrtf(vi) + a.eps))) * a.p0);
-            else opt_stp<WT>(a, p, i, pi - mhat * a.lr);
-            break;
-        }
-        case DCV_OPT_ADADELTA: {
-            if (a.wd != 0.f) gi = fmaf(a.wd, pi, gi);
-            const float sq = s1[i] * a.b2 + a.w2 * gi * gi;
-            const float acc = s2[i];
-            const float delta = sqrtf(acc + a.eps) / sqrtf(sq + a.eps) * gi;
-            opt_st<WT>(s1 + i, sq);
-            opt_st<WT>(s2 + i, acc * a.b2 + a.w2 * delta * delta);
-            opt_stp<WT>(a, p, i, pi - a.lr * delta);
-            break;
-        }
-        case DCV_OPT_ASGD: {
-            if (a.wd != 0.f) gi = fmaf(a.wd, pi, gi);
-            pi = pi * a.p0;
-            opt_stp<WT>(a, p, i, pi - a.p1 * gi);
-            break;
-        }
-        case DCV_OPT_RPROP: {
-            const float sg = gi * s1[i];
-            const float f = sg > 0.f ? a.p1 : (sg < 0.f ? a.p0 : 1.f);
-            const float st = fminf(fmaxf(s2[i] * f, a.p2), a.p3);
-            opt_st<WT>(s2 + i, st);
-            if (sg < 0.f) gi = 0.f;
-            const float sgn = gi > 0.f ? 1.f : (gi < 0.f ? -1.f : 0.f);
-            opt_stp<WT>(a, p, i, pi - sgn * st);
-            opt_st<WT>(s1 + i, gi);
-            break;
-        }
-        default: {
-            if (a.wd != 0.f) gi = fmaf(a.wd, pi, gi);
-            const float su = s2[i] + gi * gi;
-            opt_st<WT>(s2 + i, su);
-            opt_stp<WT>(a, p, i, pi - a.c1 * (gi / (sqrtf(su) + a.eps)));
-            break;
-        }
-    }
-}
-__device__ __forceinline__ void opt_update(int64_t i, float gi, float* __restrict__ p, float* __restrict__ s1, float* __restrict__ s2,
-                                           float* __restrict__ s3, const OptArgs& a) {
-    opt_update_p(i, gi, p[i], p, s1, s2, s3, a);
-}
 __global__ __launch_bounds__(256) void optimizer_kernel(float* __restrict__ p, const float* __restrict__ g, float* __restrict__ s1,
                                                         float* __restrict__ s2, float* __restrict__ s3, int64_t n, OptArgs a) {
     for (int64_t i = (int64_t)blockIdx.x * 256 + threadIdx.x; i < n; i += (int64_t)gridDim.x * 256) opt_update(i, g[i], p, s1, s2, s3, a);
@@ -239,64 +80,6 @@
     }
 }
 
-struct QuadItem {
-    const float* src;
-    int64_t dst;
-    int64_t stride;
-    int count, parts;
-    int blk0;
-    int groups;
-};
-struct QuadArgs {
-    QuadItem it[4 * DCV_MAX_LAYERS];
-    int n;
-};
-inline int quad_groups(int parts) { return parts > 32 ? 16 : 4; }
-template <int G>
-__device__ __forceinline__ void reduce_quad_block(const QuadItem& d, int blk, float* __restrict__ grads, float scale, int fuse,
-                                                  float* __restrict__ params, float* __restrict__ s1, float* __restrict__ s2,
-                                                  float* __restrict__ s3, const OptArgs& oa, double* s_red) {
-    constexpr int EPB = 1024 / G, TPG = EPB / 4;
-    const int t = threadIdx.x, g = t / TPG, sub = t % TPG;
-    const int base = blk * EPB;
-    const int mine = base + t;
-    const bool fin = t < EPB && mine < d.count;
-    float pi = 0.f;
-    if (fuse && fin) pi = params[d.dst + mine];
-    const int e0 = base + 4 * sub;
-    double acc[4] = {0.0, 0.0, 0.0, 0.0};
-    if (e0 < d.count && (d.stride & 3) == 0 && e0 + 4 <= d.stride && (reinterpret_cast<uintptr_t>(d.src) & 15) == 0) {
-        const float* p = d.src + e0;
-#pragma unroll 8
-        for (int q = g; q < d.parts; q += G) {
-            const float4 v = *reinterpret_cast<const float4*>(p + (int64_t)q * d.stride);
-            acc[0] += (double)v.x;
-            acc[1] += (double)v.y;
-            acc[2] += (double)v.z;
-            acc[3] += (double)v.w;
-        }
-    } else if (e0 < d.count) {
-        const float* p = d.src + e0;
-        const int nv = d.count - e0 < 4 ? d.count - e0 : 4;
-#pragma unroll 4
-        for (int q = g; q < d.parts; q += G) {
-#pragma unroll
-            for (int j = 0; j < 4; ++j)
-                if (j < nv) acc[j] += (double)p[(int64_t)q * d.stride + j];
-        }
-    }
-#pragma unroll
-    for (int j = 0; j < 4; ++j) s_red[g * EPB + 4 * sub + j] = acc[j];
-    __syncthreads();
-    if (fin) {
-        double tot = s_red[t];
-#pragma unroll
-        for (int k = 1; k < G; ++k) tot += s_red[k * EPB + t];
-        const float gr = (float)(tot * (double)scale);
-        handoff_store(grads + d.dst + mine, gr);
-        if (fuse) opt_update_p<true>(d.dst + mine, gr, pi, params, s1, s2, s3, oa);
-    }
-}
 __global__ __launch_bounds__(256) void reduce_grads_quad_kernel(QuadArgs a, float* __restrict__ grads, float scale, int fuse,
                                                                 float* __restrict__ params, float* __restrict__ s1,
                                                                 float* __restrict__ s2, float* __restrict__ s3, OptArgs oa) {
@@ -333,44 +116,69 @@
     return DCV_OK;
 }
 
-static int launch_reduce(dcv_mlp* m, const ReduceArgs& ra_all, int l0, int l1, bool fuse_opt, const OptArgs& oa, hipStream_t s) {
+struct ReduceSet {
     ReduceArgs ra;
-    ra.L = 0;
     int max_splits = 0, max_bblocks = 0;
     int64_t max_total = 0;
+};
+static ReduceSet reduce_set(const dcv_mlp* m, const ReduceArgs& ra_all, int l0, int l1) {
+    ReduceSet rs;
+    rs.ra.L = 0;
     auto take = [&](const ReduceDesc& d) {
-        ra.l[ra.L++] = d;
-        if (d.splits > max_splits) max_splits = d.splits;
-        if (d.bblocks > max_bblocks) max_bblocks = d.bblocks;
-        if (d.w_count + d.out > max_total) max_total = d.w_count + d.out;
+        rs.ra.l[rs.ra.L++] = d;
+        if (d.splits > rs.max_splits) rs.max_splits = d.splits;
+        if (d.bblocks > rs.max_bblocks) rs.max_bblocks = d.bblocks;
+        if (d.w_count + d.out > rs.max_total) rs.max_total = d.w_count + d.out;
     };
     for (int l = l0; l < l1; ++l) take(ra_all.l[l]);
     for (int l = l0; l < l1; ++l)
         if (m->layers[l].bn) take(ra_all.l[m->L + l]);
+    return rs;
+}
+static bool quad_takes(const ReduceSet& rs) {
+    static const bool quad_off = [] { const char* e = getenv("DCV_REDUCE_QUAD"); return e && e[0] == '0'; }();
+    return rs.max_splits <= 512 && rs.max_bblocks <= 1024 && !quad_off;
+}
+static int quad_items(const ReduceSet& rs, int part, QuadArgs* qa, int64_t* blocks_out) {
+    qa->n = 0;
+    int64_t blocks = 0;
+    auto item = [&](const float* src, int64_t dst, int64_t count, int parts, int64_t stride) {
+        if (count <= 0) return;
+        if (!src || parts < 0) parts = 0;
+        QuadItem& q = qa->it[qa->n++];
+        q = QuadItem{src, dst, stride, (int)count, parts, (int)blocks, quad_groups(parts)};
+        blocks += cdiv(count, 1024 / q.groups);
+    };
+    for (int l = 0; l < rs.ra.L; ++l) {
+        const ReduceDesc& d = rs.ra.l[l];
+        DCV_REQUIRE(d.w_count < (1ll << 31), "reduce: layer too large");
+        if (part == 0 || (part == 1) == (l == 0)) item(d.slab, d.w_off, d.w_count, d.splits, rd_wstride(d));
+        if (part != 1) item(d.bpart, d.b_off, d.out, d.bblocks, rd_bstride(d));
+    }
+    DCV_REQUIRE(blocks < (1ll << 31), "reduce: grid out of range");
+    *blocks_out = blocks;
+    return DCV_OK;
+}
+static int launch_quad(dcv_mlp* m, const QuadArgs& qa, int64_t blocks, bool fuse_opt, const OptArgs& oa, hipStream_t s) {
+    hipLaunchKernelGGL(reduce_grads_quad_kernel, dim3((unsigned)blocks), dim3(256), 0, s, qa, m->grads, 1.f, fuse_opt ? 1 : 0, m->params, m->adam_m,
+                       m->adam_v, m->opt_aux, oa);
+    DCV_CHECK_LAUNCH();
+    return DCV_OK;
+}
+
+static int launch_reduce(dcv_mlp* m, const ReduceArgs& ra_all, int l0, int l1, bool fuse_opt, const OptArgs& oa, hipStream_t s) {
+    const ReduceSet rs = reduce_set(m, ra_all, l0, l1);
+    const ReduceArgs& ra = rs.ra;
     if (ra.L <= 0) return DCV_OK;
-    static const bool quad_off = [] { const char* e = getenv("DCV_REDUCE_QUAD"); return e && e[0] == '0'; }();
-    if (max_splits <= 512 && max_bblocks <= 1024 && !quad_off) {
+    if (quad_takes(rs)) {
         QuadArgs qa;
-        qa.n = 0;
         int64_t blocks = 0;
-        auto item = [&](const float* src, int64_t dst, int64_t count, int parts, int64_t stride) {
-            if (count <= 0) return;
-            if (!src || parts < 0) parts = 0;
-            QuadItem& q = qa.it[qa.n++];
-            q = QuadItem{src, dst, stride, (int)count, parts, (int)blocks, quad_groups(parts)};
-            blocks += cdiv(count, 1024 / q.groups);
-        };
-        for (int l = 0; l < ra.L; ++l) {
-            DCV_REQUIRE(ra.l[l].w_count < (1ll << 31), "reduce: layer too large");
-            item(ra.l[l].slab, ra.l[l].w_off, ra.l[l].w_count, ra.l[l].splits, rd_wstride(ra.l[l]));
-            item(ra.l[l].bpart, ra.l[l].b_off, ra.l[l].out, ra.l[l].bblocks, rd_bstride(ra.l[l]));
-        }
+        const int rc = quad_items(rs, 0, &qa, &blocks);
+        if (rc) return rc;
         if (blocks <= 0) return DCV_OK;
-        DCV_REQUIRE(blocks < (1ll << 31), "reduce: grid out of range");
-        hipLaunchKernelGGL(reduce_grads_quad_kernel, dim3((unsigned)blocks), dim3(256), 0, s, qa, m->grads, 1.f, fuse_opt ? 1 : 0, m->params,
-                           m->adam_m, m->adam_v, m->opt_aux, oa);
-    } else if (max_splits <= 512 && max_bblocks <= 1024) {
-        int64_t bx = cdiv(max_total, 64);
+        return launch_quad(m, qa, blocks, fuse_opt, oa, s);
+    } else if (rs.max_splits <= 512 && rs.max_bblocks <= 1024) {
+        int64_t bx = cdiv(rs.max_total, 64);
         if (bx > 2048) bx = 2048;
         hipLaunchKernelGGL(reduce_grads_small_kernel, dim3((unsigned)bx, ra.L), dim3(256), 0, s, ra, m->grads, 1.f, fuse_opt ? 1 : 0, m->params,
                            m->adam_m, m->adam_v, m->opt_aux, oa);
@@ -518,7 +326,33 @@
     m->upper_cb(m->upper_cb_user);
     return DCV_OK;
 }
-int finish_grads(dcv_mlp* m, const ReduceArgs& ra, bool fuse_opt, bool upper_done, hipStream_t s) {
+int ride_upper(dcv_mlp* m, const ReduceArgs& ra, const Operand& A, const Operand& B, int64_t M, int64_t N, int64_t K, int64_t k_chunk,
+               const EpiSlab& epi, OptArgs* oa, hipStream_t s) {
+    static const bool off = [] { const char* e = getenv("DCV_NO_REDUCE_RIDE"); return e && e[0] == '1'; }();
+    if (off || m->upper_cb || m->L < 2) return 1;
+    const ReduceSet rs = reduce_set(m, ra, 0, m->L);
+    if (!quad_takes(rs) || !wgrad_reduce_applies(A, B, M, N, K, k_chunk)) return 1;
+    QuadArgs qa;
+    int64_t blocks = 0;
+    int rc = quad_items(rs, 2, &qa, &blocks);
+    if (rc) return rc;
+    if (blocks <= 0) return 1;
+    rc = first_step_state(m, s);
+    if (rc) return rc;
+    *oa = next_opt_args(m);
+    rc = launch_wgrad_reduce(A, B, M, N, K, k_chunk, epi, qa, blocks, m->grads, m->params, m->adam_m, m->adam_v, m->opt_aux, *oa, s);
+    if (rc) return rc;
+    m->last_ride = (int)blocks;
+    return DCV_OK;
+}
+int finish_grads(dcv_mlp* m, const ReduceArgs& ra, bool fuse_opt, bool upper_done, hipStream_t s, const OptArgs* ridden) {
+    if (ridden) {
+        QuadArgs qa;
+        int64_t blocks = 0;
+        const int rcq = quad_items(reduce_set(m, ra, 0, m->L), 1, &qa, &blocks);
+        if (rcq || blocks <= 0) return rcq;
+        return launch_quad(m, qa, blocks, true, *ridden, s);
+    }
     int rc = reduce_upper(m, ra, fuse_opt, &upper_done, s);
     if (rc) return rc;
     OptArgs oa{};
diff --git a/deep_cartograph_amd/csrc/mlp_state.h b/deep_cartograph_amd/csrc/mlp_state.h
--- a/deep_cartograph_amd/csrc/mlp_state.h
+++ b/deep_cartograph_amd/csrc/mlp_state.h
@@ -56,6 +56,7 @@
     dcv::TailWs tail;
     dcv::EvalGroupWs eval_ws;
     int last_eval_group;
+    int last_ride;
     void (*upper_cb)(void*);
     void* upper_cb_user;
     bool head_done;
@@ -250,7 +251,10 @@
 ReduceArgs reduce_args_of(const dcv_mlp* m, const ReduceArgsView& v);
 int launch_reduce(dcv_mlp* m, const ReduceArgs& ra, int l0, int l1, hipStream_t s);
 int reduce_upper(dcv_mlp* m, const ReduceArgs& ra, bool fuse_opt, bool* done, hipStream_t s);
-int finish_grads(dcv_mlp* m, const ReduceArgs& ra, bool fuse_opt, bool upper_done, hipStream_t s);
+struct OptArgs;
+int ride_upper(dcv_mlp* m, const ReduceArgs& ra, const Operand& A, const Operand& B, int64_t M, int64_t N, int64_t K, int64_t k_chunk,
+               const EpiSlab& epi, OptArgs* oa, hipStream_t s);
+int finish_grads(dcv_mlp* m, const ReduceArgs& ra, bool fuse_opt, bool upper_done, hipStream_t s, const OptArgs* ridden = nullptr);
 int apply_impl(dcv_mlp* m, void* stream);
 int launch_sum_partials(const double* part, int nblocks, int width, double* out, hipStream_t s);
 int stats_rows_per_block(int64_t batch);
diff --git a/deep_cartograph_amd/csrc/reduce_quad.h b/deep_cartograph_amd/csrc/reduce_quad.h
--- /dev/null
+++ b/deep_cartograph_amd/csrc/reduce_quad.h
@@ -0,0 +1,231 @@
+#pragma once
+#include "gemm_kernels.h"
+#include "handoff.h"
+
+namespace dcv {
+
+struct OptArgs {
+    int kind, flag;
+    int first;
+    float lr, b1, b2, eps, wd;
+    float c1, c2;
+    float w1, w2;
+    float decay;
+    float p0, p1, p2, p3;
+    int maximize;
+    float* img;
+    const int* img_idx;
+};
+template <bool WT>
+__device__ __forceinline__ void opt_st(float* p, float v) {
+    if constexpr (WT) handoff_store(p, v);
+    else *p = v;
+}
+template <bool WT>
+__device__ __forceinline__ void opt_stp(const OptArgs& a, float* p, int64_t i, float v) {
+    opt_st<WT>(p + i, v);
+    if (a.img != nullptr) {
+        const int j = a.img_idx[i];
+        if (j >= 0) opt_st<WT>(a.img + j, v);
+    }
+}
+template <bool WT = false>
+__device__ __forceinline__ void opt_update_p(int64_t i, float gi, float pi, float* __restrict__ p, float* __restrict__ s1, float* __restrict__ s2,
+                                             float* __restrict__ s3, const OptArgs& a) {
+    if (a.maximize) gi = -gi;
+    switch (a.kind) {
+        case DCV_OPT_ADAM:
+        case DCV_OPT_ADAMW: {
+            if (a.kind == DCV_OPT_ADAMW) pi = pi * a.decay;
+            else if (a.wd != 0.f) gi = fmaf(a.wd, pi, gi);
+            float mi = s1[i], vi = s2[i];
+            mi = mi + (gi - mi) * a.w1;
+            vi = vi * a.b2 + a.w2 * gi * gi;
+            float vden = vi;
+            if (a.flag) {
+                vden = fmaxf(s3[i], vi);
+                opt_st<WT>(s3 + i, vden);
+            }
+            const float denom = sqrtf(vden) / a.c2 + a.eps;
+            opt_st<WT>(s1 + i, mi);
+            opt_st<WT>(s2 + i, vi);
+            opt_stp<WT>(a, p, i, pi - a.c1 * (mi / denom));
+            break;
+        }
+        case DCV_OPT_SGD: {
+            if (a.wd != 0.f) gi = fmaf(a.wd, pi, gi);
+            if (a.b1 != 0.f) {
+                float bi = a.first ? gi : s1[i] * a.b1 + a.w1 * gi;
+                opt_st<WT>(s1 + i, bi);
+                gi = a.flag ? fmaf(a.b1, bi, gi) : bi;
+            }
+            opt_stp<WT>(a, p, i, pi - a.lr * gi);
+            break;
+        }
+        case DCV_OPT_RMSPROP: {
+            if (a.wd != 0.f) gi = fmaf(a.wd, pi, gi);
+            float sq = s2[i] * a.b2 + a.w2 * gi * gi;
+            opt_st<WT>(s2 + i, sq);
+            float avg;
+            if (a.flag) {
+                float ga = s3[i];
+                ga = ga + (gi - ga) * a.w2;
+                opt_st<WT>(s3 + i, ga);
+                avg = sqrtf(sq - ga * ga) + a.eps;
+            } else {
+                avg = sqrtf(sq) + a.eps;
+            }
+            if (a.b1 > 0.f) {
+                const float bi = s1[i] * a.b1 + gi / avg;
+                opt_st<WT>(s1 + i, bi);
+                opt_stp<WT>(a, p, i, pi - a.lr * bi);
+            } else {
+                opt_stp<WT>(a, p, i, pi - a.lr * (gi / avg));
+            }
+            break;
+        }
+        case DCV_OPT_ADAMAX: {
+            if (a.wd != 0.f) gi = fmaf(a.wd, pi, gi);
+            float mi = s1[i];
+            mi = mi + (gi - mi) * a.w1;
+            const float ui = fmaxf(s2[i] * a.b2, fabsf(gi) + a.eps);
+            opt_st<WT>(s1 + i, mi);
+            opt_st<WT>(s2 + i, ui);
+            opt_stp<WT>(a, p, i, pi - a.c1 * (mi / ui));
+            break;
+        }
+        case DCV_OPT_NADAM: {
+            if (a.wd != 0.f) {
+                if (a.flag) pi = pi * a.decay;
+                else gi = fmaf(a.wd, pi, gi);
+            }
+            float mi = s1[i], vi = s2[i];
+            mi = mi + (gi - mi) * a.w1;
+            vi = vi * a.b2 + a.w2 * gi * gi;
+            const float denom = sqrtf(vi / a.c2) + a.eps;
+            opt_st<WT>(s1 + i, mi);
+            opt_st<WT>(s2 + i, vi);
+            pi = pi + a.p0 * (gi / denom);
+            opt_stp<WT>(a, p, i, pi + a.p1 * (mi / denom));
+            break;
+        }
+        case DCV_OPT_RADAM: {
+            if (a.wd != 0.f) {
+                if (a.flag) pi = pi * a.decay;
+                else gi = fmaf(a.wd, pi, gi);
+            }
+            float mi = s1[i], vi = s2[i];
+            mi = mi + (gi - mi) * a.w1;
+            vi = vi * a.b2 + a.w2 * gi * gi;
+            opt_st<WT>(s1 + i, mi);
+            opt_st<WT>(s2 + i, vi);
+            const float mhat = mi / a.c1;
+            if (a.p0 > 0.f) opt_stp<WT>(a, p, i, pi - ((mhat * a.lr) * (a.c2 / (sqrtf(vi) + a.eps))) * a.p0);
+            else opt_stp<WT>(a, p, i, pi - mhat * a.lr);
+            break;
+        }
+        case DCV_OPT_ADADELTA: {
+            if (a.wd != 0.f) gi = fmaf(a.wd, pi, gi);
+            const float sq = s1[i] * a.b2 + a.w2 * gi * gi;
+            const float acc = s2[i];
+            const float delta = sqrtf(acc + a.eps) / sqrtf(sq + a.eps) * gi;
+            opt_st<WT>(s1 + i, sq);
+            opt_st<WT>(s2 + i, acc * a.b2 + a.w2 * delta * delta);
+            opt_stp<WT>(a, p, i, pi - a.lr * delta);
+            break;
+        }
+        case DCV_OPT_ASGD: {
+            if (a.wd != 0.f) gi = fmaf(a.wd, pi, gi);
+            pi = pi * a.p0;
+            opt_stp<WT>(a, p, i, pi - a.p1 * gi);
+            break;
+        }
+        case DCV_OPT_RPROP: {
+            const float sg = gi * s1[i];
+            const float f = sg > 0.f ? a.p1 : (sg < 0.f ? a.p0 : 1.f);
+            const float st = fminf(fmaxf(s2[i] * f, a.p2), a.p3);
+            opt_st<WT>(s2 + i, st);
+            if (sg < 0.f) gi = 0.f;
+            const float sgn = gi > 0.f ? 1.f : (gi < 0.f ? -1.f : 0.f);
+            opt_stp<WT>(a, p, i, pi - sgn * st);
+            opt_st<WT>(s1 + i, gi);
+            break;
+        }
+        default: {
+            if (a.wd != 0.f) gi = fmaf(a.wd, pi, gi);
+            const float su = s2[i] + gi * gi;
+            opt_st<WT>(s2 + i, su);
+            opt_stp<WT>(a, p, i, pi - a.c1 * (gi / (sqrtf(su) + a.eps)));
+            break;
+        }
+    }
+}
+__device__ __forceinline__ void opt_update(int64_t i, float gi, float* __restrict__ p, float* __restrict__ s1, float* __restrict__ s2,
+                                           float* __restrict__ s3, const OptArgs& a) {
+    opt_update_p(i, gi, p[i], p, s1, s2, s3, a);
+}
+
+struct QuadItem {
+    const float* src;
+    int64_t dst;
+    int64_t stride;
+    int count, parts;
+    int blk0;
+    int groups;
+};
+struct QuadArgs {
+    QuadItem it[4 * DCV_MAX_LAYERS];
+    int n;
+};
+inline int quad_groups(int parts) { return parts > 32 ? 16 : 4; }
+template <int G>
+__device__ __forceinline__ void reduce_quad_block(const QuadItem& d, int blk, float* __restrict__ grads, float scale, int fuse,
+                                                  float* __restrict__ params, float* __restrict__ s1, float* __restrict__ s2,
+                                                  float* __restrict__ s3, const OptArgs& oa, double* s_red) {
+    constexpr int EPB = 1024 / G, TPG = EPB / 4;
+    const int t = threadIdx.x, g = t / TPG, sub = t % TPG;
+    const int base = blk * EPB;
+    const int mine = base + t;
+    const bool fin = t < EPB && mine < d.count;
+    float pi = 0.f;
+    if (fuse && fin) pi = params[d.dst + mine];
+    const int e0 = base + 4 * sub;
+    double acc[4] = {0.0, 0.0, 0.0, 0.0};
+    if (e0 < d.count && (d.stride & 3) == 0 && e0 + 4 <= d.stride && (reinterpret_cast<uintptr_t>(d.src) & 15) == 0) {
+        const float* p = d.src + e0;
+#pragma unroll 8
+        for (int q = g; q < d.parts; q += G) {
+            const float4 v = *reinterpret_cast<const float4*>(p + (int64_t)q * d.stride);
+            acc[0] += (double)v.x;
+            acc[1] += (double)v.y;
+            acc[2] += (double)v.z;
+            acc[3] += (double)v.w;
+        }
+    } else if (e0 < d.count) {
+        const float* p = d.src + e0;
+        const int nv = d.count - e0 < 4 ? d.count - e0 : 4;
+#pragma unroll 4
+        for (int q = g; q < d.parts; q += G) {
+#pragma unroll
+            for (int j = 0; j < 4; ++j)
+                if (j < nv) acc[j] += (double)p[(int64_t)q * d.stride + j];
+        }
+    }
+#pragma unroll
+    for (int j = 0; j < 4; ++j) s_red[g * EPB + 4 * sub + j] = acc[j];
+    __syncthreads();
+    if (fin) {
+        double tot = s_red[t];
+#pragma unroll
+        for (int k = 1; k < G; ++k) tot += s_red[k * EPB + t];
+        const float gr = (float)(tot * (double)scale);
+        handoff_store(grads + d.dst + mine, gr);
+        if (fuse) opt_update_p<true>(d.dst + mine, gr, pi, params, s1, s2, s3, oa);
+    }
+}
+
+bool wgrad_reduce_applies(const Operand& A, const Operand& B, int64_t M, int64_t N, int64_t K, int64_t k_chunk);
+int launch_wgrad_reduce(const Operand& A, const Operand& B, int64_t M, int64_t N, int64_t K, int64_t k_chunk, const EpiSlab& e, const QuadArgs& qa,
+                        int64_t qblocks, float* grads, float* params, float* s1, float* s2, float* s3, const OptArgs& oa, hipStream_t s);
+
+}
diff --git a/deep_cartograph_amd/csrc/ride.hip b/deep_cartograph_amd/csrc/ride.hip
--- /dev/null
+++ b/deep_cartograph_amd/csrc/ride.hip
@@ -0,0 +1,75 @@
+#include "reduce_quad.h"
+
+namespace dcv {
+
+template <class Cfg>
+__global__ __launch_bounds__(256, 2) void wgrad_reduce_kernel(Operand A, Operand B, GemmDims d, EpiSlab e, int blocks1, QuadArgs qa,
+                                                            float* __restrict__ grads, float* __restrict__ params, float* __restrict__ s1,
+                                                            float* __restrict__ s2, float* __restrict__ s3, OptArgs oa) {
+    extern __shared__ __attribute__((aligned(16))) float lds_f[];
+    if ((int)blockIdx.x < blocks1) {
+        const BlockMap bm = map_block<kTN>(d, (int)blockIdx.x);
+        e.z = bm.split;
+        gemm_block<kTN, Cfg, 1, true, false, EpiSlab>(A, B, 0, d, bm.tile_m, bm.tile_n, bm.k_begin, bm.k_end, lds_f, e, -1);
+    } else {
+        const int b = (int)blockIdx.x - blocks1;
+        int l = 0;
+        while (l + 1 < qa.n && b >= qa.it[l + 1].blk0) ++l;
+        const QuadItem& q = qa.it[l];
+        double* s_red = reinterpret_cast<double*>(lds_f);
+        if (q.groups == 16) reduce_quad_block<16>(q, b - q.blk0, grads, 1.f, 1, params, s1, s2, s3, oa, s_red);
+        else reduce_quad_block<4>(q, b - q.blk0, grads, 1.f, 1, params, s1, s2, s3, oa, s_red);
+    }
+}
+
+template <class Cfg>
+static int launch_ride_cfg(const Operand& A, const Operand& B, int64_t M, int64_t N, int64_t K, int64_t kc, const EpiSlab& e, const QuadArgs& qa,
+                           int64_t qblocks, float* grads, float* params, float* s1, float* s2, float* s3, const OptArgs& oa, hipStream_t s) {
+    GemmPlan p;
+    const int rc = prepare_gemm<kTN, Cfg, 1, EpiSlab>(A, B, M, N, K, kc, e, nullptr, nullptr, &p);
+    if (rc) return rc;
+    DCV_REQUIRE(p.vec && !p.gather, "wgrad + reduction launch: operands need the 16-byte, ungathered loader");
+    const int64_t blocks1 = (int64_t)p.d.tiles_m * p.d.tiles_n * p.splits;
+    DCV_REQUIRE(blocks1 + qblocks < (1ll << 31), "wgrad + reduction launch: grid out of range");
+    constexpr size_t lds = gemm_lds_bytes<Cfg, 1>();
+    static_assert(lds >= 1024 * sizeof(double), "the reduction blocks take 8 KB of the product's LDS");
+    auto kern = wgrad_reduce_kernel<Cfg>;
+    if (lds > 64 * 1024) {
+        static bool attr_set = false;
+        if (!attr_set) {
+            DCV_CHECK_HIP(hipFuncSetAttribute(reinterpret_cast<const void*>(kern), hipFuncAttributeMaxDynamicSharedMemorySize, (int)lds));
+            attr_set = true;
+        }
+    }
+    const dim3 grid((unsigned)(blocks1 + qblocks));
+    if (g_launch_ev.start != nullptr) {
+        const LaunchEvents ev = g_launch_ev;
+        g_launch_ev = LaunchEvents{};
+        g_launch_taken = ev.start;
+        hipExtLaunchKernelGGL(kern, grid, dim3(256), (uint32_t)lds, s, ev.start, ev.stop, 0u, A, B, p.d, e, (int)blocks1, qa, grads, params, s1, s2, s3, oa);
+    } else {
+        hipLaunchKernelGGL(kern, grid, dim3(256), lds, s, A, B, p.d, e, (int)blocks1, qa, grads, params, s1, s2, s3, oa);
+    }
+    DCV_CHECK_LAUNCH();
+    return DCV_OK;
+}
+
+bool wgrad_reduce_applies(const Operand& A, const Operand& B, int64_t M, int64_t N, int64_t K, int64_t kc) {
+    const CfgPick c = pick_cfg<kTN, false>(M, N, K, kc);
+    if (c != kPickQuarter && c != kPickBig) return false;
+    return A.vec_ok && B.vec_ok && A.rows.idx == nullptr && B.rows.idx == nullptr;
+}
+
+int launch_wgrad_reduce(const Operand& A, const Operand& B, int64_t M, int64_t N, int64_t K, int64_t kc, const EpiSlab& e, const QuadArgs& qa,
+                        int64_t qblocks, float* grads, float* params, float* s1, float* s2, float* s3, const OptArgs& oa, hipStream_t s) {
+    DCV_REQUIRE(wgrad_reduce_applies(A, B, M, N, K, kc) && qblocks > 0, "wgrad + reduction launch: not applicable");
+    const bool big = pick_cfg<kTN, false>(M, N, K, kc) == kPickBig;
+    if (gemm_split()) {
+        if (big) return launch_ride_cfg<CfgBigT<true>>(A, B, M, N, K, kc, e, qa, qblocks, grads, params, s1, s2, s3, oa, s);
+        return launch_ride_cfg<CfgQuarterT<true>>(A, B, M, N, K, kc, e, qa, qblocks, grads, params, s1, s2, s3, oa, s);
+    }
+    if (big) return launch_ride_cfg<CfgBigT<false>>(A, B, M, N, K, kc, e, qa, qblocks, grads, params, s1, s2, s3, oa, s);
+    return launch_ride_cfg<CfgQuarterT<false>>(A, B, M, N, K, kc, e, qa, qblocks, grads, params, s1, s2, s3, oa, s);
+}
+
+}
diff --git a/deep_cartograph_amd/hip.py b/deep_cartograph_amd/hip.py
--- a/deep_cartograph_amd/hip.py
+++ b/deep_cartograph_amd/hip.py
@@ -648,6 +648,13 @@
     def last_path(self) -> int:
         return int(self.lib.dcv_mlp_last_path(self.h))
 
+    def last_ride(self) -> int:
+        return int(self.lib.dcv_mlp_last_ride(self.h))
+
+    def opt_state_view(self, which: int) -> Optional[torch.Tensor]:
+        ptr = self.lib.dcv_mlp_opt_state(self.h, int(which))
+        return self._flat_view(ptr, self.n_params, torch.float32) if ptr else None
+
     def dropout_step(self) -> int:
         return int(self.lib.dcv_mlp_dropout_step(self.h))
 
diff --git a/include/dcv.h b/include/dcv.h
--- a/include/dcv.h
+++ b/include/dcv.h
@@ -160,6 +160,8 @@
                      int32_t set, void* stream);
 int32_t dcv_mlp_last_path(const dcv_mlp* m);
 int32_t dcv_mlp_last_eval_group(const dcv_mlp* m);
+int32_t dcv_mlp_last_ride(const dcv_mlp* m);
+float* dcv_mlp_opt_state(dcv_mlp* m, int32_t which);
 int dcv_mlp_layer_output(dcv_mlp* m, int32_t layer, int64_t rows, float* out_d, void* stream);
 int dcv_mlp_train_step(dcv_mlp* m, const float* Xn_d, int64_t ld, const int64_t* idx_d, int64_t row0,
                        int32_t batch, void* stream);
```

New measurement: 83.47 million (median of 6 runs). 1.1% higher.
